# janhq/cortex.llamacpp

Hardware: AMD Instinct MI355X
Metric: decode tok/s, Llama-3-8B Q4_K_M GGUF (prefill tok/s in `prefill_tok_s`) (higher is better)
Workload: dtype int8 dot (Q4_K/Q6_K x Q8_K), f32 accumulate

## Files before the change

cortex.llamacpp_amd/binding.py:

```python
from __future__ import annotations

import ctypes as C
import os

import numpy as np

HERE = os.path.dirname(os.path.abspath(__file__))
F32, F16, Q4_0, Q8_0, Q4_K, Q5_K, Q6_K, Q8_K = 0, 1, 2, 8, 12, 13, 14, 15
Q2_K, Q3_K = 10, 11
Q5_0, IQ4_NL = 6, 20
Q4_1, Q5_1 = 3, 7
IQ4_XS = 23
BF16 = 30
MXFP4 = 39


class MI355Error(RuntimeError):
    pass


def lib_path() -> str:
    return os.environ.get("MI355_LLAMA_LIB") or os.path.join(HERE, "lib", "libmi355_llama.so")


class ModelParams(C.Structure):
    _fields_ = [("n_gpu_layers", C.c_int32), ("main_gpu", C.c_int32), ("use_mmap", C.c_int32), ("use_mlock", C.c_int32),
                ("tp_rank", C.c_int32), ("tp_size", C.c_int32), ("prefill_planes", C.c_int32)]


class ContextParams(C.Structure):
    _fields_ = [("n_ctx", C.c_uint32), ("n_batch", C.c_uint32), ("n_ubatch", C.c_uint32), ("n_seq_max", C.c_uint32),
                ("type_k", C.c_int32), ("type_v", C.c_int32), ("flash_attn", C.c_int32), ("embeddings", C.c_int32),
                ("use_graphs", C.c_int32), ("logits_to_host", C.c_int32)]


class Batch(C.Structure):
    _fields_ = [("n_tokens", C.c_int32), ("token", C.POINTER(C.c_int32)), ("embd", C.POINTER(C.c_float)),
                ("pos", C.POINTER(C.c_int32)), ("n_seq_id", C.POINTER(C.c_int32)),
                ("seq_id", C.POINTER(C.POINTER(C.c_int32))), ("logits", C.POINTER(C.c_int8))]


_vp, _i32, _i64, _u32, _u64, _f32, _sz, _cp = C.c_void_p, C.c_int32, C.c_int64, C.c_uint32, C.c_uint64, C.c_float, C.c_size_t, C.c_char_p
ENGINE_CB = C.CFUNCTYPE(None, C.c_char_p, C.c_char_p, C.c_void_p)
SYMBOLS = {
    "mi355_backend_init": (C.c_int, []),
    "mi355_backend_free": (None, []),
    "mi355_device_count": (C.c_int, []),
    "mi355_last_error": (_cp, []),
    "mi355_time_us": (_i64, []),
    "mi355_print_system_info": (_cp, []),
    "mi355_model_default_params": (ModelParams, []),
    "mi355_model_load_from_file": (_vp, [_cp, ModelParams]),
    "mi355_model_free": (None, [_vp]),
    "mi355_model_n_vocab": (_i32, [_vp]),
    "mi355_model_n_embd": (_i32, [_vp]),
    "mi355_model_n_layer": (_i32, [_vp]),
    "mi355_model_n_head": (_i32, [_vp]),
    "mi355_model_n_head_kv": (_i32, [_vp]),
    "mi355_model_n_ctx_train": (_i32, [_vp]),
    "mi355_model_size": (_u64, [_vp]),
    "mi355_model_cpu_buffer": (_u64, [_vp]),
    "mi355_model_other_buffer": (_u64, [_vp]),
    "mi355_model_bytes_per_token": (_u64, [_vp]),
    "mi355_model_planes_bytes": (_u64, [_vp]),
    "mi355_debug_set_option": (C.c_int, [_cp, _i32]),
    "mi355_model_desc": (_cp, [_vp]),
    "mi355_model_meta_str": (C.c_int, [_vp, _cp, _cp, _sz]),
    "mi355_context_default_params": (ContextParams, []),
    "mi355_context_new": (_vp, [_vp, ContextParams]),
    "mi355_context_free": (None, [_vp]),
    "mi355_n_ctx": (_u32, [_vp]),
    "mi355_n_batch": (_u32, [_vp]),
    "mi355_n_ubatch": (_u32, [_vp]),
    "mi355_context_device_bytes": (_u64, [_vp]),
    "mi355_batch_init": (Batch, [_i32, _i32, _i32]),
    "mi355_batch_free": (None, [Batch]),
    "mi355_decode": (_i32, [_vp, Batch]),
    "mi355_greedy_steps": (_i32, [_vp, _i32, _i32, _i32, _i32, _vp]),
    "mi355_get_logits_ith": (C.POINTER(C.c_float), [_vp, _i32]),
    "mi355_get_argmax_ith": (_i32, [_vp, _i32]),
    "mi355_get_topk_ith": (_i32, [_vp, _i32, _i32, _i32, _vp, _vp, _vp, _f32, _f32, _f32, _vp, _vp]),
    "mi355_debug_mega_steps": (C.c_int64, [_vp]),
    "mi355_debug_engine_steps": (C.c_int64, [_vp]),
    "mi355_debug_fused_skipped_steps": (C.c_int64, [_vp]),
    "mi355_debug_qkv_attn_launches": (C.c_int64, [_vp]),
    "mi355_debug_qkv_attn_plan": (C.c_int64, [C.c_int32] * 10 + [C.POINTER(C.c_int32)]),
    "mi355_set_embeddings": (None, [_vp, _i32]),
    "mi355_get_embeddings_ith": (C.POINTER(C.c_float), [_vp, _i32]),
    "mi355_synchronize": (None, [_vp]),
    "mi355_kv_cache_clear": (None, [_vp]),
    "mi355_kv_cache_seq_rm": (_i32, [_vp, _i32, _i32, _i32]),
    "mi355_kv_cache_seq_cp": (None, [_vp, _i32, _i32, _i32, _i32]),
    "mi355_kv_cache_seq_add": (None, [_vp, _i32, _i32, _i32, _i32]),
    "mi355_kv_cache_used_cells": (_i32, [_vp]),
    "mi355_debug_enable_taps": (None, [_vp, _i32]),
    "mi355_debug_layer_out": (_i32, [_vp, _i32, _vp, _sz]),
    "mi355_op_quantize_act": (C.c_int, [_i32, _vp, _i64, _i64, _vp]),
    "mi355_op_rms_norm_quant": (C.c_int, [_vp, _vp, _i64, _i64, _f32, _vp, _vp]),
    "mi355_op_swiglu_quant": (C.c_int, [_vp, _vp, _i64, _i64, _vp]),
    "mi355_op_mul_mat": (C.c_int, [_i32, _vp, _i64, _i64, _vp, _i64, _vp, _vp, _vp]),
    "mi355_op_mul_mat_add": (C.c_int, [_i32, _vp, _i64, _i64, _vp, _i64, _vp, _vp]),
    "mi355_op_mul_mat_fused": (C.c_int, [_i32, _vp, _i64, _i64, _vp, _vp, _f32, _vp]),
    "mi355_op_f32_to_bf16": (C.c_int, [_vp, _i64, _vp]),
    "mi355_op_mul_mat_bf16": (C.c_int, [_i32, _vp, _vp, _i64, _vp, _i64, _vp, _vp, _i32, _i32, _i32, _i32, _vp]),
    "mi355_op_ffn_gate_up": (C.c_int, [_i32, _vp, _vp, _i64, _i64, _vp, _i64, _vp]),
    "mi355_op_rms_norm_mul": (C.c_int, [_vp, _vp, _i64, _i64, _f32, _vp]),
    "mi355_op_rope": (C.c_int, [_vp, _i32, _i32, _i32, _vp, _i64, _f32, _f32, _vp, _i32]),
    "mi355_op_rope_yarn": (C.c_int, [_vp, _i32, _i32, _i32, _vp, _i64, _f32, _f32, _vp, _i32, _f32, _f32, _f32, _f32]),
    "mi355_op_get_rows": (C.c_int, [_i32, _vp, _i64, _i64, _vp, _i64, _vp]),
    "mi355_op_swiglu": (C.c_int, [_vp, _vp, _i64, _vp]),
    "mi355_op_soft_max": (C.c_int, [_vp, _vp, _i64, _i64, _f32, _vp]),
    "mi355_op_moe_route": (C.c_int, [_vp, _i64, _i32, _i32, _vp, _vp]),
    "mi355_op_moe_router": (C.c_int, [_i32, _vp, _i32, _i64, _vp, _i64, _i32, _i32, _vp, _vp, _vp, _vp]),
    "mi355_op_flash_attn": (C.c_int, [_vp, _i64, _i32, _i32, _i32, _i32, _vp, _i32, _vp, _i32, _vp, _vp, _f32, _vp]),
    "mi355_op_attn_step": (C.c_int, [_vp, _vp, _vp, _i32, _i32, _i32, _i32, _vp, _i32, _vp, _i32, _vp, _i32, _i32, _f32, _i32, _f32, _i32, _vp, _i64, _vp, _i32,
                                     _vp, _vp, _vp, _vp]),
    "mi355_op_attn_decode_neox": (C.c_int, [_vp, _vp, _vp, _i32, _i32, _i32, _i32, _vp, _i32, _vp, _i32, _vp, _i32, _i32, _f32, _f32, _vp, _vp, _f32, _i32,
                                            _vp, _vp, _vp]),
    "mi355_op_kv_store": (C.c_int, [_i32, _vp, _vp, _vp, _i64, _i32, _i32, _i32, _i32, _i32, _i32, _i32, _i32, _vp, _vp, _f32, _f32, _vp, _vp, _vp, _f32, _vp, _vp]),
    "mi355_op_k_shift": (C.c_int, [_i32, _i32, _i32, _i32, _i32, _i32, _vp, _f32, _f32, _vp, _f32, _f32, _f32, _f32, _vp]),
    "mi355_bench_hbm_read": (C.c_double, [_sz, C.c_int]),
    "mi355_profile_last_decode": (_i32, [_vp, C.POINTER(_cp), C.POINTER(_f32), _i32]),
    "mi355_profile_enable": (None, [_vp, _i32]),
    "mi355_debug_force_moe_ids": (C.c_int, [_vp, _vp, _i32, _i32, _i32]),
    "mi355_bench_weight_sweep": (C.c_double, [_vp, C.c_int, C.POINTER(_u64)]),
    "mi355_bench_weight_sweep2": (C.c_double, [_vp, C.c_int, C.POINTER(_u64), C.POINTER(C.c_int32)]),
    "mi355_tokenize": (_i32, [_vp, _cp, _i32, C.POINTER(C.c_int32), _i32, _i32, _i32]),
    "mi355_token_to_piece": (_i32, [_vp, _i32, C.c_char_p, _i32, _i32]),
    "mi355_token_bos": (_i32, [_vp]),
    "mi355_token_eos": (_i32, [_vp]),
    "mi355_token_is_eog": (_i32, [_vp, _i32]),
    "mi355_engine_create": (_vp, []),
    "mi355_engine_destroy": (None, [_vp]),
    "mi355_engine_set_release_callback": (None, [_vp, _vp]),
    "mi355_engine_load_model": (None, [_vp, _cp, ENGINE_CB, _vp]),
    "mi355_engine_unload_model": (None, [_vp, _cp, ENGINE_CB, _vp]),
    "mi355_engine_get_model_status": (None, [_vp, _cp, ENGINE_CB, _vp]),
    "mi355_engine_get_models": (None, [_vp, _cp, ENGINE_CB, _vp]),
    "mi355_engine_handle_chat_completion": (None, [_vp, _cp, ENGINE_CB, _vp]),
    "mi355_engine_handle_embedding": (None, [_vp, _cp, ENGINE_CB, _vp]),
    "mi355_engine_is_supported": (_i32, [_vp, _cp]),
    "mi355_engine_stop_inferencing": (None, [_vp, _cp]),
    "mi355_engine_load": (None, [_vp, _cp, _cp, _i32, _cp, _i32, _i32]),
    "mi355_engine_unload": (None, [_vp]),
    "mi355_engine_set_file_logger": (None, [_vp, _i32, _cp]),
    "mi355_engine_set_log_level": (None, [_vp, _i32]),
    "mi355_engine_set_log_callback": (None, [_vp, _vp, _vp]),
    "mi355_clip_model_load": (_vp, [_cp, _i32]),
    "mi355_clip_free": (None, [_vp]),
    "mi355_clip_n_mmproj_embd": (_i32, [_vp]),
    "mi355_clip_n_patches": (_i32, [_vp]),
    "mi355_clip_image_size": (_i32, [_vp]),
    "mi355_clip_max_image_rows": (_i32, [_vp]),
    "mi355_clip_image_preprocess_grid": (_i32, [_vp, _vp, _i32, _i32, _vp, _sz, _vp, _vp]),
    "mi355_clip_image_load_from_bytes": (_i32, [_vp, _sz, C.POINTER(_i32), C.POINTER(_i32), _vp, _sz]),
    "mi355_clip_image_preprocess": (_i32, [_vp, _vp, _i32, _i32, _vp]),
    "mi355_clip_image_encode": (_i32, [_vp, _vp, _vp]),
    "mi355_llava_image_embed_from_bytes": (_i32, [_vp, _vp, _sz, _vp, _sz]),
    "mi355_tp_p2p_local_handle": (C.c_int, [_vp, _sz, _sz]),
    "mi355_tp_p2p_local_handle2": (C.c_int, [_vp, _sz, _sz, _sz]),
    "mi355_tp_p2p_prompt_exchanges": (C.c_int64, []),
    "mi355_tp_p2p_enable": (C.c_int, [_vp, _sz]),
    "mi355_tp_p2p_exchanges": (C.c_int64, []),
    "mi355_tp_unique_id": (C.c_int, [_vp, _sz]),
    "mi355_tp_init": (C.c_int, [_i32, _i32, _i32, _vp, _sz]),
    "mi355_tp_shutdown": (None, []),
    "mi355_tp_worker_main": (C.c_int, [C.c_int]),
    "mi355_tp_rank": (_i32, []),
# ... 498 lines not shown
        pos = np.asarray(pos, np.int32).reshape(-1)
        n = tokens.size
        b = self._batch(n)
        b.n_tokens = n
        C.memmove(b.token, tokens.ctypes.data, 4 * n)
        C.memmove(b.pos, pos.ctypes.data, 4 * n)
        for i in range(n):
            b.n_seq_id[i] = 1
            b.seq_id[i][0] = 0 if seq is None else int(seq[i] if np.ndim(seq) else seq)
            b.logits[i] = (1 if i == n - 1 else 0) if logits is None else int(bool(logits[i]))
        rc = self.lib.mi355_decode(self.h, b)
        if rc < 0:
            raise MI355Error(f"mi355_decode failed ({rc}): {_err(self.lib)}")
        return rc

    def decode_embd(self, embd, pos, seq=None, logits=None) -> int:
        embd = np.ascontiguousarray(embd, np.float32)
        pos = np.asarray(pos, np.int32).reshape(-1)
        n = pos.size
        if embd.shape != (n, self.model.n_embd):
            raise ValueError(f"embd must be [{n}][{self.model.n_embd}]")
        b = self.lib.mi355_batch_init(n, self.model.n_embd, 1)
        try:
            b.n_tokens = n
            C.memmove(b.embd, embd.ctypes.data, embd.nbytes)
            C.memmove(b.pos, pos.ctypes.data, 4 * n)
            for i in range(n):
                b.n_seq_id[i] = 1
                b.seq_id[i][0] = 0 if seq is None else int(seq[i] if np.ndim(seq) else seq)
                b.logits[i] = (1 if i == n - 1 else 0) if logits is None else int(bool(logits[i]))
            rc = self.lib.mi355_decode(self.h, b)
        finally:
            self.lib.mi355_batch_free(b)
        if rc < 0:
            raise MI355Error(f"mi355_decode failed ({rc}): {_err(self.lib)}")
        return rc

    def greedy_steps(self, first: int, pos0: int, n: int, seq: int = 0) -> np.ndarray:
        out = np.empty(n, np.int32)
        done = self.lib.mi355_greedy_steps(self.h, int(first), int(pos0), int(seq), int(n), out.ctypes.data)
        if done != n:
            raise MI355Error(f"mi355_greedy_steps stopped after {done} of {n}: {_err(self.lib)}")
        return out

    def logits(self, i: int = -1) -> np.ndarray:
        p = self.lib.mi355_get_logits_ith(self.h, i)
        if not p:
            raise MI355Error(f"no logits for that batch row: {_err(self.lib)}")
        return np.ctypeslib.as_array(p, shape=(self.model.n_vocab,)).copy()

    def logits_ready(self, i: int = -1) -> None:
        if not self.lib.mi355_get_logits_ith(self.h, i):
            raise MI355Error(f"no logits for that batch row: {_err(self.lib)}")

    def set_embeddings(self, on: bool = True) -> None:
        self.lib.mi355_set_embeddings(self.h, int(on))

    def embeddings(self, i: int = -1) -> np.ndarray:
        p = self.lib.mi355_get_embeddings_ith(self.h, i)
        if not p:
            raise MI355Error("no embeddings for that row")
        return np.ctypeslib.as_array(p, shape=(self.model.n_embd,)).copy()

    def argmax(self, i: int = -1) -> int:
        return int(self.lib.mi355_get_argmax_ith(self.h, i))

    def mega_steps(self) -> int:
        return int(self.lib.mi355_debug_mega_steps(self.h))

    def topk(self, k: int, i: int = -1, adj_tok=(), adj_bias=(), adj_count=(), repeat: float = 1.0, freq: float = 0.0, present: float = 0.0):
        at = np.ascontiguousarray(adj_tok, np.int32); ab = np.ascontiguousarray(adj_bias, np.float32); ac = np.ascontiguousarray(adj_count, np.int32)
        toks = np.zeros(k, np.int32); lg = np.zeros(k, np.float32)
        r = self.lib.mi355_get_topk_ith(self.h, i, k, at.size, _ptr(at), _ptr(ab), _ptr(ac), repeat, freq, present, _ptr(toks), _ptr(lg))
        if r != k:
            raise MI355Error(f"mi355_get_topk_ith failed: {_err(self.lib)}")
        return toks, lg

    def fused_skipped_steps(self) -> int:
        return int(self.lib.mi355_debug_fused_skipped_steps(self.h))

    def qkv_attn_launches(self) -> int:
        return int(self.lib.mi355_debug_qkv_attn_launches(self.h))

    def engine_steps(self) -> int:
        return int(self.lib.mi355_debug_engine_steps(self.h))

    def synchronize(self):
        self.lib.mi355_synchronize(self.h)

    def kv_clear(self):
        self.lib.mi355_kv_cache_clear(self.h)

    def kv_seq_rm(self, seq, p0, p1) -> bool:
        return bool(self.lib.mi355_kv_cache_seq_rm(self.h, seq, p0, p1))

    def kv_seq_cp(self, s, d, p0, p1):
        self.lib.mi355_kv_cache_seq_cp(self.h, s, d, p0, p1)

    def kv_seq_add(self, seq, p0, p1, delta):
        self.lib.mi355_kv_cache_seq_add(self.h, seq, p0, p1, delta)

    def kv_used(self) -> int:
        return int(self.lib.mi355_kv_cache_used_cells(self.h))

    def enable_taps(self, on: bool = True):
        self.lib.mi355_debug_enable_taps(self.h, int(on))

    def layer_out(self, il: int, n_tokens: int) -> np.ndarray:
        out = np.zeros((n_tokens, self.model.n_embd), np.float32)
        n = self.lib.mi355_debug_layer_out(self.h, il, _ptr(out), out.size)
        if n < 0:
            raise MI355Error("debug taps not enabled")
        return out[:n]

    def profile(self, on: bool = True):
        self.lib.mi355_profile_enable(self.h, int(on))

    def last_profile(self) -> dict:
        names = (_cp * 64)()
        us = (_f32 * 64)()
        n = self.lib.mi355_profile_last_decode(self.h, names, us, 64)
        return {names[i].decode(): float(us[i]) for i in range(n)}

    def force_moe_ids(self, ids: np.ndarray) -> None:
        ids = np.ascontiguousarray(ids, np.int32)
        rc = self.lib.mi355_debug_force_moe_ids(self.h, _ptr(ids), ids.shape[0], ids.shape[1], ids.shape[2])
        if rc != 0:
            raise MI355Error(f"mi355_debug_force_moe_ids failed ({rc}): {_err(self.lib)}")

    def weight_sweep_us(self, iters: int = 5):
        b = _u64(0)
        us = self.lib.mi355_bench_weight_sweep(self.h, iters, C.byref(b))
        return float(us), int(b.value)

    def weight_sweep(self, iters: int = 5):
        b, n = _u64(0), C.c_int32(0)
        us = self.lib.mi355_bench_weight_sweep2(self.h, iters, C.byref(b), C.byref(n))
        return float(us), int(b.value), int(n.value)

    def close(self):
        if self._b is not None:
            self.lib.mi355_batch_free(self._b)
            self._b = None
        if self.h:
            self.lib.mi355_context_free(self.h)
            self.h = None


class Engine:

    def __init__(self):
        import json
        import threading
        self._json, self._threading = json, threading
        self.lib = load_library()
        self.h = self.lib.mi355_engine_create()
        if not self.h:
            raise MI355Error(f"mi355_engine_create failed: {_err(self.lib)}")

    def _call(self, fn, body: dict, wait_done: bool = True, timeout: float = 120.0):
        out, done = [], self._threading.Event()

        def on(status, payload, _user):
            st, bd = self._json.loads(status.decode("utf-8", "replace")), self._json.loads(payload.decode("utf-8", "replace"))
            out.append((st, bd))
            if st.get("is_done", True) or st.get("has_error", False):
# ... 38 lines not shown
```

cortex.llamacpp_amd/csrc/c_api.cc:

```cpp
#include "../../include/mi355_llama.h"

#include <atomic>
#include <memory>
#include <new>
#include <chrono>
#include <cstdio>
#include <cstdlib>
#include <cstring>
#include <string>
#include <vector>

#include "../host/clip.h"
#include "../host/engine.h"
#include "../host/hip_backend.h"
#include "../host/log.h"
#include "../host/runtime.h"
#include "../host/tp_comm.h"
#include "../host/tp_split.h"
#include "../host/vocab.h"

namespace mi355 {
const std::string &last_error_string();
}

// ... 144 lines not shown
        std::string err;
        if (!c->init(err)) { fail(err); return nullptr; }
        mi355_context *h = new mi355_context{c.get(), {}};
        c.release();
        return h;
    )
}
void mi355_context_free(mi355_context *ctx) {
    if (!ctx) return;
    delete ctx->c;
    delete ctx;
}
uint32_t mi355_n_ctx(const mi355_context *ctx) { return ctx->c->cp.n_ctx; }
uint32_t mi355_n_batch(const mi355_context *ctx) { return ctx->c->cp.n_batch; }
uint32_t mi355_n_ubatch(const mi355_context *ctx) { return ctx->c->cp.n_ubatch; }
uint64_t mi355_context_device_bytes(const mi355_context *ctx) { return ctx->c->device_bytes; }

mi355_batch mi355_batch_init(int32_t n_tokens, int32_t embd, int32_t n_seq_max) {
    mi355_batch b{};
    if (embd > 0) b.embd = (float *)calloc((size_t)n_tokens * (size_t)embd, sizeof(float));
    else b.token = (mi355_token *)calloc((size_t)n_tokens, sizeof(mi355_token));
    b.pos = (mi355_pos *)calloc((size_t)n_tokens, sizeof(mi355_pos));
    b.n_seq_id = (int32_t *)calloc((size_t)n_tokens, sizeof(int32_t));
    b.seq_id = (mi355_seq_id **)calloc((size_t)n_tokens + 1, sizeof(mi355_seq_id *));
    for (int i = 0; i < n_tokens; i++) b.seq_id[i] = (mi355_seq_id *)calloc((size_t)(n_seq_max > 0 ? n_seq_max : 1), sizeof(mi355_seq_id));
    b.seq_id[n_tokens] = nullptr;
    b.logits = (int8_t *)calloc((size_t)n_tokens, 1);
    return b;
}
void mi355_batch_free(mi355_batch b) {
    free(b.token); free(b.embd); free(b.pos); free(b.n_seq_id); free(b.logits);
    if (b.seq_id) {
        for (int i = 0; b.seq_id[i]; i++) free(b.seq_id[i]);
        free(b.seq_id);
    }
}

int32_t mi355_decode(mi355_context *ctx, mi355_batch batch) {
    if (!ctx) return MI355_ERR_ARG;
    MI355_GUARD(return MI355_ERR_ARG,
        const int rc = ctx->c->decode(batch.n_tokens, batch.embd ? nullptr : batch.token, batch.pos, batch.n_seq_id, batch.seq_id, batch.logits, batch.embd);
        if (rc < 0) fail(ctx->c->last_error);
        return rc;
    )
}
int32_t mi355_greedy_steps(mi355_context *ctx, mi355_token first, mi355_pos pos0, mi355_seq_id seq, int32_t n, mi355_token *out_tokens) {
    if (!ctx || n < 0) return MI355_ERR_ARG;
    MI355_GUARD(return MI355_ERR_ARG,
        int32_t tok = first, one = 1, sid = seq;
        int32_t *sp = &sid;
        const int8_t flag = 1;
        for (int32_t i = 0; i < n; i++) {
            int32_t pos = pos0 + i;
            const int rc = ctx->c->decode(1, &tok, &pos, &one, &sp, &flag);
            if (rc != 0) { if (rc < 0) fail(ctx->c->last_error); return i; }
            if (!ctx->c->logits_ith(0)) { fail("no logits row"); return i; }
            tok = ctx->c->argmax_ith(0);
            if (tok < 0) { fail(ctx->c->last_error.empty() ? "arg-max failed" : ctx->c->last_error); return i; }
            if (out_tokens) out_tokens[i] = tok;
        }
        return n;
    )
}
float *mi355_get_logits_ith(mi355_context *ctx, int32_t i) {
    float *p = ctx->c->logits_ith(i);
    if (!p) fail(ctx->c->last_error.empty() ? "no logits for that batch row" : ctx->c->last_error);
    return p;
}
int32_t mi355_get_argmax_ith(mi355_context *ctx, int32_t i) { return ctx->c->argmax_ith(i); }
int32_t mi355_get_topk_ith(mi355_context *ctx, int32_t i, int32_t k, int32_t n_adj, const int32_t *adj_tok, const float *adj_bias, const int32_t *adj_count,
                           float penalty_repeat, float penalty_freq, float penalty_present, int32_t *toks_out, float *logits_out) {
    if (!ctx || !toks_out || !logits_out || n_adj < 0 || n_adj > TOPK_MAX_ADJ || (n_adj > 0 && (!adj_tok || !adj_bias || !adj_count))) { fail("bad arguments"); return -1; }
    TopkAdj a{};
    a.n = n_adj; a.repeat = penalty_repeat; a.freq = penalty_freq; a.present = penalty_present;
    for (int j = 0; j < n_adj; j++) { a.tok[j] = adj_tok[j]; a.bias[j] = adj_bias[j]; a.cnt[j] = adj_count[j]; }
    const int r = ctx->c->topk_ith(i, k, a, toks_out, logits_out);
    if (r < 0) fail(ctx->c->last_error.empty() ? "top-k failed" : ctx->c->last_error);
    return r;
}
int64_t mi355_debug_mega_steps(const mi355_context *ctx) { return ctx->c->mega_steps; }
int64_t mi355_debug_engine_steps(const mi355_context *ctx) { return ctx->c->engine_steps; }
int64_t mi355_debug_fused_skipped_steps(const mi355_context *ctx) { return ctx->c->fused_skipped_steps; }
int64_t mi355_debug_qkv_attn_launches(const mi355_context *ctx) { return ctx->c->qkv_attn_launches; }
int64_t mi355_debug_qkv_attn_plan(int32_t type_q, int32_t type_k, int32_t type_v, int32_t type_o, int32_t n_embd, int32_t n_head, int32_t n_head_kv, int32_t head_dim,
                                  int32_t type_kv, int32_t n_kv, int32_t *slots_out) {
    int slots = 0;
    const size_t lds = qkv_attn_out_plan_lds(type_q, type_k, type_v, type_o, n_embd, n_head, n_head_kv, head_dim, type_kv, n_kv, &slots);
    if (slots_out) *slots_out = slots;
    return (int64_t)lds;
}
void mi355_set_embeddings(mi355_context *ctx, int32_t enabled) { ctx->c->embeddings_enabled = enabled != 0 || ctx->c->model->hp.encoder; }
float *mi355_get_embeddings_ith(mi355_context *ctx, int32_t i) { return ctx->c->embeddings_ith(i); }
void mi355_synchronize(mi355_context *ctx) { ctx->c->synchronize(); }

mi355_clip *mi355_clip_model_load(const char *path, int32_t main_gpu) {
    if (!path) { fail("clip_model_load: no path"); return nullptr; }
    MI355_GUARD(return nullptr,
        std::unique_ptr<mi355_clip> c(new mi355_clip);
        const std::string err = c->m.load(path, main_gpu < 0 ? 0 : main_gpu);
        if (!err.empty()) { fail(err); return nullptr; }
        return c.release();
    )
}
void mi355_clip_free(mi355_clip *clip) { delete clip; }
int32_t mi355_clip_n_mmproj_embd(const mi355_clip *clip) { return clip ? clip->m.proj_dim : 0; }
int32_t mi355_clip_n_patches(const mi355_clip *clip) { return clip ? clip->m.n_patches() : 0; }
int32_t mi355_clip_image_size(const mi355_clip *clip) { return clip ? clip->m.image_size : 0; }
int32_t mi355_clip_max_image_rows(const mi355_clip *clip) { return clip ? clip->m.max_image_rows() : 0; }
int32_t mi355_clip_image_preprocess_grid(const mi355_clip *clip, const uint8_t *rgb, int32_t nx, int32_t ny, float *out, size_t out_floats, int32_t *grid_w, int32_t *grid_h) {
    if (!clip || !rgb || !out || nx <= 0 || ny <= 0) { fail("clip_image_preprocess_grid: bad arguments"); return MI355_ERR_ARG; }
    MI355_GUARD(return MI355_ERR_ARG,
        ClipImageU8 img;
        img.nx = nx; img.ny = ny; img.rgb.assign(rgb, rgb + (size_t)3 * nx * ny);
        std::vector<std::vector<float>> imgs;
        int gw = 0, gh = 0;
        clip->m.preprocess_all(img, imgs, gw, gh);
        const size_t per = (size_t)3 * clip->m.image_size * clip->m.image_size;
        if (out_floats < per * imgs.size()) { fail("clip_image_preprocess_grid: output buffer too small"); return MI355_ERR_ARG; }
        for (size_t i = 0; i < imgs.size(); i++) memcpy(out + i * per, imgs[i].data(), per * sizeof(float));
        if (grid_w) *grid_w = gw;
        if (grid_h) *grid_h = gh;
        return (int32_t)imgs.size();
    )
}
int32_t mi355_clip_image_load_from_bytes(const uint8_t *bytes, size_t n_bytes, int32_t *nx, int32_t *ny, uint8_t *rgb_out, size_t rgb_cap) {
    MI355_GUARD(return MI355_ERR_ARG,
        ClipImageU8 img;
        const std::string err = clip_image_load_from_bytes(bytes, n_bytes, img);
        if (!err.empty()) { fail(err); return MI355_ERR_ARG; }
        if (nx) *nx = img.nx;
        if (ny) *ny = img.ny;
        if (rgb_out) {
            if (rgb_cap < img.rgb.size()) { fail("clip_image_load_from_bytes: rgb_cap too small"); return MI355_ERR_ARG; }
            memcpy(rgb_out, img.rgb.data(), img.rgb.size());
        }
        return MI355_OK;
    )
}
int32_t mi355_clip_image_preprocess(const mi355_clip *clip, const uint8_t *rgb, int32_t nx, int32_t ny, float *out) {
    if (!clip || !rgb || !out || nx <= 0 || ny <= 0) { fail("clip_image_preprocess: bad arguments"); return MI355_ERR_ARG; }
    MI355_GUARD(return MI355_ERR_ARG,
        ClipImageU8 img;
        img.nx = nx; img.ny = ny; img.rgb.assign(rgb, rgb + (size_t)3 * nx * ny);
        std::vector<float> f;
        clip->m.preprocess(img, f);
        memcpy(out, f.data(), f.size() * sizeof(float));
        return MI355_OK;
    )
}
int32_t mi355_clip_image_encode(mi355_clip *clip, const float *img, float *out) {
    if (!clip || !img || !out) { fail("clip_image_encode: bad arguments"); return MI355_ERR_ARG; }
    MI355_GUARD(return MI355_ERR_ARG,
        const std::string err = clip->m.encode(img, out);
        if (!err.empty()) { fail(err); return MI355_ERR_ARG; }
        return MI355_OK;
    )
}
int32_t mi355_llava_image_embed_from_bytes(mi355_clip *clip, const uint8_t *bytes, size_t n_bytes, float *out, size_t out_floats) {
    if (!clip || !bytes || !out) { fail("llava_image_embed: bad arguments"); return MI355_ERR_ARG; }
    MI355_GUARD(return MI355_ERR_ARG,
        ClipImageU8 img;
        std::string err = clip_image_load_from_bytes(bytes, n_bytes, img);
        if (!err.empty()) { fail(err); return MI355_ERR_ARG; }
        std::vector<float> rows;
        int n_rows = 0;
        err = clip->m.embed(img, rows, n_rows);
// ... 843 lines not shown
    if (form < 2 && ((size_t)n_rot + kv_dim) * 4 > 48 * 1024) { fail("n_head_kv * head_dim too wide for the generic kernel's LDS"); return MI355_ERR_ARG; }
    if (form < 2 && (q_norm || k_norm) && (n_rot != D || (D != 64 && D != 128))) { fail("the q / k norm works on whole heads of 64 or 128"); return MI355_ERR_ARG; }
    std::vector<uint8_t> kc, vc;
    std::vector<uint16_t> ks, vs;
    cache_planes_from_rows(type_k, k_cache, G, D, n_cells, kc, ks);
    cache_planes_from_rows(type_v, v_cache, G, D, n_cells, vc, vs);
    DevBuf dk(kc.size()), dks(ks.size() * 2 + 16), dv(vc.size()), dvs(vs.size() * 2 + 16), dqn((size_t)D * 4), dkn_w((size_t)D * 4), dff((size_t)n_rot * 2 + 16);
    DevBuf dq((size_t)T * q_dim * 4), dkn((size_t)T * kv_dim * 4), dvn((size_t)T * kv_dim * 4), dtp((size_t)T * 4), dcell((size_t)T * 4), dcsb((size_t)T * n_rot * 4 + 64);
    if (!dk.up(kc.data(), kc.size()) || !dv.up(vc.data(), vc.size()) || !dks.p || !dvs.p || !dq.p || (q && !dq.up(q, (size_t)T * q_dim * 4)) ||
        !dkn.up(k, (size_t)T * kv_dim * 4) || !dvn.up(v, (size_t)T * kv_dim * 4) || !dtp.up(tok_pos, (size_t)T * 4) || !dcell.up(tok_cell, (size_t)T * 4) || !dcsb.p ||
        (q_norm && !dqn.up(q_norm, (size_t)D * 4)) || (k_norm && !dkn_w.up(k_norm, (size_t)D * 4)) ||
        (freq_factors && !dff.up(freq_factors, (size_t)(n_rot / 2) * 4))) { fail("device alloc/copy failed"); return MI355_ERR_OOM; }
    if (!ks.empty() && !dks.up(ks.data(), ks.size() * 2)) return MI355_ERR_OOM;
    if (!vs.empty() && !dvs.up(vs.data(), vs.size() * 2)) return MI355_ERR_OOM;
    RopeArgs ra{};
    ra.n_rot = n_rot; ra.freq_base = rope_base; ra.freq_scale = freq_scale; ra.freq_factors = freq_factors ? dff.as<float>() : nullptr; ra.neox = neox ? 1 : 0;
    ra.q_norm = q_norm ? dqn.as<float>() : nullptr; ra.k_norm = k_norm ? dkn_w.as<float>() : nullptr; ra.qk_eps = eps;
    if (form == 2 && !rope_q_kv_store_fast_applicable(H, G, D, type_k, type_v, ra)) { fail("the vectorised prompt store has no form for these arguments"); return MI355_ERR_ARG; }
    if (form == 3 && !kv_store_fast_applicable(G, D, type_k, type_v, ra)) { fail("the small-batch decode store has no form for these arguments"); return MI355_ERR_ARG; }
    KVLayerView kv{};
    kv.k = dk.as<uint8_t>(); kv.kd = dks.as<uint16_t>(); kv.v = dv.as<uint8_t>(); kv.vd = dvs.as<uint16_t>();
    hipError_t e = hipSuccess;
    if (form != 0) e = launch_rope_table(dtp.as<int32_t>(), (int)T, ra, dcsb.as<float>(), nullptr);
    if (e != hipSuccess) return hip_fail(e, "rope_table");
    if (form < 2)
        e = launch_rope_kv_store(dq.as<float>(), dkn.as<float>(), dvn.as<float>(), (int)T, H, G, D, dtp.as<int32_t>(), dcell.as<int32_t>(), ra, kv, type_k, type_v, n_cells,
                                 form == 1 ? dcsb.as<float>() : nullptr, nullptr);
    else if (form == 2)
        e = launch_rope_q_kv_store_fast(dq.as<float>(), dkn.as<float>(), dvn.as<float>(), (int)T, H, G, D, dcsb.as<float>(), ra, dcell.as<int32_t>(), kv, type_k, type_v,
                                        n_cells, nullptr);
    else
        e = launch_kv_store_fast(dkn.as<float>(), dvn.as<float>(), (int)T, G, D, dcsb.as<float>(), ra, dcell.as<int32_t>(), kv, type_k, type_v, n_cells, nullptr);
    if (e == hipSuccess) e = hipDeviceSynchronize();
    if (e != hipSuccess) return hip_fail(e, "kv_store");
    if (form != 3 && !dq.down(q, (size_t)T * q_dim * 4)) return MI355_ERR_HIP;
    if (!cache_rows_from_planes(type_k, dk, dks, G, D, n_cells, k_cache) || !cache_rows_from_planes(type_v, dv, dvs, G, D, n_cells, v_cache)) return MI355_ERR_HIP;
    return MI355_OK;
}

int mi355_op_k_shift(int32_t type_k, int32_t G, int32_t D, int32_t n_rot, int32_t neox, int32_t n_cells, const int32_t *delta, float rope_base, float freq_scale,
                     const float *freq_factors, float ext_factor, float attn_factor, float corr_lo, float corr_hi, void *k_cache) {
    if (!need_device()) return MI355_ERR_NO_DEVICE;
    if (!delta || !k_cache || G < 1 || D < 32 || D % 32 || n_rot < 2 || n_rot > D || n_rot % 2 || n_cells < 1) { fail("bad geometry / null argument"); return MI355_ERR_ARG; }
    if (type_k != T_F16 && type_k != T_Q8_0 && type_k != T_Q4_0) { fail("bad cache type"); return MI355_ERR_ARG; }
    if (((size_t)n_rot + (size_t)G * D) * 4 > 48 * 1024) { fail("n_head_kv * head_dim too wide for the kernel's LDS"); return MI355_ERR_ARG; }
    std::vector<uint8_t> kc;
    std::vector<uint16_t> ks;
    cache_planes_from_rows(type_k, k_cache, G, D, n_cells, kc, ks);
    DevBuf dk(kc.size()), dks(ks.size() * 2 + 16), dd((size_t)n_cells * 4), dff((size_t)n_rot * 2 + 16);
    if (!dk.up(kc.data(), kc.size()) || !dks.p || !dd.up(delta, (size_t)n_cells * 4) || (freq_factors && !dff.up(freq_factors, (size_t)(n_rot / 2) * 4))) {
        fail("device alloc/copy failed"); return MI355_ERR_OOM;
    }
    if (!ks.empty() && !dks.up(ks.data(), ks.size() * 2)) return MI355_ERR_OOM;
    RopeArgs ra{};
    ra.n_rot = n_rot; ra.freq_base = rope_base; ra.freq_scale = freq_scale; ra.freq_factors = freq_factors ? dff.as<float>() : nullptr; ra.neox = neox ? 1 : 0;
    ra.ext_factor = ext_factor; ra.attn_factor = attn_factor; ra.corr_lo = corr_lo; ra.corr_hi = corr_hi;
    KVLayerView kv{};
    kv.k = dk.as<uint8_t>(); kv.kd = dks.as<uint16_t>();
    hipError_t e = launch_k_shift(kv, type_k, G, D, n_cells, dd.as<int32_t>(), ra, nullptr);
    if (e == hipSuccess) e = hipDeviceSynchronize();
    if (e != hipSuccess) return hip_fail(e, "k_shift");
    return cache_rows_from_planes(type_k, dk, dks, G, D, n_cells, k_cache) ? MI355_OK : MI355_ERR_HIP;
}

int mi355_debug_set_option(const char *name, int32_t value) {
    if (!name) return MI355_ERR_ARG;
    if (!strcmp(name, "mmq_planes")) { g_op_mmq_planes = value != 0; return MI355_OK; }
    if (!strcmp(name, "mmq_tiles")) { mmq_set_tiles(value); return MI355_OK; }
    if (!strcmp(name, "mmq_q80_tiles")) { mmq_q80_set_tiles(value); return MI355_OK; }
    if (!strcmp(name, "mmq_split")) { mmq_set_split(value); return MI355_OK; }
    if (!strcmp(name, "mmq_lds_form")) { mmq_set_lds_form(value); return MI355_OK; }
    if (!strcmp(name, "mmq_ksplit")) { g_op_mmq_ksplit = value != 0; return MI355_OK; }
    if (!strcmp(name, "attn_store_fuse")) { set_attn_store_fuse(value != 0); return MI355_OK; }
    if (!strcmp(name, "rope_fast")) { set_rope_fast(value != 0); return MI355_OK; }
    if (!strcmp(name, "decode_mega") || !strcmp(name, "decode_engine")) {
        if (value > 0 && !experiments_built()) { fail(std::string(name) + ": the experiment kernels are not in this build (MI355_BUILD_EXPERIMENTS=1 python cortex.llamacpp_amd/build.py --force)"); return MI355_ERR_ARG; }
        if (name[7] == 'm') set_decode_mega(value != 0); else set_decode_engine(value);
        return MI355_OK;
    }
    if (!strcmp(name, "tp_p2p")) { tp_p2p_use(value != 0); return MI355_OK; }
    if (!strcmp(name, "tp_p2p_prompt")) { tp_p2p_use_prompt(value != 0); return MI355_OK; }
    if (!strcmp(name, "mmvq_stream")) { mmvq_set_stream(value != 0); return MI355_OK; }
    if (!strcmp(name, "attn_out_fused")) { set_attn_out_fused(value); return MI355_OK; }
    if (!strcmp(name, "qkv_attn_fused")) { set_qkv_attn_fused(value); return MI355_OK; }
    if (!strcmp(name, "moe_group_min")) { set_moe_group_min(value); return MI355_OK; }
    if (!strcmp(name, "moe_q80_grouped")) { set_moe_q80_grouped(value != 0); return MI355_OK; }
    if (!strcmp(name, "fa_v_acc_f16")) { set_fa_v_acc_f16(value); return MI355_OK; }
    if (!strcmp(name, "raise_stream_error")) { debug_raise_stream_error((unsigned)value); return MI355_OK; }
    if (!strcmp(name, "tp_null_group")) { tp_set_null_group(0, value); return MI355_OK; }
    fail(std::string("unknown option ") + name);
    return MI355_ERR_ARG;
}

int mi355_tp_unique_id(void *id_out, size_t cap) {
    if (!need_device()) return MI355_ERR_NO_DEVICE;
    std::string err;
    const int n = tp_unique_id(id_out, cap, err);
    if (n < 0) { fail(err); return MI355_ERR_ARG; }
    return n;
}
int mi355_tp_init(int32_t device, int32_t rank, int32_t size, const void *id, size_t id_len) {
    if (!need_device()) return MI355_ERR_NO_DEVICE;
    if (hipSetDevice(device) != hipSuccess) { fail("hipSetDevice failed"); return MI355_ERR_ARG; }
    std::string err;
    if (tp_init(rank, size, id, id_len, err) != 0) { fail(err); return MI355_ERR_ARG; }
    return MI355_OK;
}
void mi355_tp_shutdown(void) { tp_shutdown(); }
int mi355_tp_worker_main(int sock_fd) {
    try {
        if (!g_backend_ok && mi355_backend_init() != MI355_OK) return 66;
        return tp_split_worker_main(sock_fd);
    } catch (const std::exception &e) {
        fprintf(stderr, "mi355_tp_worker: %s\n", e.what());
        return 70;
    } catch (...) { return 70; }
}
int32_t mi355_tp_rank(void) { return tp_rank(); }
int32_t mi355_tp_size(void) { return tp_size(); }
int mi355_tp_set_host_exchange(mi355_tp_host_exchange fn, void *user, int32_t rank, int32_t size) {
    if (fn && (size < 1 || rank < 0 || rank >= size)) { fail("bad rank / size"); return MI355_ERR_ARG; }
    tp_set_host_exchange(reinterpret_cast<tp_host_exchange_fn>(fn), user, rank, size);
    return MI355_OK;
}

int mi355_tp_p2p_local_handle2(void *out, size_t cap, size_t max_floats, size_t prompt_floats) {
    if (!need_device()) return MI355_ERR_NO_DEVICE;
    std::string err;
    const int n = tp_p2p_local_handle(out, cap, max_floats, prompt_floats, err);
    if (n < 0) { fail(err); return MI355_ERR_ARG; }
    return n;
}
int mi355_tp_p2p_local_handle(void *out, size_t cap, size_t max_floats) { return mi355_tp_p2p_local_handle2(out, cap, max_floats, 0); }
int mi355_tp_p2p_enable(const void *handles, size_t len) {
    if (!need_device()) return MI355_ERR_NO_DEVICE;
    std::string err;
    if (tp_p2p_enable(handles, len, err) != 0) { fail(err); return MI355_ERR_HIP; }
    return MI355_OK;
}
int64_t mi355_tp_p2p_exchanges(void) { return tp_p2p_exchanges(); }
int64_t mi355_tp_p2p_prompt_exchanges(void) { return tp_p2p_prompt_exchanges(); }

double mi355_bench_hbm_read(size_t bytes, int iters) {
    if (!need_device()) return -1.0;
    return hbm_read_probe(bytes, iters);
}

static Vocab *model_vocab(mi355_model *m) {
    if (!m) { fail("null model"); return nullptr; }
    if (!m->vocab_tried) {
        m->vocab_tried = true;
        std::string err;
        m->vocab_ok = m->vocab.load(*m->m->file, err);
        if (!m->vocab_ok) fail("tokenizer: " + err);
    }
    return m->vocab_ok ? &m->vocab : nullptr;
}
int32_t mi355_tokenize(mi355_model *m, const char *text, int32_t text_len, mi355_token *out, int32_t cap, int32_t add_special, int32_t parse_special) {
    MI355_GUARD(return INT32_MIN,
        Vocab *v = model_vocab(m);
        if (!v || !text || text_len < 0) return INT32_MIN;
        const std::vector<int32_t> ids = v->tokenize(std::string(text, (size_t)text_len), add_special != 0, parse_special != 0);
        if ((int64_t)ids.size() > cap || !out) return -(int32_t)ids.size();
        memcpy(out, ids.data(), ids.size() * sizeof(int32_t));
        return (int32_t)ids.size();
    )
// ... 94 lines not shown
```

cortex.llamacpp_amd/csrc/kernels.h:

```cpp
#pragma once

#include "dev_common.h"

namespace mi355 {

struct ActQuant {
    int8_t *qs = nullptr;
    float *d = nullptr;
    int16_t *bsums = nullptr;
    int8_t *qs0 = nullptr;
    uint16_t *d0 = nullptr;
};

enum { EPI_STORE = 0, EPI_ADD = 1, EPI_SWIGLU = 2 };

struct MMVQSeg {
    const uint8_t *W;
    float *out;
    const float *resid;
    int type;
    int n_rows;
    int ld_out;
    size_t row_bytes;
    const int32_t *expert_sel;
    size_t expert_stride;
};

struct MMVQArgs {
    MMVQSeg seg[3];
    int seg_block0[4];
    int n_seg;
    int K;
    int T;
    int epi;
    int need_q8k, need_q80;
    int nck;
    int red_off;
    const int8_t *aq; const float *ad; const int16_t *abs;
    const int8_t *aq0; const uint16_t *ad0;
    int fuse_mode;
    const float *nx; const float *nw; float neps;
    int n_sel, sel_out_stride, sel_nx_stride;
    float *out_host;
};

hipError_t launch_mmvq(MMVQArgs a, hipStream_t st);
void mmvq_fast_set_threads(int nt);
inline bool mmvq_fast_kb_ok(int kb) { return (kb >= 1 && kb <= 7) || kb == 9 || kb == 10 || kb == 11 || kb == 14 || kb == 15; }
bool mmvq_fast_applicable(const MMVQArgs &a);
hipError_t launch_mmvq_fast(MMVQArgs a, hipStream_t st);
hipError_t launch_mmvq_ints(MMVQArgs a, int32_t *isum, int32_t *msum, hipStream_t st);
size_t mmvq_fast_plan(MMVQArgs &a, int blocks, int waves);
void mmvq_set_stream(bool on);
bool mmvq_stream_applicable(const MMVQArgs &a);
void mmvq_stream_set_anyorder_for_timing(bool on);
hipError_t launch_mmvq_stream(MMVQArgs a, hipStream_t st);

void mmvq_stream_plan(MMVQArgs &a, int blocks);
void mmvq_stream_set_error_word(unsigned *w);
struct KernelTimer {
    virtual ~KernelTimer() = default;
    virtual bool next(const char *role, hipEvent_t *start, hipEvent_t *stop) = 0;
};
void set_kernel_timer(KernelTimer *t);
KernelTimer *kernel_timer();

bool experiments_built();
struct EngineLayer {
    MMVQArgs wo, gu, dn, qkv;
    int has_qkv;
    int qk_norm;
};
bool decode_engine_applicable(const EngineLayer &l, int E, int FF);
void decode_engine_plan(EngineLayer &l);
size_t decode_engine_granule_words(int E, int FF);
void decode_engine_set_error_word(unsigned *w);
hipError_t launch_decode_engine(const EngineLayer *layer_dev, int E, int FF, unsigned long long *granules, const unsigned *epoch_dev, int layer_index,
                                unsigned long long *probe, hipStream_t st);

void set_num_cu(int n);
int num_cu();

bool mmq_applicable(int type, int K, int T);
void mmq_set_tiles(int mt);
size_t mmq_planes_bytes(int type, int64_t n_rows, int K);
size_t mmq_q80_copy_bytes(int type, int64_t n_rows, int K);
size_t mmq_q80_copy_row_bytes(int type, int K);
hipError_t launch_expand_q80_copy(int type, const uint8_t *W, size_t row_bytes, int n_rows, int K, uint8_t *dst, hipStream_t st);
hipError_t launch_mmq_expand(int type, const uint8_t *W, size_t row_bytes, int n_rows, int K, uint8_t *planes, hipStream_t st);
struct MMQWorkspace { float *p = nullptr; size_t bytes = 0; };
void mmq_set_split(int n);
void mmq_set_lds_form(int on);
bool mmq_planes_moe_ok(int type, int n_rows, int K);
hipError_t launch_mmq_planes_swiglu_moe(int type, const uint8_t *planes_gate, const uint8_t *planes_up, size_t plane_stride, int n_expert, const int32_t *meta,
                                        int n_rows, int K, int rows_max, const ActQuant &q, float *out, int ld_out, hipStream_t st);
hipError_t launch_mmq_planes_moe(int type, const uint8_t *planes, size_t plane_stride, int n_expert, const int32_t *meta, int n_rows, int K, int rows_max,
                                 const ActQuant &q, float *out, int ld_out, hipStream_t st);
hipError_t launch_mmq_planes(int type, const uint8_t *planes, int n_rows, int K, int T, const ActQuant &q, const int8_t *bh, const int8_t *bl,
                             float *out, int ld_out, const float *resid, hipStream_t st, MMQWorkspace wsp = MMQWorkspace());
struct MMQSeg {
    const uint8_t *W; size_t row_bytes; int n_rows, type;
    float *out; int ld_out; const float *resid;
    int tile0;
};
bool mmq_q80_applicable(int type, int K, int T);
hipError_t launch_mmq_q80(const uint8_t *W, size_t row_bytes, int n_rows, int K, int T, const ActQuant &q, float *out, int ld_out,
                          const float *resid, hipStream_t st, int form = 0, bool any_T = false);
enum : int { Q80_FORM_F16 = 0, Q80_FORM_MINS = 1, Q80_FORM_E8 = 2 };
int mmq_q80_copy_form(int type);
bool mmq_q80_moe_ok(int type, int n_rows, int K);
hipError_t launch_mmq_q80_moe(int type, const uint8_t *const *W, float *const *outs, int n_seg, size_t expert_stride, int n_expert, const int32_t *meta, int n_rows,
                              int K, int rows_max, const ActQuant &q, int ld_out, hipStream_t st);
void mmq_q80_set_tiles(int mt);
hipError_t launch_mmq_planes_multi(int type, const uint8_t *planes, const int *seg_rows, float *const *outs, const int *lds_out, int n_seg, int K, int T,
                                   const ActQuant &q, const int8_t *bh, const int8_t *bl, const float *resid, hipStream_t st,
                                   MMQWorkspace wsp = MMQWorkspace(), const int *seg_types = nullptr);
bool mmq_planes_mixed_ok(const int *seg_rows, int n_seg, int K, int T, MMQWorkspace wsp);
bool mmq_planes_swiglu_ok(int type_gate, int type_up, int n_rows, int K, int T);
hipError_t launch_mmq_planes_swiglu(int type, const uint8_t *planes_gate, const uint8_t *planes_up, int n_rows, int K, int T, const ActQuant &q,
                                    float *out, int ld_out, hipStream_t st);
bool mmq_ksplit_applicable(int type, int K, int T);
bool mmq_ksplit_preferred(int type, int n_rows, int K, int T, bool has_planes, bool pair = false);
hipError_t launch_mmq_ksplit_multi(const MMQSeg *segs, int n_seg, int K, int T, const ActQuant &q, const int8_t *bh, const int8_t *bl,
                                   bool swiglu, hipStream_t st);
hipError_t launch_mmq_ksplit(int type, const uint8_t *W, size_t row_bytes, int n_rows, int K, int T, const ActQuant &q,
                             const int8_t *bh, const int8_t *bl, float *out, int ld_out, const float *resid, hipStream_t st);
size_t mmq_prep_bytes(int K, int T);
// ... 194 lines not shown
```

cortex.llamacpp_amd/csrc/mmvq_stream.hip:

```cpp
#include "mmvq_stream_dev.h"

namespace mi355 {

namespace {

template <int KB, int FUSE, bool MOE>
__device__ __forceinline__ void stream_body(const MMVQArgs &ka) {
    extern __shared__ __attribute__((aligned(16))) uint8_t smem[];
#ifdef MI355_STREAM_PROBE
    const unsigned long long t_top = wall_clock64();
#endif
    StOp a;
    op_setup<false, MOE>(ka, a);
    const int wave = uni(tid_now() >> 6);
    sync_init(smem);
#ifdef MI355_STREAM_PROBE
    {
        unsigned dep = uni((int)a.total); asm volatile("" : "+s"(dep));
        const unsigned long long t_args = wall_clock64() + (dep & 0);
        if (g_stream_probe && (threadIdx.x & 63) == 0) {
            unsigned long long *pp = &g_stream_probe[(((size_t)(a.nck >> 2) * 256 + blockIdx.x) * ST_NW + wave) * 8];
            pp[0] = t_top; pp[7] = t_args;
        }
    }
#endif
    if (a.n_rows_wg <= 0) return;
    if (wave < ST_NL) {
        const int lane = tid_now() & 63;
        int *sy = reinterpret_cast<int *>(smem + ST_OFF_SYNC);
        LoaderState st{0, 0, 0, (unsigned)ST_RING_SLOTS, 0};
        const int early = (FUSE == 1 && a.ns_pad > ST_RING_SLOTS) ? ST_EARLY : 0;
        if (early == 0) ST_SPIN_WHILE(ld_sync(sy + SY_GO) < ST_NC, 0);
        ST_STAMP(2);
        loader_op(st, a, smem, wave, 0u, lane, early);
        ST_STAMP(1);
        loader_drain(st, smem, wave);
        ST_STAMP(5);
        return;
    }
    consumer_dispatch<KB, FUSE>(a, smem, wave - ST_NL, 0u, st_layout(KB));
}
struct StFast { const float *nx; const uint8_t *wbase; unsigned ow0, ow1, ow2, onw, kf, sg0, sg1, sg2, rb01, rb2; };
__device__ __forceinline__ void st_fast_setup(StFast f, StOp &o) {
    asm volatile("" : "+s"(f.ow0), "+s"(f.ow1), "+s"(f.ow2), "+s"(f.sg0), "+s"(f.sg1), "+s"(f.sg2), "+s"(f.rb01), "+s"(f.rb2));
    const unsigned kf = f.kf;
    const int nseg = (int)((kf >> 28) & 3u), lo1 = (int)((kf >> 8) & 1023u), lo2 = (int)((kf >> 18) & 1023u);
    const bool swiglu = ((kf >> 30) & 1u) != 0;
    const int b = (int)blockIdx.x;
    unsigned g = f.sg0, rb = f.rb01 & 0xffffu, ow = f.ow0;
    int lo = 0;
    if (nseg > 1 && b >= lo1) { g = f.sg1; rb = f.rb01 >> 16; ow = f.ow1; lo = lo1; }
    if (nseg > 2 && b >= lo2) { g = f.sg2; rb = f.rb2 & 0xffffu; ow = f.ow2; lo = lo2; }
    const int rpb = (int)(g & 2047u), full = (int)((g >> 11) & 1023u), rem = (int)(g >> 21);
    const int bl = b - lo;
    const int rows = bl < full ? rpb : bl == full ? rem : 0;
    o.W = f.wbase + ((size_t)ow << 4);
    o.W1 = f.wbase + ((size_t)f.ow1 << 4);
    o.b0 = bl * rpb; o.n_rows_wg = rows; o.row_bytes = rb;
    o.swiglu = swiglu;
    o.total = (unsigned)rows * rb;
    const int per_tensor = (int)((o.total + ST_SLOT - 1) / ST_SLOT);
    o.ns_raw = swiglu ? 2 * per_tensor : per_tensor;
    o.ns_pad = (o.ns_raw + 1) & ~1;
}

template <int KB>
__device__ __forceinline__ void stream_body_fast(const StFast &fa) {
    extern __shared__ __attribute__((aligned(16))) uint8_t smem[];
    const int wave = uni(tid_now() >> 6), lane = tid_now() & 63;
    EarlyAct<KB> ea;
    early_issue<KB, 1>(fa.nx, reinterpret_cast<const float *>(fa.wbase + ((size_t)fa.onw << 4)), (int)(fa.kf & 255u) << 8, wave >= ST_NL ? wave - ST_NL : 0, lane, ea);
    sync_init(smem);
    if (wave < ST_NL) {
        StOp a;
        st_fast_setup(fa, a);
        if (a.n_rows_wg <= 0) return;
        LoaderState st{0, 0, 0, (unsigned)ST_RING_SLOTS, 0};
        loader_op(st, a, smem, wave, 0u, lane, 0);
        loader_drain(st, smem, wave);
        return;
    }
    typedef const __attribute__((address_space(4))) MMVQArgs *KArgP;
    static_assert(alignof(MMVQArgs) == 8, "kernel argument layout: 14 preloaded dwords, then MMVQArgs at byte 56");
    const __attribute__((address_space(4))) char *kseg = (const __attribute__((address_space(4))) char *)__builtin_amdgcn_kernarg_segment_ptr();
    asm volatile("" : "+s"(kseg) :: "memory");
    const __attribute__((address_space(4))) MMVQArgs &ka = *(KArgP)(kseg + 56);
    StOp a;
    op_setup<false, false>(ka, a);
    if (wave == ST_NL && lane == 0) {
        StOp la;
        st_fast_setup(fa, la);
        const uint8_t *w_arg = a.W;
        if (la.n_rows_wg != a.n_rows_wg || (a.n_rows_wg > 0 && (la.W != w_arg || la.b0 != a.b0 || la.total != a.total || la.row_bytes != a.row_bytes || la.ns_pad != a.ns_pad ||
                                                                 (a.swiglu && la.W1 != a.W1)))) st_timeout(ST_ERR_LOADER);
    }
    if (a.n_rows_wg <= 0) return;
    consumer_dispatch<KB, 1, 0, true>(a, smem, wave - ST_NL, 0u, st_layout(KB), EngIO(), &ea);
}
#define MI355_ST_KERNEL_FAST(NAME)                                                                            \
    template <int KB>                                                                                         \
    __global__ __launch_bounds__(ST_NT) void NAME(const float *f_nx, const uint8_t *f_wbase, unsigned f_ow0, unsigned f_ow1, unsigned f_ow2, unsigned f_onw, unsigned f_kf, \
                                                  unsigned f_sg0, unsigned f_sg1, unsigned f_sg2, unsigned f_rb01, unsigned f_rb2, const MMVQArgs ka_by_value) {            \
        stream_body_fast<KB>(StFast{f_nx, f_wbase, f_ow0, f_ow1, f_ow2, f_onw, f_kf, f_sg0, f_sg1, f_sg2, f_rb01, f_rb2});                                                \
    }
MI355_ST_KERNEL_FAST(mmvq_stream_gate_up_fast)
MI355_ST_KERNEL_FAST(mmvq_stream_head_fast)
#undef MI355_ST_KERNEL_FAST

template <int KB>
__device__ __forceinline__ void stream_body_early(const float *f_nx, unsigned f_k8) {
    extern __shared__ __attribute__((aligned(16))) uint8_t smem[];
    const int wave = uni(tid_now() >> 6), lane = tid_now() & 63;
    EarlyAct<KB> ea;
    early_issue<KB, 2>(f_nx, nullptr, (int)f_k8 << 8, wave >= ST_NL ? wave - ST_NL : 0, lane, ea);
    sync_init(smem);
    typedef const __attribute__((address_space(4))) MMVQArgs *KArgP;
    const __attribute__((address_space(4))) char *kseg = (const __attribute__((address_space(4))) char *)__builtin_amdgcn_kernarg_segment_ptr();
    asm volatile("" : "+s"(kseg) :: "memory");
    const __attribute__((address_space(4))) MMVQArgs &ka = *(KArgP)(kseg + 16);
    StOp a;
    op_setup<false, false>(ka, a);
    if (a.n_rows_wg <= 0) return;
    if (wave < ST_NL) {
        int *sy = reinterpret_cast<int *>(smem + ST_OFF_SYNC);
        LoaderState st{0, 0, 0, (unsigned)ST_RING_SLOTS, 0};
        ST_SPIN_WHILE(ld_sync(sy + SY_GO) < ST_NC, 0);
        loader_op(st, a, smem, wave, 0u, lane, 0);
        loader_drain(st, smem, wave);
        return;
    }
    if (wave == ST_NL && lane == 0 && (a.nx != f_nx || (unsigned)(a.K >> 8) != f_k8)) st_timeout(ST_ERR_LOADER);
    consumer_dispatch<KB, 2, 0, true>(a, smem, wave - ST_NL, 0u, st_layout(KB), EngIO(), &ea);
}
template <int KB>
__global__ __launch_bounds__(ST_NT) void mmvq_stream_ffn_down_early(const float *f_nx, unsigned f_k8, const MMVQArgs ka_by_value) {
    static_assert(alignof(MMVQArgs) == 8, "kernel argument layout: two preloaded words (12 bytes), then MMVQArgs at byte 16");
    stream_body_early<KB>(f_nx, f_k8);
}

#define MI355_ST_KERNEL(NAME)                                                                                 \
    template <int KB, int FUSE, bool MOE = false>                                                             \
    __global__ __launch_bounds__(ST_NT) void NAME(const MMVQArgs ka) { stream_body<KB, FUSE, MOE>(ka); }
MI355_ST_KERNEL(mmvq_stream_kernel)
MI355_ST_KERNEL(mmvq_stream_qkv)
MI355_ST_KERNEL(mmvq_stream_gate_up)
MI355_ST_KERNEL(mmvq_stream_ffn_down)
MI355_ST_KERNEL(mmvq_stream_head)
#undef MI355_ST_KERNEL

}

#ifdef MI355_STREAM_PROBE
void mmvq_stream_set_probe(unsigned long long *p) { (void)hipMemcpyToSymbol(HIP_SYMBOL(g_stream_probe), &p, sizeof(p)); }
#endif

#ifndef MI355_STREAM_Q80_MIN_MB
#define MI355_STREAM_Q80_MIN_MB 16
#endif
static constexpr size_t STREAM_Q80_MIN_BYTES = (size_t)MI355_STREAM_Q80_MIN_MB << 20;

bool mmvq_stream_applicable(const MMVQArgs &a) {
    if (a.T != 1 || a.K <= 0 || (a.K % 256) != 0) return false;
    if (a.out_host && (a.n_seg != 1 || a.epi != EPI_STORE || a.n_sel > 1 || a.seg[0].expert_sel)) return false;
    if (a.n_sel > 1 && (a.n_sel > 8 || (a.epi == EPI_SWIGLU ? 1 : a.n_seg) != 1 || a.epi == EPI_ADD)) return false;
    if (a.n_sel > 1 || a.seg[0].expert_sel) {
        const int kbm = (a.K + 2047) >> 11;
        if (!((a.fuse_mode == 1 && (kbm == 1 || kbm == 2)) || (a.fuse_mode == 2 && (kbm == 2 || kbm == 4 || kbm == 7)))) return false;
    }
    const int kb = (a.K + 2047) >> 11;
    if (kb != 1 && kb != 2 && kb != 3 && kb != 4 && kb != 6 && kb != 7 && kb != 10) return false;
    if (a.fuse_mode < 0 || a.fuse_mode > 2) return false;
    if (a.fuse_mode == 1 && a.K > 8192) return false;
    const bool swiglu = a.epi == EPI_SWIGLU;
    if (swiglu && a.fuse_mode != 1) return false;
    if (swiglu && (a.n_seg != 2 || a.seg[0].type != a.seg[1].type || a.seg[0].n_rows != a.seg[1].n_rows || a.seg[0].row_bytes != a.seg[1].row_bytes)) return false;
    const int n = swiglu ? 1 : a.n_seg;
    bool all_q80 = true;
    size_t launch_bytes = 0;
    for (int s = 0; s < (swiglu ? 2 : n); s++) { all_q80 = all_q80 && a.seg[s].type == T_Q8_0; launch_bytes += (size_t)a.seg[s].n_rows * a.seg[s].row_bytes; }
    if (all_q80 && launch_bytes < STREAM_Q80_MIN_BYTES) return false;
    for (int s = 0; s < (swiglu ? 2 : n); s++) {
        const MMVQSeg &g = a.seg[s];
        const int t = g.type;
        if (t != T_Q4_K && t != T_Q5_K && t != T_Q6_K && t != T_Q8_0 && t != T_Q2_K && t != T_Q3_K && t != T_Q4_0 && t != T_Q5_0 && t != T_IQ4_NL && t != T_IQ4_XS && !nib32_has_min(t) && t != T_MXFP4) return false;
        if (g.expert_sel && (s != 0 && !(swiglu && s == 1))) return false;
        if ((g.row_bytes % 16) != 0 || g.row_bytes < 512) return false;
        if (g.row_bytes > (size_t)ST_MAX_STEP) return false;
        if (kb <= 2 && 2 * g.row_bytes > (size_t)ST_PAIR_MAX) return false;
        if ((reinterpret_cast<uintptr_t>(g.W) & 15) != 0) return false;
        if (a.fuse_mode == 0 && (act_is_q80(t) || !a.aq || !a.ad || !a.abs)) return false;
    }
    if (a.fuse_mode == 0 && (((uintptr_t)a.aq | (uintptr_t)a.ad | (uintptr_t)a.abs) & 15) != 0) return false;
    if (a.fuse_mode != 0 && (reinterpret_cast<uintptr_t>(a.nx) & 15) != 0) return false;
    if (a.fuse_mode == 1 && (reinterpret_cast<uintptr_t>(a.nw) & 15) != 0) return false;
    return true;
}

void mmvq_stream_set_error_word(unsigned *w) { (void)hipMemcpyToSymbol(HIP_SYMBOL(g_st_err_word), &w, sizeof(w)); }

void mmvq_stream_plan(MMVQArgs &a, int max_blocks) {
    const bool swiglu = a.epi == EPI_SWIGLU;
    const int n = swiglu ? 1 : a.n_seg;
    double bytes[3] = {0, 0, 0}, total = 0;
    for (int s = 0; s < n; s++) { bytes[s] = (double)a.seg[s].n_rows * (double)a.seg[s].row_bytes; total += bytes[s]; }
    int left = max_blocks;
    a.seg_block0[0] = 0;
    for (int s = 0; s < n; s++) {
        int nb = s == n - 1 ? left : (int)((double)max_blocks * bytes[s] / total + 0.5);
        if (nb < 1) nb = 1;
        if (nb > left - (n - 1 - s)) nb = left - (n - 1 - s);
        if (nb > a.seg[s].n_rows) nb = a.seg[s].n_rows;
        a.seg_block0[s + 1] = a.seg_block0[s] + nb;
        left -= nb;
    }
    for (int s = n; s < 3; s++) a.seg_block0[s + 1] = a.seg_block0[n];
    if (swiglu) a.n_seg = 1;
}

static KernelTimer *g_kernel_timer = nullptr;
void set_kernel_timer(KernelTimer *t) { g_kernel_timer = t; }
KernelTimer *kernel_timer() { return g_kernel_timer; }
static bool g_stream_anyorder = false;
void mmvq_stream_set_anyorder_for_timing(bool on) { g_stream_anyorder = on; }

static StFast st_fast_pack(const MMVQArgs &a, int blocks) {
    StFast f{};
    const bool swiglu = a.epi == EPI_SWIGLU;
    const int nseg = a.n_seg;
    if (a.n_sel > 1 || a.seg[0].expert_sel || a.fuse_mode != 1 || !a.nx || !a.nw || nseg < 1 || nseg > 3 || (a.K >> 8) > 255 || a.out_host) return f;
    uintptr_t lo = ~(uintptr_t)0, hi = 0;
    const void *ptrs[4] = {a.seg[0].W, nseg > 1 || swiglu ? (const void *)a.seg[1].W : (const void *)a.seg[0].W, nseg > 2 ? a.seg[2].W : a.seg[0].W, (const void *)a.nw};
    for (int i = 0; i < 4; i++) { const uintptr_t p = (uintptr_t)ptrs[i]; if (p & 15) return f; lo = p < lo ? p : lo; hi = p > hi ? p : hi; }
    if (((hi - lo) >> 4) > 0xffffffffull) return f;
    f.nx = a.nx; f.wbase = reinterpret_cast<const uint8_t *>(lo);
    f.ow0 = (unsigned)(((uintptr_t)ptrs[0] - lo) >> 4); f.ow1 = (unsigned)(((uintptr_t)ptrs[1] - lo) >> 4);
    f.ow2 = (unsigned)(((uintptr_t)ptrs[2] - lo) >> 4); f.onw = (unsigned)(((uintptr_t)ptrs[3] - lo) >> 4);
    unsigned sg[3] = {0, 0, 0}, rb[3] = {0, 0, 0};
    for (int s = 0; s < nseg; s++) {
        const int nblk = a.seg_block0[s + 1] - a.seg_block0[s];
        if (nblk <= 0 || a.seg[s].row_bytes > 0xffffu) return f;
        const int rpb = (a.seg[s].n_rows + nblk - 1) / nblk;
        const int full = a.seg[s].n_rows / rpb, rem = a.seg[s].n_rows - full * rpb;
        if (rpb > 2047 || full > 1023 || rem > 2047) return f;
        sg[s] = (unsigned)rpb | ((unsigned)full << 11) | ((unsigned)rem << 21);
        rb[s] = (unsigned)a.seg[s].row_bytes;
    }
    if (a.seg_block0[0] != 0 || a.seg_block0[1] > 1023 || a.seg_block0[2] > 1023 || blocks != a.seg_block0[3]) return f;
    if (swiglu && (a.seg[1].row_bytes != a.seg[0].row_bytes || a.seg[1].n_rows != a.seg[0].n_rows)) return f;
    f.sg0 = sg[0]; f.sg1 = sg[1]; f.sg2 = sg[2]; f.rb01 = rb[0] | (rb[1] << 16); f.rb2 = rb[2];
    f.kf = (unsigned)(a.K >> 8) | ((unsigned)(nseg > 1 ? a.seg_block0[1] : 0) << 8) | ((unsigned)(nseg > 2 ? a.seg_block0[2] : 0) << 18) | ((unsigned)nseg << 28) |
           (swiglu ? 1u << 30 : 0u) | (1u << 31);
    return f;
}

hipError_t launch_mmvq_stream(MMVQArgs a, hipStream_t st) {
    if (!mmvq_stream_applicable(a)) return hipErrorInvalidValue;
    const int kb = (a.K + 2047) >> 11;
    mmvq_stream_plan(a, num_cu());
    const int blocks = a.seg_block0[3];
    const size_t lds = (size_t)st_layout(kb).total;
    enum { ROLE_ANY, ROLE_QKV, ROLE_GATE_UP, ROLE_DOWN, ROLE_HEAD };
    int role = ROLE_ANY;
    if (a.n_sel <= 1 && !a.seg[0].expert_sel) {
        if (a.fuse_mode == 1 && a.epi == EPI_SWIGLU) role = ROLE_GATE_UP;
        else if (a.fuse_mode == 1 && a.epi == EPI_STORE && a.n_seg >= 2) role = ROLE_QKV;
        else if (a.fuse_mode == 1 && a.epi == EPI_STORE && a.n_seg == 1 && a.seg[0].n_rows >= 16384) role = ROLE_HEAD;
        else if (a.fuse_mode == 2 && a.epi == EPI_ADD && a.n_seg == 1) role = ROLE_DOWN;
    }
    const char *const role_name = role == ROLE_QKV ? "qkv" : role == ROLE_GATE_UP ? "gate_up" : role == ROLE_DOWN ? "ffn_down" : role == ROLE_HEAD ? "head" : "stream";
    (void)role_name;
    static const bool fast_off = getenv("MI355_STREAM_FAST_START") && getenv("MI355_STREAM_FAST_START")[0] == '0';
    const StFast fp = (role == ROLE_GATE_UP || role == ROLE_HEAD) && !fast_off && !g_stream_anyorder ? st_fast_pack(a, blocks) : StFast{};
    const bool fast_ok = (fp.kf >> 31) != 0;
    static const bool down_early_off = getenv("MI355_STREAM_DOWN_EARLY") && getenv("MI355_STREAM_DOWN_EARLY")[0] == '0';
    const bool down_early = !down_early_off && !g_stream_anyorder && a.nx && !a.out_host;
#define STREAM_K(KERNEL, KBV, FZ)                                                                                        \
    do {                                                                                                                 \
                              \
        hipError_t e = hipFuncSetAttribute(reinterpret_cast<const void *>(&KERNEL<KBV, FZ>), hipFuncAttributeMaxDynamicSharedMemorySize, (int)lds); \
        if (e != hipSuccess) return e;                                                                                   \
        hipEvent_t ev0_ = nullptr, ev1_ = nullptr;                                                                       \
        if (g_stream_anyorder) hipExtLaunchKernelGGL((KERNEL<KBV, FZ>), dim3(blocks), dim3(ST_NT), lds, st, nullptr, nullptr, hipExtAnyOrderLaunch, a); \
        else if (g_kernel_timer && g_kernel_timer->next(role_name, &ev0_, &ev1_)) hipExtLaunchKernelGGL((KERNEL<KBV, FZ>), dim3(blocks), dim3(ST_NT), lds, st, ev0_, ev1_, 0, a); \
        else hipLaunchKernelGGL((KERNEL<KBV, FZ>), dim3(blocks), dim3(ST_NT), lds, st, a);                              \
    } while (0)
#define STREAM0(KBV) STREAM_K(mmvq_stream_kernel, KBV, 0)
#define STREAM_FAST(KERNEL, KBV)                                                                                         \
    do {                                                                                                                 \
        hipError_t e = hipFuncSetAttribute(reinterpret_cast<const void *>(&KERNEL<KBV>), hipFuncAttributeMaxDynamicSharedMemorySize, (int)lds); \
        if (e != hipSuccess) return e;                                                                                   \
        hipEvent_t ev0_ = nullptr, ev1_ = nullptr;                                                                       \
        if (g_kernel_timer && g_kernel_timer->next(role_name, &ev0_, &ev1_))                                             \
            hipExtLaunchKernelGGL((KERNEL<KBV>), dim3(blocks), dim3(ST_NT), lds, st, ev0_, ev1_, 0, fp.nx, fp.wbase, fp.ow0, fp.ow1, fp.ow2, fp.onw, fp.kf, fp.sg0, fp.sg1, fp.sg2, fp.rb01, fp.rb2, a); \
        else hipLaunchKernelGGL((KERNEL<KBV>), dim3(blocks), dim3(ST_NT), lds, st, fp.nx, fp.wbase, fp.ow0, fp.ow1, fp.ow2, fp.onw, fp.kf, fp.sg0, fp.sg1, fp.sg2, fp.rb01, fp.rb2, a); \
    } while (0)
#define STREAM1(KBV)                                                                                                     \
    do {                                                                                                                 \
        if (role == ROLE_QKV) STREAM_K(mmvq_stream_qkv, KBV, 1);                                                         \
        else if (role == ROLE_GATE_UP && fast_ok) STREAM_FAST(mmvq_stream_gate_up_fast, KBV);                            \
        else if (role == ROLE_GATE_UP) STREAM_K(mmvq_stream_gate_up, KBV, 1);                                            \
        else if (role == ROLE_HEAD && fast_ok) STREAM_FAST(mmvq_stream_head_fast, KBV);                                  \
        else if (role == ROLE_HEAD) STREAM_K(mmvq_stream_head, KBV, 1);                                                  \
        else STREAM_K(mmvq_stream_kernel, KBV, 1);                                                                       \
    } while (0)
#define STREAM_EARLY(KBV)                                                                                                \
    do {                                                                                                                 \
        hipError_t e = hipFuncSetAttribute(reinterpret_cast<const void *>(&mmvq_stream_ffn_down_early<KBV>), hipFuncAttributeMaxDynamicSharedMemorySize, (int)lds); \
        if (e != hipSuccess) return e;                                                                                   \
        hipEvent_t ev0_ = nullptr, ev1_ = nullptr;                                                                       \
        if (g_kernel_timer && g_kernel_timer->next(role_name, &ev0_, &ev1_))                                             \
            hipExtLaunchKernelGGL((mmvq_stream_ffn_down_early<KBV>), dim3(blocks), dim3(ST_NT), lds, st, ev0_, ev1_, 0, a.nx, (unsigned)(a.K >> 8), a); \
        else hipLaunchKernelGGL((mmvq_stream_ffn_down_early<KBV>), dim3(blocks), dim3(ST_NT), lds, st, a.nx, (unsigned)(a.K >> 8), a); \
    } while (0)
#define STREAM2(KBV)                                                                                                     \
    do {                                                                                                                 \
        if constexpr (KBV == 6 || KBV == 7) { if (role == ROLE_DOWN && down_early) { STREAM_EARLY(KBV); break; } }       \
        if (role == ROLE_DOWN) STREAM_K(mmvq_stream_ffn_down, KBV, 2); else STREAM_K(mmvq_stream_kernel, KBV, 2);        \
    } while (0)
#define STREAM_F(KBV) do { if (a.fuse_mode == 0) STREAM0(KBV); else if (a.fuse_mode == 1) STREAM1(KBV); else STREAM2(KBV); } while (0)
#define STREAM_MOE(KBV, FZ)                                                                                              \
    do {                                                                                                                 \
        hipError_t e = hipFuncSetAttribute(reinterpret_cast<const void *>(&mmvq_stream_kernel<KBV, FZ, true>), hipFuncAttributeMaxDynamicSharedMemorySize, (int)lds); \
        if (e != hipSuccess) return e;                                                                                   \
        hipLaunchKernelGGL((mmvq_stream_kernel<KBV, FZ, true>), dim3(blocks), dim3(ST_NT), lds, st, a);                 \
    } while (0)
    if (a.n_sel > 1 || a.seg[0].expert_sel) {
        if (a.fuse_mode == 1 && kb == 1) STREAM_MOE(1, 1);
        else if (a.fuse_mode == 1 && kb == 2) STREAM_MOE(2, 1);
        else if (a.fuse_mode == 2 && kb == 2) STREAM_MOE(2, 2);
        else if (a.fuse_mode == 2 && kb == 4) STREAM_MOE(4, 2);
        else if (a.fuse_mode == 2 && kb == 7) STREAM_MOE(7, 2);
        else return hipErrorInvalidValue;
        goto STREAM_DONE;
    }
    switch (kb) {
        case 1: STREAM_F(1); break;
        case 2: STREAM_F(2); break;
        case 3: STREAM_F(3); break;
        case 4: STREAM_F(4); break;
        case 10: if (a.fuse_mode == 2) STREAM2(10); else if (a.fuse_mode == 0) STREAM0(10); else return hipErrorInvalidValue; break;
        case 6: if (a.fuse_mode == 2) STREAM2(6); else if (a.fuse_mode == 0) STREAM0(6); else return hipErrorInvalidValue; break;
        case 7: if (a.fuse_mode == 2) STREAM2(7); else if (a.fuse_mode == 0) STREAM0(7); else return hipErrorInvalidValue; break;
        default: return hipErrorInvalidValue;
    }
    STREAM_DONE:
#undef STREAM_MOE
#undef STREAM_F
#undef STREAM0
#undef STREAM1
#undef STREAM2
#undef STREAM_EARLY
// ... 7 lines not shown
```

cortex.llamacpp_amd/csrc/mmvq_stream_dev.h:

```cpp
#pragma once
#include "mmvq_fast_dev.h"
#include <hip/hip_ext.h>

namespace mi355 {

namespace {

constexpr int ST_NL = 2;
#ifndef MI355_ST_NC
#define MI355_ST_NC 8
#endif
constexpr int ST_NC = MI355_ST_NC;
static_assert(ST_NC >= 1 && ST_NC <= 14, "consumer waves");
constexpr int ST_NW = ST_NL + ST_NC, ST_NT = ST_NW * 64;
#ifndef MI355_ST_RING
#define MI355_ST_RING 131072
#endif
constexpr int ST_RING = MI355_ST_RING;
constexpr unsigned ST_MASK = ST_RING - 1;
constexpr int ST_SI = 4;
constexpr int ST_SLOT = ST_SI * 1024;
constexpr int ST_RING_SLOTS = ST_RING / ST_SLOT;
#ifndef MI355_STREAM_DEPTH
#define MI355_STREAM_DEPTH 12
// ... 64 lines not shown
}
template <bool IL> __device__ __forceinline__ void ring_load(Raw<T_Q5_K> &r, const uint8_t *ring, unsigned base, unsigned row_off, int nb, int sb, const LaneRole &L) {
    const unsigned b = row_off + (unsigned)sb * 176u;
    r.hdr = lds16(RO(b));
    r.qh = lds16(RO(b + 16u));
    r.qh1 = lds16(RO(b + 32u));
    r.q = lds16(RO(b + 48u + (unsigned)L.c * 32u));
    r.q1 = lds16(RO(b + 64u + (unsigned)L.c * 32u));
}
template <bool IL> __device__ __forceinline__ void ring_load(Raw<T_Q6_K> &r, const uint8_t *ring, unsigned base, unsigned row_off, int nb, int sb, const LaneRole &L) {
    r.ql = lds16(RO(row_off + (unsigned)sb * 128u + (unsigned)L.v * 16u));
    r.qh = lds16(RO(row_off + (unsigned)nb * 128u + (unsigned)sb * 64u + (unsigned)L.n * 32u + (unsigned)(L.w & 1) * 16u));
    const unsigned so = row_off + (unsigned)nb * 192u + (unsigned)sb * 16u + 8u * (unsigned)L.n + (unsigned)L.w;
    r.sc_lo = *reinterpret_cast<const int8_t *>(RO(so));
    r.sc_hi = *reinterpret_cast<const int8_t *>(RO(so + 4u));
    r.dh16 = *reinterpret_cast<const uint16_t *>(RO(row_off + (unsigned)nb * 208u + (unsigned)sb * 2u));
}
template <bool IL> __device__ __forceinline__ void ring_load(Raw<T_Q8_0> &r, const uint8_t *ring, unsigned base, unsigned row_off, int nb, int sb, const LaneRole &L) {
    const unsigned b = row_off + (unsigned)sb * 256u + (unsigned)L.v * 32u;
    r.q0 = lds16(RO(b));
    r.q1 = lds16(RO(b + 16u));
    r.dh16 = *reinterpret_cast<const uint16_t *>(RO(row_off + (unsigned)nb * 256u + ((unsigned)sb * 8u + (unsigned)L.v) * 2u));
}
template <bool IL> __device__ __forceinline__ void ring_load(Raw<T_Q2_K> &r, const uint8_t *ring, unsigned base, unsigned row_off, int nb, int sb, const LaneRole &L) {
    r.q = lds16(RO(row_off + (unsigned)sb * 64u + (unsigned)(L.c >> 1) * 32u + (unsigned)L.h * 16u));
    const unsigned so = row_off + (unsigned)nb * 64u + (unsigned)sb * 16u + 4u * (unsigned)L.c + (unsigned)L.h;
    r.sc_lo = *RO(so);
    r.sc_hi = *RO(so + 2u);
    r.dd = *reinterpret_cast<const uint32_t *>(RO(row_off + (unsigned)nb * 80u + (unsigned)sb * 4u));
}
template <bool IL> __device__ __forceinline__ void ring_load(Raw<T_Q3_K> &r, const uint8_t *ring, unsigned base, unsigned row_off, int nb, int sb, const LaneRole &L) {
    r.hm = lds16(RO(row_off + (unsigned)sb * 32u + (unsigned)L.h * 16u));
    r.q = lds16(RO(row_off + (unsigned)nb * 32u + (unsigned)sb * 64u + (unsigned)(L.c >> 1) * 32u + (unsigned)L.h * 16u));
    const unsigned so = row_off + (unsigned)nb * 96u + (unsigned)sb * 12u;
    r.s0w = *reinterpret_cast<const uint32_t *>(RO(so));
    r.s1w = *reinterpret_cast<const uint32_t *>(RO(so + 4u));
    r.s2w = *reinterpret_cast<const uint32_t *>(RO(so + 8u));
    r.dh16 = *reinterpret_cast<const uint16_t *>(RO(row_off + (unsigned)nb * 108u + (unsigned)sb * 2u));
}
template <bool IL, int TYPE> __device__ __forceinline__ void ring_load_nib32(RawNib32<TYPE> &r, const uint8_t *ring, unsigned base, unsigned row_off, int nb, int sb, const LaneRole &L) {
    const unsigned blk = (unsigned)sb * 8u + (unsigned)L.v, half = (unsigned)nb * 128u, nblk = (unsigned)nb * 8u;
    r.q = lds16(RO(row_off + blk * 16u));
    if (TYPE == T_Q5_0) {
        r.qh = *reinterpret_cast<const uint32_t *>(RO(row_off + half + blk * 4u));
        r.dh16 = *reinterpret_cast<const uint16_t *>(RO(row_off + half + nblk * 4u + blk * 2u));
    } else if (nib32_has_min(TYPE)) {
        const unsigned doff = half + (TYPE == T_Q5_1 ? nblk * 4u : 0u);
        r.qh = TYPE == T_Q5_1 ? *reinterpret_cast<const uint32_t *>(RO(row_off + half + blk * 4u)) : 0u;
        r.dh16 = *reinterpret_cast<const uint16_t *>(RO(row_off + doff + blk * 2u));
        r.mh16 = *reinterpret_cast<const uint16_t *>(RO(row_off + doff + nblk * 2u + blk * 2u));
    } else if (nib32_has_e8(TYPE)) {
        r.qh = 0;
        r.dh16 = *reinterpret_cast<const uint8_t *>(RO(row_off + half + blk));
    } else {
        r.qh = 0;
        r.dh16 = *reinterpret_cast<const uint16_t *>(RO(row_off + half + blk * 2u));
    }
}
template <bool IL> __device__ __forceinline__ void ring_load(Raw<T_Q4_0> &r, const uint8_t *ring, unsigned base, unsigned row_off, int nb, int sb, const LaneRole &L) { ring_load_nib32<IL, T_Q4_0>(r, ring, base, row_off, nb, sb, L); }
template <bool IL> __device__ __forceinline__ void ring_load(Raw<T_Q5_0> &r, const uint8_t *ring, unsigned base, unsigned row_off, int nb, int sb, const LaneRole &L) { ring_load_nib32<IL, T_Q5_0>(r, ring, base, row_off, nb, sb, L); }
template <bool IL> __device__ __forceinline__ void ring_load(Raw<T_IQ4_NL> &r, const uint8_t *ring, unsigned base, unsigned row_off, int nb, int sb, const LaneRole &L) { ring_load_nib32<IL, T_IQ4_NL>(r, ring, base, row_off, nb, sb, L); }
template <bool IL> __device__ __forceinline__ void ring_load(Raw<T_Q4_1> &r, const uint8_t *ring, unsigned base, unsigned row_off, int nb, int sb, const LaneRole &L) { ring_load_nib32<IL, T_Q4_1>(r, ring, base, row_off, nb, sb, L); }
template <bool IL> __device__ __forceinline__ void ring_load(Raw<T_Q5_1> &r, const uint8_t *ring, unsigned base, unsigned row_off, int nb, int sb, const LaneRole &L) { ring_load_nib32<IL, T_Q5_1>(r, ring, base, row_off, nb, sb, L); }
template <bool IL> __device__ __forceinline__ void ring_load(Raw<T_MXFP4> &r, const uint8_t *ring, unsigned base, unsigned row_off, int nb, int sb, const LaneRole &L) { ring_load_nib32<IL, T_MXFP4>(r, ring, base, row_off, nb, sb, L); }
template <bool IL> __device__ __forceinline__ void ring_load(Raw<T_IQ4_XS> &r, const uint8_t *ring, unsigned base, unsigned row_off, int nb, int sb, const LaneRole &L) {
    r.q = lds16(RO(row_off + (unsigned)sb * 128u + (unsigned)L.v * 16u));
    r.sl = *reinterpret_cast<const uint32_t *>(RO(row_off + (unsigned)nb * 128u + (unsigned)sb * 4u));
    r.sh16 = *reinterpret_cast<const uint16_t *>(RO(row_off + (unsigned)nb * 132u + (unsigned)sb * 2u));
    r.dh16 = *reinterpret_cast<const uint16_t *>(RO(row_off + (unsigned)nb * 134u + (unsigned)sb * 2u));
}
#undef RO

constexpr int ST_OFF_SYNC = 0, ST_OFF_RED = 256, ST_OFF_RING = 512, ST_OFF_ACT = ST_OFF_RING + ST_RING;
struct StLayout { int qs, d, bs, total; };
__host__ __device__ inline StLayout st_layout(int kb) {
    const int Kp = kb * 2048;
    StLayout l;
    l.qs = ST_OFF_ACT;
    l.d = l.qs + Kp;
    l.bs = l.d + 1024;
    l.total = l.bs + ((Kp / 8 + 1023) & ~1023);
    return l;
}
enum { SY_LANDED = 0, SY_GO = 2, SY_THIN = 3, SY_PRO1 = 8, SY_PRO2 = 12, SY_DONE = 16, SY_READY = 17, SY_ABORT = 18, SY_GATHER = 19, SY_GDONE = 20, SY_STEP = 21, SY_FRONT = 24 };

#ifndef MI355_STREAM_SPIN_LIMIT
#define MI355_STREAM_SPIN_LIMIT (1 << 21)
#endif
constexpr int ST_SPIN_LIMIT = MI355_STREAM_SPIN_LIMIT;
__device__ unsigned *g_st_err_word = nullptr;
__device__ __attribute__((noinline)) void st_timeout(unsigned code) {
    unsigned *w = g_st_err_word;
    if (w) __hip_atomic_fetch_or(w, code, __ATOMIC_RELAXED, __HIP_MEMORY_SCOPE_SYSTEM);
}
enum { ST_ERR_SPIN = 1u, ST_ERR_LOADER = 2u, ST_ERR_DRAIN = 4u, ST_ERR_GATHER = 8u, ST_ERR_ENGINE_WAIT = 16u };
#define ST_SPIN_WHILE(cond, sleep_arg) do { int spins_ = 0; while (cond) { if (++spins_ >= ST_SPIN_LIMIT) { st_timeout(ST_ERR_SPIN); break; } __builtin_amdgcn_s_sleep(sleep_arg); } \
                                            asm volatile("" ::: "memory"); } while (0)
__device__ __forceinline__ void consumers_rendezvous(int *word, int lane, int round = 1) {
    asm volatile("" ::: "memory");
    if (lane == 0) (void)__hip_atomic_fetch_add(word, 1, __ATOMIC_RELAXED, __HIP_MEMORY_SCOPE_WORKGROUP);
    ST_SPIN_WHILE(ld_sync(word) < ST_NC * round, 1);
}

struct StOp {
    int K, epi, nck, type, n_rows, b0, n_rows_wg;
    float neps;
    const int8_t *aq; const float *ad; const int16_t *abs;
    const float *nx, *nw;
    const uint8_t *W, *W1;
    float *out; const float *resid;
    float *out2;
    unsigned row_bytes, total;
    bool swiglu, pair;
    int ns_raw, ns_pad;
};
template <bool MEM, class T> __device__ __forceinline__ T st_uni(T v) {
    if constexpr (!MEM) return v;
    else if constexpr (sizeof(T) == 4) { int b = __builtin_bit_cast(int, v); b = __builtin_amdgcn_readfirstlane(b); return __builtin_bit_cast(T, b); }
    else {
        static_assert(sizeof(T) == 8, "st_uni");
        unsigned long long b = __builtin_bit_cast(unsigned long long, v);
        const unsigned lo = (unsigned)__builtin_amdgcn_readfirstlane((int)(b & 0xffffffffull)), hi = (unsigned)__builtin_amdgcn_readfirstlane((int)(b >> 32));
        b = ((unsigned long long)hi << 32) | lo;
        return __builtin_bit_cast(T, b);
    }
}
struct StDescRegs { unsigned r0, r1; };
static_assert(sizeof(MMVQArgs) <= 512, "MMVQArgs no longer fits two words per lane");
__device__ __forceinline__ StDescRegs st_desc_load(const MMVQArgs &ka) {
    const unsigned *p = reinterpret_cast<const unsigned *>(&ka);
    const int lane = tid_now() & 63;
    constexpr int NW = (int)(sizeof(MMVQArgs) / 4);
    StDescRegs r;
    r.r0 = p[lane < NW ? lane : NW - 1];
    r.r1 = p[64 + lane < NW ? 64 + lane : NW - 1];
    return r;
}
template <class T> __device__ __forceinline__ T st_desc_get(const StDescRegs &r, size_t byte_off) {
    const int d = (int)(byte_off >> 2);
    auto word = [&](int i) { return (unsigned)__builtin_amdgcn_readlane((int)(i < 64 ? r.r0 : r.r1), i & 63); };
    if constexpr (sizeof(T) == 4) { const unsigned w = word(d); return __builtin_bit_cast(T, w); }
    else {
        static_assert(sizeof(T) == 8, "st_desc_get");
        const unsigned long long w = (unsigned long long)word(d) | ((unsigned long long)word(d + 1) << 32);
        return __builtin_bit_cast(T, w);
    }
}
template <bool MEM = false, bool MOE = false, class KA = MMVQArgs>
__device__ __forceinline__ void op_setup(const KA &ka, StOp &o) {
    StDescRegs dr{0u, 0u};
    if constexpr (MEM) dr = st_desc_load(*reinterpret_cast<const MMVQArgs *>(&ka));
#define U(x) (MEM ? st_desc_get<decltype(st_uni<false>(x))>(dr, (size_t)((uintptr_t)&(x) - (uintptr_t)&ka)) : (x))
    const int n_seg = U(ka.n_seg), sb0 = U(ka.seg_block0[0]), sb1 = U(ka.seg_block0[1]), sb2 = U(ka.seg_block0[2]), sb3 = U(ka.seg_block0[3]);
    const int K = U(ka.K), epi = U(ka.epi), nck = U(ka.nck);
    const float neps = U(ka.neps);
    const int8_t *aq = U(ka.aq); const float *ad = U(ka.ad); const int16_t *abs = U(ka.abs); const float *nx = U(ka.nx), *nw = U(ka.nw);
    const uint8_t *w0 = U(ka.seg[0].W), *w1 = U(ka.seg[1].W), *w2 = U(ka.seg[2].W);
    float *o0 = U(ka.seg[0].out), *o1 = U(ka.seg[1].out), *o2 = U(ka.seg[2].out), *oh = U(ka.out_host);
    const float *r0 = U(ka.seg[0].resid), *r1 = U(ka.seg[1].resid), *r2 = U(ka.seg[2].resid);
    const int t0 = U(ka.seg[0].type), t1 = U(ka.seg[1].type), t2 = U(ka.seg[2].type);
    const int n0 = U(ka.seg[0].n_rows), n1 = U(ka.seg[1].n_rows), n2 = U(ka.seg[2].n_rows);
    const unsigned rb0 = (unsigned)U(ka.seg[0].row_bytes), rb1 = (unsigned)U(ka.seg[1].row_bytes), rb2 = (unsigned)U(ka.seg[2].row_bytes);
    int n_sel = 0, sel_os = 0, sel_ns = 0;
    const int32_t *es0 = nullptr, *es1 = nullptr;
    size_t est0 = 0, est1 = 0;
    if constexpr (MOE) {
        n_sel = U(ka.n_sel); sel_os = U(ka.sel_out_stride); sel_ns = U(ka.sel_nx_stride);
        es0 = U(ka.seg[0].expert_sel); es1 = U(ka.seg[1].expert_sel);
        est0 = U(ka.seg[0].expert_stride); est1 = U(ka.seg[1].expert_stride);
    }
#undef U
#define PIN(x) asm volatile("" :: "s"(x))
    PIN(n_seg); PIN(sb0); PIN(sb1); PIN(sb2); PIN(sb3); PIN(K); PIN(epi); PIN(nck); PIN(neps);
    PIN(aq); PIN(ad); PIN(abs); PIN(nx); PIN(nw);
    PIN(w0); PIN(w1); PIN(w2); PIN(o0); PIN(o1); PIN(o2); PIN(oh); PIN(r0); PIN(r1); PIN(r2);
    PIN(t0); PIN(t1); PIN(t2); PIN(n0); PIN(n1); PIN(n2); PIN(rb0); PIN(rb1); PIN(rb2);
    if constexpr (MOE) { PIN(n_sel); PIN(sel_os); PIN(sel_ns); PIN(es0); PIN(es1); PIN(est0); PIN(est1); }
#undef PIN
    int s = 0;
    if (n_seg > 1 && (int)blockIdx.x >= sb1) s = 1;
    if (n_seg > 2 && (int)blockIdx.x >= sb2) s = 2;
    const int lo = s == 0 ? sb0 : s == 1 ? sb1 : sb2, hi = s == 0 ? sb1 : s == 1 ? sb2 : sb3;
    int nblk = hi - lo, bl = (int)blockIdx.x - lo;
    int sel_j = 0;
    if (MOE && n_sel > 1 && nblk >= n_sel && bl >= 0 && bl < nblk) {
        const int per = nblk / n_sel;
        sel_j = bl / per < n_sel ? bl / per : n_sel - 1;
        bl -= sel_j * per;
        nblk = sel_j == n_sel - 1 ? nblk - sel_j * per : per;
    }
    o.K = K; o.epi = epi; o.nck = nck; o.neps = neps; o.aq = aq; o.ad = ad; o.abs = abs; o.nw = nw;
    o.W = s == 0 ? w0 : s == 1 ? w1 : w2; o.W1 = w1;
    if (MOE && es0 && s == 0) {
        o.W += (size_t)es0[sel_j] * est0;
        if (es1) o.W1 += (size_t)es1[sel_j] * est1;
    }
    o.nx = nx; o.out = s == 0 ? o0 : s == 1 ? o1 : o2;
    o.out2 = n_seg == 1 ? oh : nullptr;
    if constexpr (MOE) { o.nx = nx + (size_t)sel_j * (size_t)sel_ns; o.out += (size_t)sel_j * (size_t)sel_os; }
    o.resid = s == 0 ? r0 : s == 1 ? r1 : r2;
    o.type = s == 0 ? t0 : s == 1 ? t1 : t2;
    o.n_rows = s == 0 ? n0 : s == 1 ? n1 : n2;
    o.row_bytes = s == 0 ? rb0 : s == 1 ? rb1 : rb2;
    int b0 = 0, b1 = 0;
    if (nblk > 0 && bl >= 0 && (int)blockIdx.x < sb3) {
        const int rpb = (o.n_rows + nblk - 1) / nblk;
        b0 = bl * rpb; b1 = b0 + rpb;
        if (b0 > o.n_rows) b0 = o.n_rows;
        if (b1 > o.n_rows) b1 = o.n_rows;
    }
    o.b0 = b0; o.n_rows_wg = b1 - b0;
    o.swiglu = epi == EPI_SWIGLU;
    o.pair = 2 * o.row_bytes <= (unsigned)ST_PAIR_MAX;
    o.total = (unsigned)o.n_rows_wg * o.row_bytes;
    const int per_tensor = (int)((o.total + ST_SLOT - 1) / ST_SLOT);
    o.ns_raw = o.swiglu ? 2 * per_tensor : per_tensor;
    o.ns_pad = (o.ns_raw + 1) & ~1;
}

struct EngIO {
    const float *xf = nullptr;
    int ready_round = 0;
    int round = 1;
    unsigned long long *gran = nullptr;
    unsigned tag = 0;
    float *plain = nullptr;
    const float *rs = nullptr;
    unsigned long long *probe = nullptr;
    int step_base = 0;
};
__device__ __forceinline__ void st_store_granule(unsigned long long *g, unsigned tag, unsigned value) {
    __hip_atomic_store(g, ((unsigned long long)tag << 32) | value, __ATOMIC_RELAXED, __HIP_MEMORY_SCOPE_AGENT);
}

template <int KB> struct EarlyAct {
    static constexpr int NJW = (KB * 8 + ST_NC - 1) / ST_NC;
    f32x4_t x[NJW], w[NJW];
};
template <int KB, int FUSE>
__device__ __forceinline__ void early_issue(const float *nx, const float *nw, int K, int c, int lane, EarlyAct<KB> &ea) {
    const int nbt = K >> 8;
#pragma unroll
    for (int i = 0; i < EarlyAct<KB>::NJW; i++) {
        const int b = c + ST_NC * i;
        const int bc = b < nbt ? b : (nbt > 0 ? nbt - 1 : 0);
        ea.x[i] = *reinterpret_cast<const f32x4_t *>(nx + bc * 256 + lane * 4);
        if (FUSE == 1) ea.w[i] = *reinterpret_cast<const f32x4_t *>(nw + bc * 256 + lane * 4);
    }
}
template <int KB, int FUSE, bool Q80, bool XLDS = false, bool EARLY = false>
__device__ __forceinline__ void consumer_prologue(const StOp &a, uint8_t *smem, const StLayout &lay, int c, int lane, const EngIO &io = EngIO(), const EarlyAct<KB> *ea = nullptr) {
    constexpr int NJW = (KB * 8 + ST_NC - 1) / ST_NC;
    const int nbt = a.K >> 8;
    int8_t *qs = reinterpret_cast<int8_t *>(smem + lay.qs);
    float *d = reinterpret_cast<float *>(smem + lay.d);
    int16_t *bs = reinterpret_cast<int16_t *>(smem + lay.bs);
    double *red = reinterpret_cast<double *>(smem + ST_OFF_RED);
    int *sy = reinterpret_cast<int *>(smem + ST_OFF_SYNC);
    f32x4_t rxv[NJW], rwv[NJW];
#pragma unroll
    for (int i = 0; i < NJW; i++) {
// ... 84 lines not shown
    int idle_polls;
    int w_depth = 0, w_space = 0;
};
__device__ __forceinline__ int vm_outstanding() {
    unsigned x;
    asm volatile("s_getreg_b32 %0, hwreg(HW_REG_IB_STS)" : "=s"(x) :: "memory");
    return (int)((x & 0xfu) | ((x >> 18) & 0x30u));
}
__device__ __forceinline__ void loader_publish(LoaderState &st, int *sy, int q) {
    const int done = st.pre + ST_SI * st.issued - vm_outstanding();
    const int landed = done <= st.pre ? 0 : (done - st.pre) / ST_SI;
    if (landed > st.published) { st.published = landed; st_sync(sy + SY_LANDED + q, landed); }
}
template <bool THIN = false>
__device__ __forceinline__ void loader_op(LoaderState &st, const StOp &a, uint8_t *smem, int q, unsigned g0, int lane, int early_slots = 0) {
    int *sy = reinterpret_cast<int *>(smem + ST_OFF_SYNC);
    bool go = early_slots <= 0;
    if (a.ns_pad == 0) return;
    const unsigned ring_lds = lds_addr(smem + ST_OFF_RING);
    const uint8_t *W = (a.swiglu && q == 1 ? a.W1 : a.W) + (size_t)a.b0 * a.row_bytes;
    const unsigned total = a.total, last = total - 16u;
    const unsigned run_stride = a.swiglu ? ST_SLOT : 2u * ST_SLOT;
    unsigned run_off = a.swiglu ? 0u : (unsigned)q * ST_SLOT;
    const uint8_t *pl = W + run_off + (size_t)lane * 16;
    const int n_mine = a.ns_pad / 2;
    for (int i = 0; i < n_mine;) {
        if (!go && i >= early_slots) { ST_SPIN_WHILE(ld_sync(sy + SY_GO) < ST_NC, 0); go = true; }
        loader_publish(st, sy, q);
        const unsigned g = g0 + 2u * (unsigned)i + (unsigned)q;
        int depth = ST_D * ST_SI + st.pre <= 60 ? ST_D : (60 - st.pre) / ST_SI;
        if (THIN && uni(ld_sync(sy + SY_THIN)) != 0) depth = ST_THIN_D;
        bool wait = st.issued - st.published >= depth;
        if (wait) st.w_depth++;
        if (!wait && g + 1u > st.free_until) {
            int f = 0x7fffffff;
#pragma unroll
            for (int c = 0; c < ST_NC; c++) { const int x = uni(ld_sync(sy + SY_FRONT + c)); f = x < f ? x : f; }
            st.free_until = (unsigned)f + ST_RING_SLOTS;
            wait = g + 1u > st.free_until;
            if (wait) st.w_space++;
        }
        if (wait) {
            if (++st.idle_polls > ST_SPIN_LIMIT) { st_timeout(ST_ERR_LOADER); return; }
            __builtin_amdgcn_s_sleep(1);
            continue;
        }
        st.idle_polls = 0;
        const unsigned dst = ring_lds + ((g * ST_SLOT) & ST_MASK);
        if (run_off + ST_SLOT <= total) dma_slot(pl, dst);
        else {
#pragma unroll
            for (int p = 0; p < ST_SI; p++) {
                const unsigned off = run_off + (unsigned)lane * 16u + p * 1024u;
                dma16<true>(W + (off < total ? off : last), dst + p * 1024);
            }
        }
        pl += run_stride; run_off += run_stride;
        i++;
        st.issued++;
    }
}
__device__ __forceinline__ void loader_drain(LoaderState &st, uint8_t *smem, int q) {
    int *sy = reinterpret_cast<int *>(smem + ST_OFF_SYNC);
    int polls = 0;
    while (st.published < st.issued) {
        if (++polls >= ST_SPIN_LIMIT) { st_timeout(ST_ERR_DRAIN); break; }
        loader_publish(st, sy, q); __builtin_amdgcn_s_sleep(1);
    }
}
__device__ __forceinline__ int loader_planes(const StOp &a, uint8_t *smem, const StLayout &lay, int lane) {
    const int nb = a.K >> 8;
    const int nq = (a.K + 1023) >> 10, nbs = ((a.K >> 3) + 1023) >> 10;
    for (int c = 0; c < nq + 1 + nbs; c++) {
        const uint8_t *src; int size; unsigned dst;
        if (c < nq) { src = reinterpret_cast<const uint8_t *>(a.aq) + c * 1024; size = a.K - c * 1024; if (size > 1024) size = 1024; dst = lay.qs + c * 1024; }
        else if (c == nq) { src = reinterpret_cast<const uint8_t *>(a.ad); size = nb * 4; dst = lay.d; }
        else { const int i = c - nq - 1; src = reinterpret_cast<const uint8_t *>(a.abs) + i * 1024; size = (a.K >> 3) - i * 1024; if (size > 1024) size = 1024; dst = lay.bs + i * 1024; }
        const int o = lane * 16 < size ? lane * 16 : size - 16;
        dma16<false>(src + o, lds_addr(smem + dst));
    }
    return nq + 1 + nbs;
}

template <int TYPE, int KB, int FUSE, bool SWIGLU, bool PAIR, int ENG = 0, bool EARLY = false>
__device__ __forceinline__ void consumer_op(const StOp &a, uint8_t *smem, int c, unsigned g0, const StLayout &lay, const EngIO &io = EngIO(), const EarlyAct<KB> *ea = nullptr) {
    using R = Raw<TYPE>;
    constexpr int NP = role_passes<TYPE, KB>(), SBP = role_sbp<TYPE>();
    constexpr bool ACT_REGS = NP <= 2;
    constexpr int STEP = (SWIGLU || PAIR) ? 2 : 1;
    constexpr int UO = (PAIR && !SWIGLU) ? 2 : 1;
    const int lane = tid_now() & 63;
    const int wave = c + ST_NL; (void)wave;
    const LaneRole L = make_role<TYPE>(lane);
    const int nb = a.K >> 8;
    const unsigned rb = a.row_bytes;
    int *sy = reinterpret_cast<int *>(smem + ST_OFF_SYNC);
    const uint8_t *ring = smem + ST_OFF_RING;
    const unsigned base0 = (g0 * ST_SLOT) & ST_MASK, base1 = SWIGLU ? (base0 + ST_SLOT) & ST_MASK : base0;
    const int n_rows_wg = a.n_rows_wg, b0 = a.b0;
    const int n_steps = (n_rows_wg + UO - 1) / UO;
    auto front_of = [&](int s) { return (int)(g0 + (SWIGLU ? 2u * (((unsigned)s * rb) >> 12) : ((unsigned)s * (unsigned)STEP * rb) >> 12)); };
    if (lane == 0) st_sync(sy + SY_FRONT + c, (int)g0);
    const bool rsd_regs = !SWIGLU && a.epi == EPI_ADD && !(ENG != 0 && io.rs) && n_rows_wg <= 64;
    float rsd = 0.0f;
    if (rsd_regs && lane < n_rows_wg) rsd = a.resid[b0 + lane];

    if (FUSE == 1 || FUSE == 2) consumer_prologue<KB, FUSE, act_is_q80(TYPE), ENG == 1, EARLY>(a, smem, lay, c, lane, io, ea);
    else if (FUSE == 3) {
        ST_SPIN_WHILE(ld_sync(sy + SY_READY) < io.ready_round && ld_sync(sy + SY_ABORT) == 0, 1);
    } else if (ENG == 0) {
        const int tix = c * 64 + lane, nq16 = a.K >> 4, nbs16 = a.K >> 7, nb4 = a.K >> 8;
        constexpr int NQ = (KB * 2048 / 16 + ST_NC * 64 - 1) / (ST_NC * 64);
        u32x4_t cq[NQ], cb = {0u, 0u, 0u, 0u};
        float cd = 0.0f;
#pragma unroll
        for (int i = 0; i < NQ; i++) {
            int j = tix + i * ST_NC * 64;
            if (j >= nq16) j = nq16 - 1;
            cq[i] = *reinterpret_cast<const u32x4_t *>(a.aq + (size_t)j * 16);
        }
        cb = *reinterpret_cast<const u32x4_t *>(reinterpret_cast<const uint8_t *>(a.abs) + (size_t)(tix < nbs16 ? tix : nbs16 - 1) * 16);
        cd = a.ad[tix < nb4 ? tix : nb4 - 1];
        asm volatile("" ::: "memory");
        if (lane == 0) (void)__hip_atomic_fetch_add(sy + SY_GO, 1, __ATOMIC_RELAXED, __HIP_MEMORY_SCOPE_WORKGROUP);
#pragma unroll
        for (int i = 0; i < NQ; i++) {
            const int j = tix + i * ST_NC * 64;
            if (j < nq16) *reinterpret_cast<u32x4_t *>(smem + lay.qs + (size_t)j * 16) = cq[i];
        }
        if (tix < nbs16) *reinterpret_cast<u32x4_t *>(smem + lay.bs + (size_t)tix * 16) = cb;
        if (tix < nb4) reinterpret_cast<float *>(smem + lay.d)[tix] = cd;
        consumers_rendezvous(sy + SY_PRO2, lane, io.round);
    } else {
        asm volatile("" ::: "memory");
        if (lane == 0) (void)__hip_atomic_fetch_add(sy + SY_GO, 1, __ATOMIC_RELAXED, __HIP_MEMORY_SCOPE_WORKGROUP);
        ST_SPIN_WHILE(ld_sync(sy + SY_LANDED) < 1, 1);
    }
    ST_STAMP(2);
    const bool eprobe = ENG != 0 && io.probe != nullptr;
    unsigned long long ep_t0 = 0, ep_w = 0, ep_d = 0;
    if (eprobe) { ep_t0 = wall_clock64(); if (lane == 0) io.probe[0] = ep_t0; }
    ActL AL{reinterpret_cast<const int8_t *>(smem + lay.qs), reinterpret_cast<const float *>(smem + lay.d), reinterpret_cast<const int16_t *>(smem + lay.bs)};
    ActSlice S0, S1;
    if (ACT_REGS) {
        S0 = read_slice_t<TYPE>(AL, L.sbl, nb, L);
        if (NP > 1) S1 = read_slice_t<TYPE>(AL, SBP + L.sbl, nb, L);
    }

    float res = 0.0f;
    int rrow = b0;
    int n_done = 0, flushed = 0;
    auto flush = [&](int upto) {
        const int cnt = upto - flushed;
        const int row = rrow;
        float rv = 0.0f;
        if (rsd_regs) rv = __int_as_float(__builtin_amdgcn_ds_bpermute((row - b0) << 2, __float_as_int(rsd)));
        if (lane < cnt) {
            float v = res;
            if (!SWIGLU && a.epi == EPI_ADD) v = (ENG != 0 && io.rs ? io.rs[row - b0] : rsd_regs ? rv : a.resid[row]) + v;
            if (ENG != 0 && io.gran) {
                st_store_granule(io.gran + row, io.tag, __float_as_uint(v));
                if (io.plain) io.plain[row] = v;
            } else {
                a.out[row] = v;
                if (ENG == 0 && a.out2) a.out2[row] = v;
            }
        }
        flushed = upto;
    };
    ST_ACC_DECL;
    ST_T0();
#ifndef MI355_ST_TICKETS
#define MI355_ST_TICKETS 0
#endif
    int s_static = c;
    auto claim = [&]() {
        if (ENG == 0 && !MI355_ST_TICKETS) { const int t = s_static; s_static += ST_NC; return t; }
        int t = 0;
        if (lane == 0) t = __hip_atomic_fetch_add(sy + SY_STEP, 1, __ATOMIC_RELAXED, __HIP_MEMORY_SCOPE_WORKGROUP);
        return uni(t) - io.step_base;
    };
    for (int s = claim(); s < n_steps; s = claim()) {
        if (lane == 0) st_sync(sy + SY_FRONT + c, front_of(s));
        const bool two = STEP == 2 && (SWIGLU || s * 2 + 1 < n_rows_wg);
        const unsigned off0 = SWIGLU ? (unsigned)s * rb : (unsigned)s * (unsigned)STEP * rb;
        const unsigned off1 = SWIGLU ? off0 : (two ? off0 + rb : off0);
        const unsigned end = SWIGLU ? off0 + rb : off0 + (two ? 2u : 1u) * rb;
        const unsigned n = (end + ST_SLOT - 1) / ST_SLOT;
        const unsigned gn = g0 + (SWIGLU ? 2u * n : n);
        const int need0 = (int)((gn + 1u) >> 1), need1 = (int)(gn >> 1);
        ST_SPIN_WHILE(ld_sync(sy + SY_LANDED) < need0 || ld_sync(sy + SY_LANDED + 1) < need1, 1);
        ST_ACC(st_acc_w);
        if (eprobe) { const unsigned long long t_ = wall_clock64(); ep_w += t_ - ep_t0; ep_t0 = t_; }
        float acc0 = 0.0f, acc1 = 0.0f;
#pragma unroll NP <= 2 ? NP : 2
        for (int p = 0; p < NP; p++) {
            const ActSlice sl = ACT_REGS ? (p == 0 ? S0 : S1) : read_slice_t<TYPE>(AL, p * SBP + L.sbl, nb, L);
            int sb = p * SBP + L.sbl;
            if (sb >= nb) sb = nb - 1;
            R w0, w1;
            ring_load<SWIGLU>(w0, ring, base0, off0, nb, sb, L);
            if (STEP == 2) ring_load<SWIGLU>(w1, ring, base1, off1, nb, sb, L);
            acc0 += w0.dot(sl, L);
            if (STEP == 2) acc1 += w1.dot(sl, L);
        }
        const float v0 = wave_sum(acc0);
        const float v1 = STEP == 2 ? wave_sum(acc1) : 0.0f;
        asm volatile("" ::: "memory");
        ST_ACC(st_acc_d);
        if (eprobe) { const unsigned long long t_ = wall_clock64(); ep_d += t_ - ep_t0; ep_t0 = t_; }
        const int row0 = b0 + s * UO;
        if (SWIGLU) {
            const float y = (v0 / (1.0f + expf(-v0))) * v1;
            if (lane == (n_done & 63)) { res = y; rrow = row0; }
            n_done++;
        } else {
            if (lane == (n_done & 63)) { res = v0; rrow = row0; }
            n_done++;
            if (two) {
                if ((n_done & 63) == 0) flush(n_done);
                if (lane == (n_done & 63)) { res = v1; rrow = row0 + 1; }
                n_done++;
            }
        }
        if ((n_done & 63) == 0) flush(n_done);
    }
    asm volatile("" ::: "memory");
    if (lane == 0) st_sync(sy + SY_FRONT + c, (int)(g0 + (unsigned)a.ns_pad));
    ST_STAMP(4);
    ST_ACC_OUT();
    if (eprobe && lane == 0) { io.probe[1] = ep_w; io.probe[2] = ep_d; }
    if (flushed < n_done) flush(n_done);
#ifdef MI355_STREAM_PROBE
    asm volatile("s_waitcnt vmcnt(0)" ::: "memory");
    ST_STAMP(5);
#endif
}
template <int KB, int FUSE, int ENG = 0, bool EARLY = false>
__device__ __forceinline__ void consumer_dispatch(const StOp &a, uint8_t *smem, int c, unsigned g0, const StLayout &lay, const EngIO &io = EngIO(), const EarlyAct<KB> *ea = nullptr) {
#define RUN(TY)                                                                                               \
    do {                                                                                                      \
        if (a.swiglu) { if constexpr (FUSE == 1 || (FUSE == 3 && KB <= 4)) consumer_op<TY, KB, FUSE, true, true, ENG, EARLY>(a, smem, c, g0, lay, io, ea); } \
        else if (a.pair) { if constexpr (KB <= 4 || ENG == 0) consumer_op<TY, KB, FUSE, false, true, ENG, EARLY>(a, smem, c, g0, lay, io, ea); } \
        else { if constexpr (KB >= 3) consumer_op<TY, KB, FUSE, false, false, ENG, EARLY>(a, smem, c, g0, lay, io, ea); } \
    } while (0)
    switch (a.type) {
        case T_Q4_K: RUN(T_Q4_K); break;
        case T_Q5_K: RUN(T_Q5_K); break;
        case T_Q6_K: RUN(T_Q6_K); break;
        case T_Q8_0: if constexpr (FUSE == 1 || FUSE == 2) RUN(T_Q8_0); break;
        case T_Q2_K: if constexpr (ENG == 0) RUN(T_Q2_K); break;
        case T_Q3_K: if constexpr (ENG == 0) RUN(T_Q3_K); break;
        case T_Q4_0: if constexpr (ENG == 0 && (FUSE == 1 || FUSE == 2)) RUN(T_Q4_0); break;
        case T_Q5_0: if constexpr (ENG == 0 && (FUSE == 1 || FUSE == 2)) RUN(T_Q5_0); break;
        case T_IQ4_NL: if constexpr (ENG == 0 && (FUSE == 1 || FUSE == 2)) RUN(T_IQ4_NL); break;
        case T_Q4_1: if constexpr (ENG == 0 && (FUSE == 1 || FUSE == 2)) RUN(T_Q4_1); break;
        case T_Q5_1: if constexpr (ENG == 0 && (FUSE == 1 || FUSE == 2)) RUN(T_Q5_1); break;
        case T_MXFP4: if constexpr (ENG == 0 && (FUSE == 1 || FUSE == 2)) RUN(T_MXFP4); break;
        case T_IQ4_XS: if constexpr (ENG == 0) RUN(T_IQ4_XS); break;
        default: break;
    }
#undef RUN
}

__device__ __forceinline__ void sync_init(uint8_t *smem) {
    if (threadIdx.x < 64) reinterpret_cast<int *>(smem + ST_OFF_SYNC)[threadIdx.x] = 0;
    __syncthreads();
}

}

}
```

cortex.llamacpp_amd/host/runtime.cc:

```cpp
#include "runtime.h"

#include <dlfcn.h>
#include "tp_comm.h"

#include <algorithm>
#include <atomic>
#include <cmath>
#include <cstdarg>
#include <cstdio>
#include <cstring>

namespace mi355 {

unsigned stream_error_epoch();
static unsigned *stream_error_word();

static thread_local std::string g_err;
void set_error(const char *fmt, ...) {
    char buf[1024];
    va_list ap;
    va_start(ap, fmt);
    vsnprintf(buf, sizeof buf, fmt, ap);
    va_end(ap);
    g_err = buf;
// ... 313 lines not shown
    d_delta_ = (int32_t *)dalloc(NC * 4);
    const size_t Tp = (T + 1) & ~(size_t)1;
    stage_bytes_ = 16 + Tp * 4 * 5 + Tp * 8;
    stage_bytes_ = (stage_bytes_ + 15) & ~(size_t)15;
    d_stage_ = (uint8_t *)dalloc(stage_bytes_);
    if (hipHostMalloc((void **)&h_stage_, stage_bytes_, hipHostMallocDefault) != hipSuccess) { err = "pinned alloc failed"; return false; }
    d_nkv_ = (int32_t *)d_stage_;
    d_tok_ = (int32_t *)(d_stage_ + 16);
    d_pos_ = d_tok_ + Tp;
    d_seq_ = d_pos_ + Tp;
    d_cell_ = d_seq_ + Tp;
    d_outrow_ = d_cell_ + Tp;
    d_seqmask_ = (uint64_t *)(d_outrow_ + Tp);

    const size_t QA = std::max(E, (size_t)hp.n_head * D);
    x_ = (float *)dalloc(T * E * 4);
    xn_ = (float *)dalloc(T * E * 4);
    q_ = (float *)dalloc(T * QA * 4);
    k_ = (float *)dalloc(T * G * D * 4);
    v_ = (float *)dalloc(T * G * D * 4);
    att_ = (float *)dalloc(T * QA * 4);
    ffn_ = (float *)dalloc(T * FF * 4);
    ffn_u_ = (float *)dalloc(T * FF * 4);
    xo_ = (float *)dalloc(T * E * 4);
    xb_ = (uint16_t *)dalloc(T * std::max({E, FF, QA}) * 2);
    if (hp.tp_exchange) {
        if (!tp_active() || tp_size() != hp.tp_size || tp_rank() != hp.tp_rank) { err = "model was loaded as rank " + std::to_string(hp.tp_rank) + " of " + std::to_string(hp.tp_size) + " but the process has no matching row-split group (mi355_tp_init)"; return false; }
        tp_part_ = (float *)dalloc(T * E * 4);
        if (tp_uses_host()) cp.use_graphs = false;
        if (const char *tg = getenv("MI355_TP_GRAPHS")) { if (tg[0] == '0') cp.use_graphs = false; }
    }
    if (hp.n_expert > 0) {
        router_ = (float *)dalloc(T * hp.n_expert * 4);
        moe_ids_ = (int32_t *)dalloc(T * hp.n_expert_used * 4);
        moe_w_ = (float *)dalloc(T * hp.n_expert_used * 4);
        moe_out_ = (float *)dalloc((size_t)hp.n_expert_used * T * E * 4);
        if (T >= 8) {
            const size_t GR = (size_t)hp.n_expert_used * T;
            bool okg = true;
            alloc_actq(aq_eg_, E, GR, true, true, allocs_, device_bytes, okg);
            alloc_actq(aq_ffg_, FF, GR, true, true, allocs_, device_bytes, okg);
            ffn_g_ = (float *)dalloc(GR * FF * 4);
            ffn_ug_ = (float *)dalloc(GR * FF * 4);
            y_g_ = (float *)dalloc(GR * E * 4);
            moe_meta_ = (int32_t *)dalloc((size_t)(2 * hp.n_expert + 1) * 4);
            moe_slot_ = (int32_t *)dalloc(GR * 4);
            moe_tok_ = (int32_t *)dalloc(GR * 4);
            if (!okg || !ffn_g_ || !ffn_ug_ || !y_g_ || !moe_tok_ ||
                hipHostMalloc((void **)&h_moe_meta_, (size_t)(2 * hp.n_expert + 1) * 4, hipHostMallocDefault) != hipSuccess) { err = "MoE batch buffers allocation failed"; return false; }
        }
    }
    bool ok = true;
    alloc_actq(aq_e_, E, T, true, true, allocs_, device_bytes, ok);
    alloc_actq(aq_o_, QA, T, true, true, allocs_, device_bytes, ok);
    alloc_actq(aq_ff_, FF, T, true, true, allocs_, device_bytes, ok);
    const int prep_rows = (int)T * (hp.n_expert > 0 ? std::max(1, (int)hp.n_expert_used) : 1);
    mmq_bh_ = (int8_t *)dalloc(mmq_prep_bytes((int)std::max({E, FF, QA}), prep_rows));
    mmq_bl_ = (int8_t *)dalloc(mmq_prep_bytes((int)std::max({E, FF, QA}), prep_rows));
    mmq_ws_.bytes = std::min((size_t)4 * T * std::max<size_t>(QA, (size_t)(hp.n_head + 2 * hp.n_head_kv) * D) * sizeof(float),
                             (size_t)(num_cu() * 7 / 4) * 128 * 256 * sizeof(float));
    mmq_ws_.p = T >= 128 ? (float *)dalloc(mmq_ws_.bytes) : nullptr;
    if (!mmq_ws_.p) mmq_ws_.bytes = 0;
    if (!ok || !x_ || !ffn_u_ || !xb_) { err = "activation buffer allocation failed"; return false; }

    size_t ws = 0;
    for (int t = 1; t <= (int)T; t++) {
        const int sp = flash_attn_pick_splits(t, (int)G, (int)NC);
        ws = std::max(ws, flash_attn_workspace_floats(t, hp.n_head, (int)D, sp));
    }
    ws = std::max(ws, flash_attn_workspace_floats(std::min<int>((int)T, 64), hp.n_head, (int)D, flash_attn_decode_splits((int)NC)));
    for (int t = 32; t <= (int)T; t += 32)
        ws = std::max(ws, flash_attn_workspace_floats(t, hp.n_head, (int)D, flash_attn_prefill_splits(t, hp.n_head, (int)G, (int)D, (int)NC)));
    att_part_ = (float *)dalloc(ws * 4);
    att_part_floats_ = ws;
    att_counters_ = (unsigned *)dalloc(64 * ATT_SYNC_STRIDE * sizeof(unsigned));
    if (!att_part_ || !att_counters_) { err = "attention workspace allocation failed"; return false; }
    if (hipMemset(att_counters_, 0, 64 * ATT_SYNC_STRIDE * sizeof(unsigned)) != hipSuccess) { err = "hipMemset failed"; return false; }
    d_step_serial_ = (unsigned *)dalloc(64);
    d_ao_flags_ = (unsigned *)dalloc((size_t)std::max(1, hp.n_layer) * 64 * ATT_SYNC_STRIDE * sizeof(unsigned));
    d_ao_gran_ = (unsigned long long *)dalloc(attn_out_granule_words((int)(hp.n_head * D)) * 8);
    d_qkv_gran_ = (unsigned long long *)dalloc(qkv_attn_granule_words((int)(hp.n_head * D), (int)(hp.n_head_kv * D)) * 8);
    if (!d_step_serial_ || !d_ao_flags_ || !d_ao_gran_ || !d_qkv_gran_) { err = "step serial / flag allocation failed"; return false; }
    d_argmax_ = (int32_t *)dalloc(T * 4);
    argmax_scratch_ = (float *)dalloc(T * 129 * 4);
    rope_cs_ = (float *)dalloc(T * (size_t)hp.n_rot * 4);
    chunk_stride_ = (int)((NC + 63) / 64);
    d_chunks_ = (int32_t *)dalloc((size_t)64 * (chunk_stride_ + 1) * 4);
    if (hipHostMalloc((void **)&h_chunks_, (size_t)64 * (chunk_stride_ + 1) * 4, hipHostMallocDefault) != hipSuccess) { err = "pinned alloc failed"; return false; }
    d_embd_ = (float *)dalloc(T * E * 4);
    if (hipHostMalloc((void **)&h_embd_, T * E * 4, hipHostMallocDefault) != hipSuccess) { err = "pinned alloc failed"; return false; }
    if (hipHostMalloc((void **)&h_argmax_, T * 4, hipHostMallocDefault) != hipSuccess) { err = "pinned alloc failed"; return false; }
    embeddings_enabled = cp.embeddings || model->hp.encoder;
    if (model->hp.encoder) {
        d_pos_open_ = (int32_t *)dalloc(T * 4);
        std::vector<int32_t> open((size_t)T, 0x7fffffff);
        if (!d_pos_open_ || hipMemcpy(d_pos_open_, open.data(), T * 4, hipMemcpyHostToDevice) != hipSuccess) { err = "encoder position buffer allocation failed"; return false; }
    }
    kv_clear();
    if (hipDeviceSynchronize() != hipSuccess) { err = "device synchronise failed"; return false; }
    return true;
}

void Context::kv_clear() {
    for (auto &c : cells_) c = KVCell();
    head_ = 0;
    has_shift_ = false;
    meta_dirty_ = true;
    region_next_.clear();
}
bool Context::kv_seq_rm(int seq, int p0, int p1) {
    if (seq >= 64) return false;
    if (p0 < 0) p0 = 0;
    if (p1 < 0) p1 = 0x7fffffff;
    int new_head = (int)cells_.size();
    for (int i = 0; i < (int)cells_.size(); i++) {
        KVCell &c = cells_[(size_t)i];
        if (c.pos < p0 || c.pos >= p1) continue;
        if (seq < 0) c.seqs = 0;
        else if (c.seqs & (1ull << seq)) c.seqs &= ~(1ull << seq);
        else continue;
        if (!c.seqs) { c.pos = -1; c.delta = 0; if (i < new_head) new_head = i; }
    }
    if (new_head < (int)cells_.size() && new_head < head_) head_ = new_head;
    if (new_head < (int)cells_.size()) region_next_.clear();
    meta_dirty_ = true;
    return true;
}
void Context::kv_seq_cp(int src, int dst, int p0, int p1) {
    if (src == dst || src < 0 || dst < 0 || src >= 64 || dst >= 64) return;
    if (p0 < 0) p0 = 0;
    if (p1 < 0) p1 = 0x7fffffff;
    for (auto &c : cells_)
        if ((c.seqs & (1ull << src)) && c.pos >= p0 && c.pos < p1) c.seqs |= 1ull << dst;
    meta_dirty_ = true;
}
void Context::kv_seq_add(int seq, int p0, int p1, int delta) {
    if (seq < 0 || seq >= 64) return;
    if (p0 < 0) p0 = 0;
    if (p1 < 0) p1 = 0x7fffffff;
    if (p0 == p1 || delta == 0) return;
    for (auto &c : cells_) {
        if (!(c.seqs & (1ull << seq)) || c.pos < p0 || c.pos >= p1) continue;
        has_shift_ = true;
        c.pos += delta;
        c.delta += delta;
        if (c.pos < 0) { c.pos = -1; c.seqs = 0; c.delta = 0; region_next_.clear(); }
    }
    meta_dirty_ = true;
}
int Context::kv_used_cells() const {
    int n = 0;
    for (const auto &c : cells_) n += c.pos >= 0;
    return n;
}

int Context::find_slot(int n) {
    const int NC = (int)cells_.size();
    if (n > NC) return -1;
    int head = head_, tested = 0;
    while (true) {
        if (head + n > NC) { tested += NC - head; head = 0; if (tested >= NC) return -1; continue; }
        bool ok = true;
        for (int i = 0; i < n; i++)
            if (cells_[(size_t)(head + i)].pos >= 0) { ok = false; head += i + 1; tested += i + 1; break; }
        if (ok) return head;
        if (tested >= NC) return -1;
// ... 46 lines not shown
    (void)hipStreamSynchronize(stream_);
    RopeArgs ra = rope_args(*model, true);
    for (int il = 0; il < hp.n_layer; il++)
        (void)launch_k_shift(kv_[(size_t)il], cp.type_k, hp.n_head_kv, hp.head_dim, (int)cp.n_ctx, d_delta_, ra, stream_);
    has_shift_ = false;
}

void Context::prof_begin() {
    if (!profile_) return;
    for (auto &pe : prof_events_) (void)hipEventDestroy(pe.second);
    prof_events_.clear();
    if (!ktimer_) ktimer_ = new KTimer;
    ktimer_->used = 0;
    set_kernel_timer(ktimer_);
    prof_mark("begin");
}
void Context::prof_mark(const char *name) {
    if (!profile_) return;
    hipEvent_t ev;
    if (hipEventCreate(&ev) != hipSuccess) return;
    (void)hipEventRecord(ev, stream_);
    prof_events_.emplace_back(name, ev);
}
void Context::prof_end() {
    if (!profile_) return;
    set_kernel_timer(nullptr);
    (void)hipStreamSynchronize(stream_);
    last_profile_.clear();
    if (ktimer_) {
        for (size_t i = 0; i < ktimer_->used; i++) {
            const KTimer::Rec &r = ktimer_->pool[i];
            float ms = 0;
            if (hipEventElapsedTime(&ms, r.a, r.b) != hipSuccess) continue;
            const std::string kn = std::string("k:") + r.role, nn = std::string("n:") + r.role;
            bool fk = false, fn = false;
            for (auto &e : last_profile_) { if (e.name == kn) { e.us += ms * 1000.0f; fk = true; } else if (e.name == nn) { e.us += 1.0f; fn = true; } }
            if (!fk) last_profile_.push_back({kn, ms * 1000.0f});
            if (!fn) last_profile_.push_back({nn, 1.0f});
        }
    }
    for (size_t i = 1; i < prof_events_.size(); i++) {
        float ms = 0;
        (void)hipEventElapsedTime(&ms, prof_events_[i - 1].second, prof_events_[i].second);
        bool found = false;
        for (auto &e : last_profile_)
            if (e.name == prof_events_[i].first) { e.us += ms * 1000.0f; found = true; break; }
        if (!found) last_profile_.push_back({prof_events_[i].first, ms * 1000.0f});
    }
}


static MMVQSeg make_seg(const DevTensor &w, float *out, int ld_out, const float *resid, const int32_t *esel) {
    MMVQSeg s{};
    s.W = w.data; s.out = out; s.resid = resid; s.type = w.type; s.n_rows = (int)w.N; s.ld_out = ld_out; s.row_bytes = w.row_bytes;
    s.expert_sel = esel; s.expert_stride = w.row_bytes * (size_t)w.N;
    return s;
}

static void chunk_act(MMVQArgs &a, const ActQuant &aq, int K, int t0) {
    a.aq = aq.qs ? aq.qs + (size_t)t0 * K : nullptr;
    a.ad = aq.d ? aq.d + (size_t)t0 * (K / 256) : nullptr;
    a.abs = aq.bsums ? aq.bsums + (size_t)t0 * (K / 16) : nullptr;
    a.aq0 = aq.qs0 ? aq.qs0 + (size_t)t0 * K : nullptr;
    a.ad0 = aq.d0 ? aq.d0 + (size_t)t0 * (K / 32) : nullptr;
}

static MMVQArgs single_token_desc(int n_seg, int K, int epi, int fuse, const float *nx, const float *nw, float eps, const ActQuant &aq) {
    MMVQArgs a{};
    a.n_seg = n_seg; a.K = K; a.T = 1; a.epi = epi;
    a.fuse_mode = fuse; a.nx = nx; a.nw = nw; a.neps = eps;
    chunk_act(a, aq, K, 0);
    return a;
}

static bool can_fuse(int K, int T) { return T == 1 && K <= 8192 && (K & 31) == 0; }

static hipError_t mmvq_tokens(MMVQSeg *segs, int n_seg, int K, int T, int epi, const ActQuant &aq, hipStream_t st, const Fuse &fz = Fuse()) {
    for (int t0 = 0; t0 < T;) {
        const int rem = T - t0, nt = rem >= 16 ? 16 : rem >= 8 ? 8 : rem >= 4 ? 4 : rem >= 2 ? 2 : 1;
        MMVQArgs a{};
        a.n_seg = n_seg; a.K = K; a.T = nt; a.epi = epi;
        a.fuse_mode = fz.mode; a.nx = fz.x; a.nw = fz.w; a.neps = fz.eps;
        a.out_host = nt == 1 && T == 1 ? fz.out_host : nullptr;
        for (int s = 0; s < n_seg; s++) {
            a.seg[s] = segs[s];
            a.seg[s].out = segs[s].out + (size_t)t0 * segs[s].ld_out;
            if (segs[s].resid) a.seg[s].resid = segs[s].resid + (size_t)t0 * segs[s].ld_out;
        }
        chunk_act(a, aq, K, t0);
        hipError_t e = launch_mmvq(a, st);
        if (e != hipSuccess) return e;
        t0 += nt;
    }
    return hipSuccess;
}

hipError_t Context::ensure_prep(const ActQuant &aq, int K, int T) {
    if (prep_owner_ == aq.qs && prep_K_ == K && prep_T_ == T && aq.qs) return hipSuccess;
    HIP_TRY(launch_mmq_prep(aq, K, T, mmq_bh_, mmq_bl_, stream_));
    prep_written(aq, K, T);
    return hipSuccess;
}

static bool q80_copy(const DevTensor &w, int K, int T) {
    return type_has_q80_copy(w.type) && w.planes && w.n_expert == 1 && mmq_q80_applicable(T_Q8_0, K, T);
}
static bool planes_small(const DevTensor &w, int K, int T) { return type_is_planes_only(w.type) && w.planes && T >= 32 && (K % 256) == 0; }

hipError_t Context::linear(const DevTensor &w, const ActQuant &aq, const float *x_f32, int K, int T, float *out, int ld_out,
                           const float *resid, int epi) {
    if (type_is_quant(w.type)) {
        if (mmq_q80_applicable(w.type, K, T) && pending_fuse_.mode == 0 && epi != EPI_SWIGLU && aq.qs0)
            return launch_mmq_q80(w.data, w.row_bytes, (int)w.N, K, T, aq, out, ld_out, epi == EPI_ADD ? resid : nullptr, stream_);
        const int8_t *bh = bh_over_ ? bh_over_ : mmq_bh_, *bl = bh_over_ ? bl_over_ : mmq_bl_;
        if (mmq_ksplit_preferred(w.type, (int)w.N, K, T, w.planes != nullptr) && pending_fuse_.mode == 0 && epi != EPI_SWIGLU) {
            if (w.type != T_Q6_K && !bh_over_) HIP_TRY(ensure_prep(aq, K, T));
            return launch_mmq_ksplit(w.type, w.data, w.row_bytes, (int)w.N, K, T, aq, bh, bl, out, ld_out, epi == EPI_ADD ? resid : nullptr, stream_);
        }
        if (mmq_applicable(w.type, K, T) && pending_fuse_.mode == 0 && epi != EPI_SWIGLU) {
            if ((w.type != T_Q6_K || !w.planes) && !bh_over_) HIP_TRY(ensure_prep(aq, K, T));
            if (w.planes) return launch_mmq_planes(w.type, w.planes, (int)w.N, K, T, aq, bh, bl, out, ld_out, epi == EPI_ADD ? resid : nullptr, stream_, mmq_ws_);
            return launch_mmq(w.type, w.data, w.row_bytes, (int)w.N, K, T, aq, bh, bl, out, ld_out, epi == EPI_ADD ? resid : nullptr, stream_);
        }
        if (q80_copy(w, K, T) && pending_fuse_.mode == 0 && epi != EPI_SWIGLU && aq.qs0)
            return launch_mmq_q80(w.planes, mmq_q80_copy_row_bytes(w.type, K), (int)w.N, K, T, aq, out, ld_out, epi == EPI_ADD ? resid : nullptr, stream_, mmq_q80_copy_form(w.type));
        if (planes_small(w, K, T) && pending_fuse_.mode == 0 && epi != EPI_SWIGLU && aq.qs) {
            if (w.type == T_Q2_K && !bh_over_) HIP_TRY(ensure_prep(aq, K, T));
            return launch_mmq_planes(w.type, w.planes, (int)w.N, K, T, aq, bh, bl, out, ld_out, epi == EPI_ADD ? resid : nullptr, stream_, mmq_ws_);
        }
        MMVQSeg s = make_seg(w, out, ld_out, resid, nullptr);
        return mmvq_tokens(&s, 1, K, T, epi, aq, stream_, pending_fuse_);
    }
    if (w.type == T_BF16) {
        const DevTensor *ws1[1] = {&w};
        float *outs1[1] = {out};
        HIP_TRY(launch_f32_to_bf16(x_f32, xb_, (size_t)T * K, stream_));
        return linear_bf16(ws1, outs1, nullptr, 1, K, T, ld_out, resid, epi);
    }
    if (mmf16_applicable(w.type, (int)w.N, K, T, w.data, x_f32, out) && w.n_expert == 1 && (ld_out & 3) == 0)
        return launch_mmf16(w.data, (int)w.N, K, x_f32, T, out, ld_out, epi == EPI_ADD ? resid : nullptr, stream_);
    return launch_mmv_float(w.type, w.data, (int)w.N, K, x_f32, T, out, ld_out, epi == EPI_ADD ? resid : nullptr, stream_);
}

static bool bf16_takes_mfma(const DevTensor *const *ws, float *const *outs, int n, int K, int T, int ld_out, const void *xb) {
    bool mfma = true;
    for (int i = 0; i < n; i++) mfma &= mmbf16_applicable(T_BF16, (int)ws[i]->N, K, T, ws[i]->data, xb, outs[i]) && ws[i]->n_expert == 1 && ((n == 1 ? ld_out : (int)ws[i]->N) & 3) == 0;
    return mfma;
}

hipError_t Context::linear_bf16(const DevTensor *const *ws, float *const *outs, const float *const *bias, int n, int K, int T, int ld_out, const float *resid, int epi) {
    if (bf16_takes_mfma(ws, outs, n, K, T, ld_out, xb_)) {
        for (int i = 0; i < n; i++)
            HIP_TRY(launch_mmbf16(ws[i]->data, (int)ws[i]->N, K, xb_, T, outs[i], n == 1 ? ld_out : (int)ws[i]->N, epi == EPI_ADD ? resid : nullptr, bias ? bias[i] : nullptr, 1.0f, false, stream_));
        if (epi == EPI_SWIGLU) HIP_TRY(launch_swiglu(outs[0], outs[1], outs[0], (int64_t)T * ws[0]->N, stream_));
        return hipSuccess;
    }
    MMVBF16Args a{};
    a.n_seg = n; a.K = K; a.epi = epi; a.resid = epi == EPI_ADD ? resid : nullptr; a.xb = xb_;
    for (int i = 0; i < n; i++) a.seg[i] = MMVBF16Seg{ws[i]->data, outs[i], bias ? bias[i] : nullptr, (int)ws[i]->N, n == 1 ? ld_out : (int)ws[i]->N, ws[i]->row_bytes};
    return launch_mmv_bf16_tokens(a, T, stream_);
}

hipError_t Context::linear_multi(const DevTensor *const *ws, float *const *outs, int n, const ActQuant &aq, const float *x_f32, int T, const float *const *bias, bool *bias_done) {
    bool all_q = true, all_bf = n <= 3;
    for (int i = 0; i < n; i++) { all_q &= type_is_quant(ws[i]->type); all_bf &= ws[i]->type == T_BF16 && ws[i]->n_expert == 1; }
    const int K = (int)ws[0]->K;
// ... 711 lines not shown
    if (exps_q && T >= g_moe_group_min && aq_eg_.qs) {
        HIP_TRY(launch_moe_group(moe_ids_, T, KU, hp.n_expert, moe_meta_, moe_slot_, moe_tok_, stream_));
        const bool one_launch = T >= 32 && L.gate_exps.planes && L.up_exps.planes && L.down_exps.planes && L.gate_exps.type == L.up_exps.type &&
                                L.gate_exps.N == L.up_exps.N && mmq_planes_moe_ok(L.gate_exps.type, (int)L.gate_exps.N, E) &&
                                mmq_planes_moe_ok(L.down_exps.type, (int)L.down_exps.N, FF) && (L.gate_exps.N % 64) == 0;
        const bool q80_ok = T >= 32 && L.gate_exps.planes && L.up_exps.planes && L.down_exps.planes && L.gate_exps.type == T_MXFP4 && L.up_exps.type == T_MXFP4 &&
                            L.down_exps.type == T_MXFP4 && L.gate_exps.N == L.up_exps.N && mmq_q80_moe_ok(T_MXFP4, (int)L.gate_exps.N, E) &&
                            mmq_q80_moe_ok(T_MXFP4, (int)L.down_exps.N, FF) && aq_eg_.qs0 && aq_ffg_.qs0;
        if (q80_ok && g_moe_q80_grouped) HIP_TRY(moe_grouped_q80(il, T));
        else HIP_TRY(one_launch ? moe_grouped_one_launch(il, T) : moe_grouped_per_expert(il, T, q80_ok));
    } else {
        HIP_TRY(moe_selected(il, T));
    }
    prof_mark("moe_ffn");
    return hipSuccess;
}

hipError_t Context::ffn_block(int il, const Step &st) {
    if (model->hp.n_expert > 0) return ffn_moe(il, st);
    bool quantised = false;
    HIP_TRY(ffn_dense_gate_up(il, st, quantised));
    HIP_TRY(ffn_down(il, st, quantised));
    if (st.tp) HIP_TRY(tp_reduce_into_x(st.T));
    prof_mark("ffn_down");
    return hipSuccess;
}

hipError_t Context::tap_layer(int il, int T) {
    if (!debug_taps_ || !dbg_) return hipSuccess;
    return hipMemcpyAsync(dbg_ + (size_t)il * cp.n_ubatch * model->hp.n_embd, x_, (size_t)T * model->hp.n_embd * 4, hipMemcpyDeviceToDevice, stream_);
}

hipError_t Context::run_layers(int T, int n_kv_cap) {
    if (model->hp.encoder) return run_layers_encoder(T, n_kv_cap);
    cur_T_ = T;
    const HParams &hp = model->hp;
    const int E = hp.n_embd, FF = hp.n_ff;
    Step st = step_constants(T, n_kv_cap);
    att_splits_ = flash_attn_pick_splits(T, hp.n_head_kv, st.n_kv_max);

    bool mega = T == 1 && !profile_ && !debug_taps_ && !ub_embd_ && mega_prepare();
    AttnArgs ma{};
    if (mega) {
        ma = attn_args(0, 1, st.n_kv_max, d_pos_);
        ma.out_q = &aq_o_; ma.out_q8k = !act_is_q80(model->layers[0].wo.type); ma.out_q80 = false;
        ma.splits = flash_attn_decode_splits(st.n_kv_max);
        if (st.chunk_lists) attn_chunk_lists(ma);
        mega = flash_attn_decode_fused_applicable(ma, st.ra_step);
    }
    st.engine = T == 1 && !mega && !profile_ && !debug_taps_ && !ub_embd_ && engine_prepare();
    last_layers_engine_ = st.engine;
    HIP_TRY(launch_step_setup_embed(d_pos_, T, st.ra_step, rope_cs_, d_cell_pos_, d_cell_seq_, d_cell_, d_seqmask_, mega ? d_mega_sync_ : nullptr,
                                    d_step_serial_, model->tok_embd.type, model->tok_embd.data, E, d_tok_, x_, stream_));
    if (ub_embd_) HIP_TRY(hipMemcpyAsync(x_, ub_embd_, (size_t)T * E * sizeof(float), hipMemcpyHostToDevice, stream_));
    prof_mark("embed");
    last_layers_mega_ = mega;
    if (mega)
        return launch_decode_mega(d_mega_layers_, hp.n_layer, (E + 2047) >> 11, (FF + 2047) >> 11, ma, rope_cs_, st.ra_step.n_rot, k_, v_, d_cell_,
                                  att_counters_, d_mega_sync_, h_mega_flag_, d_mega_probe_, mega_lds_, stream_);

    for (int il = 0; il < hp.n_layer; il++) {
        const AttnPlan ap = plan_attn(il, st);
        HIP_TRY(attn_qkv(il, st, ap));
        HIP_TRY(attn_core(il, st, ap));
        if (st.engine) {
            HIP_TRY(launch_decode_engine(d_engine_layers_ + il, E, FF, d_engine_gran_, d_engine_epoch_, il, il == engine_probe_layer_ ? d_engine_probe_ : nullptr, stream_));
        } else {
            HIP_TRY(attn_output(il, st, ap));
            if (st.tp) HIP_TRY(tp_reduce_into_x(T));
            prof_mark("attn_out");
            HIP_TRY(ffn_block(il, st));
        }
        HIP_TRY(tap_layer(il, T));
    }
    return hipSuccess;
}

hipError_t Context::tp_reduce_into_x(int T) {
    return tp_all_reduce_sum(tp_part_, x_, (size_t)T * model->hp.n_embd, stream_);
}

hipError_t Context::run_output(int n_out, int out_base) {
    logits_on_host_ = false;
    if (n_out <= 0) return hipSuccess;
    const HParams &hp = model->hp;
    const int E = hp.n_embd, V = hp.n_vocab;
    float *const xo = cur_T_ == 1 && n_out == 1 ? x_ : xo_;
    if (xo != x_) HIP_TRY(launch_gather_rows_f32(x_, d_outrow_, n_out, E, xo_, stream_));
    if (hp.encoder) {
        HIP_TRY(hipMemcpyAsync(d_embd_ + (size_t)out_base * E, xo, (size_t)n_out * E * 4, hipMemcpyDeviceToDevice, stream_));
        prof_mark("embd");
        return hipSuccess;
    }
    if (embeddings_enabled) {
        HIP_TRY(launch_rmsnorm_quant(xo, (const float *)model->out_norm.data, E, n_out, hp.eps, d_embd_ + (size_t)out_base * E, nullptr, false, false, stream_));
        prof_mark("embd");
        return hipSuccess;
    }
    const bool oq = type_is_quant(model->output.type);
    static const bool zc_env = !(getenv("MI355_LOGITS_ZERO_COPY") && getenv("MI355_LOGITS_ZERO_COPY")[0] == '0');
    logits_on_host_ = zc_env && oq && cur_T_ == 1 && n_out == 1 && cp.logits_to_host && !hp.tp_exchange && h_logits_ != nullptr;
    if (oq && can_fuse(E, n_out)) {
        pending_fuse_.mode = 1; pending_fuse_.x = xo; pending_fuse_.w = (const float *)model->out_norm.data; pending_fuse_.eps = hp.eps;
    } else {
        prep_owner_ = nullptr;
        HIP_TRY(launch_rmsnorm_quant(xo, (const float *)model->out_norm.data, E, n_out, hp.eps, oq ? nullptr : xn_, &aq_e_,
                                     oq && !act_is_q80(model->output.type), act_is_q80(model->output.type), stream_));
        prof_mark("norm_quant");
    }
    float *lg = d_logits_ + (size_t)out_base * V;
    const int VL = hp.n_vocab_local, P = hp.tp_size;
    if (hp.tp_exchange && VL * P == V) {
        if (n_out > 1 && (size_t)n_out > tp_logits_rows_) {
            HIP_TRY(hipStreamSynchronize(stream_));
            tp_logits_ = (float *)dalloc((size_t)n_out * V * 4);
            if (!tp_logits_) return hipErrorOutOfMemory;
            tp_logits_rows_ = (size_t)n_out;
            HIP_TRY(hipDeviceSynchronize());
        }
        float *gathered = n_out == 1 ? lg : tp_logits_;
        float *part = gathered + (size_t)hp.tp_rank * n_out * VL;
        HIP_TRY(linear(model->output, aq_e_, xn_, E, n_out, part, VL, nullptr, EPI_STORE));
        pending_fuse_ = Fuse();
        HIP_TRY(tp_all_gather(part, gathered, (size_t)n_out * VL, stream_));
        for (int r = 0; r < P && n_out > 1; r++)
            HIP_TRY(hipMemcpy2DAsync(lg + (size_t)r * VL, (size_t)V * 4, tp_logits_ + (size_t)r * n_out * VL, (size_t)VL * 4, (size_t)VL * 4, (size_t)n_out,
                                     hipMemcpyDeviceToDevice, stream_));
    } else {
        if (logits_on_host_) pending_fuse_.out_host = h_logits_ + (size_t)out_base * V;
        HIP_TRY(linear(model->output, aq_e_, xn_, E, n_out, lg, V, nullptr, EPI_STORE));
    }
    pending_fuse_ = Fuse();
    prof_mark("lm_head");
    for (int r0 = 0; r0 < n_out; r0 += (int)cp.n_ubatch) {
        const int nr = std::min((int)cp.n_ubatch, n_out - r0);
        HIP_TRY(launch_argmax_rows(lg + (size_t)r0 * V, V, nr, h_argmax_ + out_base + r0, argmax_scratch_, (int)cp.n_ubatch, stream_));
    }
    prof_mark("argmax");
    return hipSuccess;
}

int Context::decode_ubatch(int n, const int32_t *tokens, const int32_t *pos, const int32_t *seq, const uint64_t *seqmask,
                           const int8_t *flags, int out_base) {
    { const unsigned long long ls = next_launch_serial(); if (!first_unchecked_launch_) first_unchecked_launch_ = ls; }
    cur_max_pos_ = 0;
    for (int i = 0; i < n; i++) cur_max_pos_ = std::max(cur_max_pos_, (int)pos[i]);
    std::vector<int> tcell;
    if (!alloc_cells(n, seqmask, tcell)) return 1;
    for (int i = 0; i < n; i++) {
        KVCell &c = cells_[(size_t)tcell[(size_t)i]];
        c.pos = pos[i]; c.seqs = seqmask[i]; c.delta = 0;
    }
    int hi = 0;
    for (int i = (int)cells_.size() - 1; i >= 0; i--) if (cells_[(size_t)i].pos >= 0) { hi = i + 1; break; }
    n_kv_ = std::min((int)cp.n_ctx, (hi + 31) & ~31);

    if (meta_dirty_) {
        std::vector<int32_t> cpos(cells_.size());
        std::vector<uint64_t> cseq(cells_.size());
        for (size_t i = 0; i < cells_.size(); i++) { cpos[i] = cells_[i].pos; cseq[i] = cells_[i].seqs; }
        if (hipMemcpyAsync(d_cell_pos_, cpos.data(), cpos.size() * 4, hipMemcpyHostToDevice, stream_) != hipSuccess ||
            hipMemcpyAsync(d_cell_seq_, cseq.data(), cseq.size() * 8, hipMemcpyHostToDevice, stream_) != hipSuccess ||
            hipStreamSynchronize(stream_) != hipSuccess) { last_error = "cell table upload failed"; return -1; }
        meta_dirty_ = false;
    }
    if (stage_event_) (void)hipEventSynchronize(stage_event_);
    const size_t T = ((size_t)cp.n_ubatch + 1) & ~(size_t)1;
    int32_t *h_nkv = (int32_t *)h_stage_;
    int32_t *h_tok = (int32_t *)(h_stage_ + 16), *h_pos = h_tok + T, *h_seq = h_pos + T, *h_cell = h_seq + T, *h_out = h_cell + T;
    uint64_t *h_mask = (uint64_t *)(h_out + T);
    h_nkv[0] = n_kv_;
    int n_out = 0;
    for (int i = 0; i < n; i++) {
        h_tok[i] = tokens[i]; h_pos[i] = pos[i]; h_seq[i] = seq[i]; h_cell[i] = tcell[(size_t)i]; h_mask[i] = seqmask[i];
        if (flags[i]) h_out[n_out++] = i;
    }
    if (hipMemcpyAsync(d_stage_, h_stage_, stage_bytes_, hipMemcpyHostToDevice, stream_) != hipSuccess) { last_error = "token upload failed"; return -1; }
    chunk_lmax_ = 0;
    batch_distinct_ = n >= 2 && n <= 64;
    {
        uint64_t seen = 0;
        for (int i = 0; i < n && batch_distinct_; i++) {
            const uint64_t mk = seqmask[i];
            if (mk == 0 || (mk & (mk - 1)) != 0 || (seen & mk) != 0) batch_distinct_ = false;
            seen |= mk;
        }
    }
    bool lists_usable = false;
    {
        const HParams &hp = model->hp;
        RopeArgs ra = rope_args(*model, false);
        AttnArgs aa{};
        aa.T = n; aa.H = hp.n_head; aa.G = hp.n_head_kv; aa.D = hp.head_dim; aa.n_kv_max = n_kv_; aa.type_k = cp.type_k; aa.type_v = cp.type_v;
        lists_usable = n <= 64 && flash_attn_decode_applicable(aa, ra) && kv_store_fast_applicable(aa.G, aa.D, cp.type_k, cp.type_v, ra);
    }
    if ((n >= 2 || cp.n_seq_max > 1) && lists_usable) {
        const int nch = (n_kv_ + 63) / 64;
        std::vector<uint64_t> seq_of_chunk((size_t)nch, 0ull);
        for (int i = 0; i < n_kv_ && i < (int)cells_.size(); i++)
            if (cells_[(size_t)i].pos >= 0) seq_of_chunk[(size_t)(i >> 6)] |= cells_[(size_t)i].seqs;
        int32_t *cnt = h_chunks_ + (size_t)64 * chunk_stride_;
        for (int t = 0; t < n; t++) {
            int32_t *lst = h_chunks_ + (size_t)t * chunk_stride_;
            int c = 0;
            const uint64_t bit = 1ull << (seq[t] & 63);
            for (int ch = 0; ch < nch; ch++) if (seq_of_chunk[(size_t)ch] & bit) lst[c++] = ch;
            cnt[t] = c;
            chunk_lmax_ = std::max(chunk_lmax_, c);
        }
        if (chunk_lmax_ < 1) chunk_lmax_ = 1;
        if (hipMemcpyAsync(d_chunks_, h_chunks_, (size_t)64 * (chunk_stride_ + 1) * 4, hipMemcpyHostToDevice, stream_) != hipSuccess) { last_error = "chunk list upload failed"; return -1; }
    }
    static const bool profiler_safe = getenv("MI355_PROFILER_SAFE") && getenv("MI355_PROFILER_SAFE")[0] == '1';
    if (profiler_safe) (void)hipStreamSynchronize(stream_);
    if (!stage_event_) (void)hipEventCreateWithFlags(&stage_event_, hipEventDisableTiming);
    if (stage_event_) (void)hipEventRecord(stage_event_, stream_);

    const int V = model->hp.n_vocab;
    if (n == 1 && !model->hp.encoder && !ub_embd_) { (void)mega_prepare(); (void)engine_prepare(); }
    attn_out_skip_step_ = n == 1 && !attn_out_off_ && !model->hp.encoder && !fused_acquire();
    if (attn_out_skip_step_) fused_skipped_steps++;
    bool graph_ok = cp.use_graphs && n == 1 && n_out == 1 && out_base == 0 && !profile_ && !debug_taps_ && !embeddings_enabled && moe_forced_T_ == 0 && !ub_embd_ && !attn_out_skip_step_;
    hipError_t e = hipSuccess;
    if (graph_ok) {
        int bucket = std::min((int)cp.n_ctx, (n_kv_ + 255) & ~255);
        chunk_cap_ = 0;
        if (chunk_lmax_ > 0) {
            chunk_cap_ = std::min(chunk_stride_, (chunk_lmax_ + 3) & ~3);
            bucket = -chunk_cap_;
        }
        auto git = graphs_.find(bucket);
        graph_exec_ = git == graphs_.end() ? nullptr : git->second;
        if (!graph_exec_) {
            hipGraph_t g = nullptr;
            std::string inner;
            e = hipStreamBeginCapture(stream_, hipStreamCaptureModeThreadLocal);
            if (e == hipSuccess) {
                last_error.clear();
                hipError_t e2 = run_layers(1, bucket > 0 ? bucket : std::min((int)cp.n_ctx, chunk_cap_ * 64));
                if (e2 == hipSuccess) e2 = run_output(1, 0);
                if (e2 == hipSuccess && cp.logits_to_host && !logits_on_host_) e2 = hipMemcpyAsync(h_logits_, d_logits_, (size_t)V * 4, hipMemcpyDeviceToHost, stream_);
                if (e2 != hipSuccess) inner = last_error;
                e = hipStreamEndCapture(stream_, &g);
                if (e2 != hipSuccess) e = e2;
            }
            if (e == hipSuccess) e = hipGraphInstantiate(&graph_exec_, g, nullptr, nullptr, 0);
            if (g) (void)hipGraphDestroy(g);
            if (e != hipSuccess && model->hp.tp_exchange) {
                (void)hipGetLastError();
                cp.use_graphs = false;
                graph_ok = false;
                graph_exec_ = nullptr;
                e = hipSuccess;
            } else {
                if (e != hipSuccess) { last_error = std::string("graph capture failed: ") + hipGetErrorString(e) + (inner.empty() ? "" : " / " + inner); return -1; }
                graphs_[bucket] = graph_exec_;
                graph_is_mega_[graph_exec_] = last_layers_mega_;
                graph_is_engine_[graph_exec_] = last_layers_engine_;
            }
        }
        if (graph_ok) e = hipGraphLaunch(graph_exec_, stream_);
    }
    if (!graph_ok) {
        prof_begin();
        chunk_cap_ = chunk_lmax_;
        e = run_layers(n, n_kv_);
        if (e == hipSuccess) e = run_output(n_out, out_base);
        if (profiler_safe) (void)hipStreamSynchronize(stream_);
        if (e == hipSuccess && n_out > 0 && cp.logits_to_host && !embeddings_enabled && !logits_on_host_)
            e = hipMemcpyAsync(h_logits_ + (size_t)out_base * V, d_logits_ + (size_t)out_base * V, (size_t)n_out * V * 4, hipMemcpyDeviceToHost, stream_);
        prof_end();
    }
    if (e != hipSuccess) { last_error = std::string("decode failed: ") + hipGetErrorString(e) + " / " + last_error_string(); return -1; }
    if (n == 1 && (graph_ok ? graph_is_mega_[graph_exec_] : last_layers_mega_)) mega_steps++;
    if (n == 1 && (graph_ok ? graph_is_engine_[graph_exec_] : last_layers_engine_)) engine_steps++;
    dbg_tokens_ = n;
    return 0;
}

namespace {
struct RoctxApi {
    int (*push)(const char *) = nullptr;
    int (*pop)() = nullptr;
    RoctxApi() {
        const char *ev = getenv("MI355_ROCTX");
        if (!ev || ev[0] != '1') return;
        for (const char *n : {"librocprofiler-sdk-roctx.so.1", "librocprofiler-sdk-roctx.so", "libroctx64.so.4", "libroctx64.so"}) {
            if (void *h = dlopen(n, RTLD_NOW | RTLD_GLOBAL)) {
                push = reinterpret_cast<int (*)(const char *)>(dlsym(h, "roctxRangePushA"));
                pop = reinterpret_cast<int (*)()>(dlsym(h, "roctxRangePop"));
                if (push && pop) return;
                push = nullptr; pop = nullptr;
            }
        }
    }
};
struct TraceRange {
    static RoctxApi &api() { static RoctxApi a; return a; }
    bool on = false;
    TraceRange(const char *what, int n) {
        if (!api().push) return;
        char buf[96];
        snprintf(buf, sizeof buf, "mi355_decode %s n=%d", what, n);
        api().push(buf);
        on = true;
    }
    ~TraceRange() { if (on) api().pop(); }
};
}

int Context::decode(int n_tokens, const int32_t *tokens, const int32_t *pos, const int32_t *n_seq_id, int32_t *const *seq_id,
                    const int8_t *logits_flags, const float *embd) {
    if (n_tokens <= 0) { last_error = "empty batch"; return -1; }
    const TraceRange trace_range(embd ? "embeddings" : n_tokens == 1 ? "step" : n_tokens <= 64 ? "steps" : "prompt", n_tokens);
    std::vector<int32_t> no_tokens;
    if (embd) {
        if (model->hp.encoder) { last_error = "an encoder model takes token ids, not embeddings"; return -1; }
        if (tokens) { last_error = "a batch carries token ids or embeddings, not both"; return -1; }
        if (!pos) { last_error = "an embeddings batch needs positions"; return -1; }
        no_tokens.assign((size_t)n_tokens, 0);
        tokens = no_tokens.data();
    } else if (!tokens) { last_error = "batch without tokens"; return -1; }
    if (hipSetDevice(model->device) != hipSuccess) return -1;
    const HParams &hp = model->hp;
    if (hp.encoder && (size_t)n_tokens > cp.n_ubatch) { last_error = "encoder model: a batch of " + std::to_string(n_tokens) + " tokens does not fit one micro-batch (n_ubatch " + std::to_string(cp.n_ubatch) + ")"; return -1; }
    if (has_shift_) apply_k_shift();
    if (debug_taps_ && !dbg_) dbg_ = (float *)dalloc((size_t)hp.n_layer * cp.n_ubatch * hp.n_embd * 4);

    std::vector<int32_t> seq((size_t)n_tokens);
    std::vector<uint64_t> mask((size_t)n_tokens);
    std::vector<int8_t> flags((size_t)n_tokens);
    int n_out = 0;
    out_row_of_batch_.assign((size_t)n_tokens, -1);
    for (int i = 0; i < n_tokens; i++) {
        if (tokens[i] < 0 || tokens[i] >= hp.n_vocab) { last_error = "token id " + std::to_string(tokens[i]) + " out of range [0, " + std::to_string(hp.n_vocab) + ")"; return -1; }
        if (pos && pos[i] < 0) { last_error = "negative position " + std::to_string(pos[i]) + " for token " + std::to_string(i); return -1; }
        uint64_t mk = 0;
        const int ns = n_seq_id ? n_seq_id[i] : 1;
        for (int j = 0; j < ns; j++) {
            const int s = seq_id ? seq_id[i][j] : 0;
            if (s < 0 || s >= 64) { last_error = "seq id " + std::to_string(s) + " out of range [0, 64)"; return -1; }
            mk |= 1ull << s;
        }
        seq[(size_t)i] = seq_id ? seq_id[i][0] : 0;
        mask[(size_t)i] = mk;
        flags[(size_t)i] = logits_flags ? (logits_flags[i] != 0) : (i == n_tokens - 1);
        if (flags[(size_t)i]) out_row_of_batch_[(size_t)i] = n_out++;
    }
    if ((size_t)n_out > logits_cap_rows_) {
        (void)hipStreamSynchronize(stream_);
        if (d_logits_) { (void)hipFree(d_logits_); allocs_.erase(std::find(allocs_.begin(), allocs_.end(), (void *)d_logits_)); }
        if (h_logits_) (void)hipHostFree(h_logits_);
        if (d_argmax_) {  }
        const size_t rows = std::max<size_t>((size_t)n_out, 1);
        d_logits_ = (float *)dalloc(rows * hp.n_vocab * 4);
        if (!d_logits_ || hipHostMalloc((void **)&h_logits_, rows * hp.n_vocab * 4, hipHostMallocDefault) != hipSuccess) { last_error = "logits alloc failed"; return -1; }
        if (rows > cp.n_ubatch) {
            d_argmax_ = (int32_t *)dalloc(rows * 4);
// ... 244 lines not shown
```

cortex.llamacpp_amd/host/runtime.h:

```cpp
#pragma once

#include <hip/hip_runtime.h>

#include <cstdint>
#include <map>
#include <memory>
#include <string>
#include <vector>

#include "../csrc/kernels.h"
#include "gguf.h"
#include "model_plan.h"

namespace mi355 {

struct Model : ModelLayout {
    std::unique_ptr<GGUFFile> file;
    std::string path, desc;
    int device = 0;
    std::vector<uint8_t *> arenas;
    uint64_t device_bytes = 0, host_bytes = 0, file_tensor_bytes = 0, bytes_per_token = 0, planes_bytes = 0;
    ~Model();
};

Model *model_load(const std::string &path, int main_gpu, std::string &err, int &status, int prefill_planes = -1, int tp_rank = 0, int tp_size = 1);

struct KVCell {
    int32_t pos = -1;
    int32_t delta = 0;
    uint64_t seqs = 0;
};

void debug_raise_stream_error(unsigned code);
struct ContextParams {
    uint32_t n_ctx = 512, n_batch = 2048, n_ubatch = 512, n_seq_max = 1;
    int type_k = T_F16, type_v = T_F16;
    bool flash_attn = true, embeddings = false, use_graphs = true;
    bool logits_to_host = true;
};

struct ProfileEntry { std::string name; float us; };

struct Fuse {
    int mode = 0;
    const float *x = nullptr, *w = nullptr;
    float eps = 0.0f;
    float *out_host = nullptr;
};

void set_moe_q80_grouped(bool on);
void set_moe_group_min(int tokens);
void set_attn_store_fuse(bool on);
void set_rope_fast(bool on);
void set_decode_engine(int on);
void set_decode_mega(bool on);

class Context {
  public:
    int64_t engine_steps = 0;
    int64_t qkv_attn_launches = 0;
    int64_t fused_skipped_steps = 0;
    int64_t mega_steps = 0;
    Context(Model *m, const ContextParams &p);
    ~Context();
    bool init(std::string &err);

    int decode(int n_tokens, const int32_t *tokens, const int32_t *pos, const int32_t *n_seq_id, int32_t *const *seq_id,
               const int8_t *logits_flags, const float *embd = nullptr);
    float *logits_ith(int i);
    float *embeddings_ith(int i);
    int32_t argmax_ith(int i);
    int force_moe_ids(const int32_t *ids, int n_layer, int T, int k);
    int topk_ith(int i, int k, const TopkAdj &adj, int32_t *toks, float *logits);
    int topk_rows(int n, const int *is, const int *ks, const TopkAdj *adjs, int32_t *toks, float *logits);
    void synchronize();

    void kv_clear();
    bool kv_seq_rm(int seq, int p0, int p1);
    void kv_seq_cp(int src, int dst, int p0, int p1);
    void kv_seq_add(int seq, int p0, int p1, int delta);
    int kv_used_cells() const;

    int debug_layer_out(int il, float *dst, size_t cap);
    void set_debug_taps(bool on) { debug_taps_ = on; }
    void set_profile(bool on) { profile_ = on; }
    const std::vector<ProfileEntry> &last_profile() const { return last_profile_; }
    double bench_weight_sweep(int iters, uint64_t *bytes, int *launches = nullptr);

    Model *model;
    ContextParams cp;
    uint64_t device_bytes = 0;
    std::string last_error;
    bool embeddings_enabled = false;

  private:
    struct Bufs;
    const float *ub_embd_ = nullptr;
    int decode_ubatch(int n, const int32_t *tokens, const int32_t *pos, const int32_t *seq, const uint64_t *seqmask,
                      const int8_t *flags, int out_base);
    int find_slot(int n);
    bool alloc_cells(int n, const uint64_t *seqmask, std::vector<int> &out);
    std::vector<int> region_next_;
    void apply_k_shift();
    struct Step {
        int T = 0, n_kv_max = 0;
        RopeArgs ra_step{};
        bool engine = false;
        bool tp = false;
        bool chunk_lists = false;
        int attn_mode = 2;
        bool rope_fast = true, fuse_down_env = true;
        float *out = nullptr;
        const float *resid = nullptr;
    };
    struct AttnPlan {
        RopeArgs ra;
        AttnArgs aa, af;
        MMVQSeg ao_seg;
        int ao_epi;
        QKVFuse qf;
        bool qkv_float, qkv_prologue;
        bool o_planes;
        bool decode_attn, fused_step;
        bool ao_form, qkv_in_attn;
    };
    Step step_constants(int T, int n_kv_cap) const;
    AttnArgs attn_args(int il, int T, int n_kv_max, const int32_t *tok_pos) const;
    void attn_chunk_lists(AttnArgs &aa) const;
    AttnPlan plan_attn(int il, const Step &st) const;
    hipError_t attn_qkv(int il, const Step &st, const AttnPlan &p);
    hipError_t attn_core(int il, const Step &st, const AttnPlan &p);
    hipError_t attn_output(int il, const Step &st, const AttnPlan &p);
    hipError_t ffn_block(int il, const Step &st);
    hipError_t ffn_moe(int il, const Step &st);
    bool moe_selected_desc(int il, MMVQArgs &a, MMVQArgs &d) const;
    hipError_t moe_grouped_one_launch(int il, int T);
    hipError_t moe_grouped_per_expert(int il, int T, bool q80_any = false);
    hipError_t moe_grouped_q80(int il, int T);
    hipError_t moe_selected(int il, int T);
    hipError_t ffn_dense_gate_up(int il, const Step &st, bool &quantised);
    hipError_t quantise_for_down(int il, int T, bool combined, bool planes_any_T);
    hipError_t ffn_down(int il, const Step &st, bool quantised, int *n_matvec = nullptr);
    hipError_t tap_layer(int il, int T);
    hipError_t run_layers(int T, int n_kv_cap);
    hipError_t run_layers_encoder(int T, int n_kv_cap);
    hipError_t run_output(int n_out, int out_base);
    hipError_t linear(const DevTensor &w, const ActQuant &aq, const float *x_f32, int K, int T, float *out, int ld_out,
                      const float *resid, int epi);
    hipError_t linear_multi(const DevTensor *const *ws, float *const *outs, int n, const ActQuant &aq, const float *x_f32, int T, const float *const *bias = nullptr,
                            bool *bias_done = nullptr);
    hipError_t linear_bf16(const DevTensor *const *ws, float *const *outs, const float *const *bias, int n, int K, int T, int ld_out, const float *resid, int epi);
    void prof_mark(const char *name);
    void prof_begin();
    void prof_end();
    void *dalloc(size_t bytes);

    hipStream_t stream_ = nullptr;
    int cur_T_ = 0;
    std::vector<void *> allocs_;
    std::vector<KVCell> cells_;
    int head_ = 0;
    bool has_shift_ = false;
    bool meta_dirty_ = true;

    std::vector<KVLayerView> kv_;
    int32_t *d_cell_pos_ = nullptr;
    uint64_t *d_cell_seq_ = nullptr;
    int32_t *d_delta_ = nullptr;
    int32_t *d_pos_open_ = nullptr;
    int32_t *d_tok_ = nullptr, *d_pos_ = nullptr, *d_seq_ = nullptr, *d_cell_ = nullptr, *d_nkv_ = nullptr, *d_outrow_ = nullptr;
    uint64_t *d_seqmask_ = nullptr;
    uint8_t *h_stage_ = nullptr;
    size_t stage_bytes_ = 0;
    uint8_t *d_stage_ = nullptr;
    hipEvent_t stage_event_ = nullptr;
    float *x_ = nullptr, *xn_ = nullptr, *q_ = nullptr, *k_ = nullptr, *v_ = nullptr, *att_ = nullptr, *ffn_ = nullptr, *ffn_u_ = nullptr;
    float *xo_ = nullptr, *router_ = nullptr, *moe_out_ = nullptr;
    uint16_t *xb_ = nullptr;
    float *tp_part_ = nullptr, *tp_logits_ = nullptr;
    size_t tp_logits_rows_ = 0;
    hipError_t tp_reduce_into_x(int T);
    int32_t *moe_ids_ = nullptr;
    float *moe_w_ = nullptr;
    ActQuant aq_eg_, aq_ffg_;
    float *ffn_g_ = nullptr, *ffn_ug_ = nullptr, *y_g_ = nullptr;
    int32_t *moe_meta_ = nullptr, *moe_slot_ = nullptr, *moe_tok_ = nullptr, *h_moe_meta_ = nullptr;
    ActQuant aq_e_, aq_ff_, aq_o_;
    int8_t *mmq_bh_ = nullptr, *mmq_bl_ = nullptr;
    MMQWorkspace mmq_ws_;
    const void *prep_owner_ = nullptr;
    int prep_K_ = 0, prep_T_ = 0;
    hipError_t ensure_prep(const ActQuant &aq, int K, int T);
    void prep_written(const ActQuant &aq, int K, int T) { prep_owner_ = aq.qs; prep_K_ = K; prep_T_ = T; }
    bool batch_distinct_ = false;
    const int8_t *bh_over_ = nullptr, *bl_over_ = nullptr;
    float *att_part_ = nullptr;
    size_t att_part_floats_ = 0;
    int cur_max_pos_ = 0;
    float *d_embd_ = nullptr, *h_embd_ = nullptr;
    bool embd_fetched_ = false, last_was_embd_ = false;
    int32_t *h_chunks_ = nullptr, *d_chunks_ = nullptr;
    int chunk_stride_ = 0, chunk_lmax_ = 0, chunk_cap_ = 0;
    MegaLayer *d_mega_layers_ = nullptr;
    unsigned *d_mega_sync_ = nullptr;
    int *h_mega_flag_ = nullptr;
    unsigned long long *d_mega_probe_ = nullptr;
    size_t mega_lds_ = 0;
    bool last_layers_mega_ = false;
    std::map<hipGraphExec_t, bool> graph_is_mega_, graph_is_engine_;
    bool last_layers_engine_ = false;
    int mega_state_ = 0;
    bool mega_prepare();
    bool mega_check();
    EngineLayer *d_engine_layers_ = nullptr;
    unsigned long long *d_engine_gran_ = nullptr;
    unsigned *d_engine_epoch_ = nullptr;
    unsigned long long *d_engine_probe_ = nullptr;
    int engine_probe_layer_ = -1;
    unsigned err_epoch_seen_ = 0;
    unsigned long long first_unchecked_launch_ = 0;
    bool logits_on_host_ = false;
    bool attn_out_off_ = false;
    int engine_state_ = 0;
    bool engine_prepare();
    bool fused_acquire();
    void fused_release();
    bool holds_fused_ = false, attn_out_skip_step_ = false;
    bool stream_check();
    int32_t *d_moe_forced_ = nullptr;
    int moe_forced_T_ = 0, moe_forced_cap_ = 0;
    unsigned *att_counters_ = nullptr;
    unsigned *d_step_serial_ = nullptr;
    unsigned long long *d_qkv_gran_ = nullptr;
    unsigned long long *d_ao_gran_ = nullptr;
    unsigned *d_ao_flags_ = nullptr;
    float *argmax_scratch_ = nullptr, *rope_cs_ = nullptr;
    void *topk_scratch_ = nullptr;
    uint8_t *d_topk_adj_ = nullptr, *h_topk_adj_ = nullptr;
    int topk_rows_cap_ = 0;
    unsigned long long *h_topk_ = nullptr;
    Fuse pending_fuse_;
    int att_splits_ = 1;
    float *dbg_ = nullptr;
    bool debug_taps_ = false;
    int dbg_tokens_ = 0;
    float *d_logits_ = nullptr, *h_logits_ = nullptr;
    int32_t *d_argmax_ = nullptr, *h_argmax_ = nullptr;
    size_t logits_cap_rows_ = 0;
    std::vector<int> out_row_of_batch_;
    int n_out_last_ = 0;
    bool logits_fetched_ = false, argmax_fetched_ = false;
    hipGraphExec_t graph_exec_ = nullptr;
    std::map<int, hipGraphExec_t> graphs_;
    bool profile_ = false;
    std::vector<std::pair<std::string, hipEvent_t>> prof_events_;
    std::vector<ProfileEntry> last_profile_;
    struct KTimer;
    KTimer *ktimer_ = nullptr;
    int n_kv_ = 0;
};

}
```

include/mi355_llama.h:

```cpp
#ifndef MI355_LLAMA_H
#define MI355_LLAMA_H

#include <stddef.h>
#include <stdint.h>

#ifdef __cplusplus
extern "C" {
#endif

#define MI355_API __attribute__((visibility("default")))

typedef struct mi355_model   mi355_model;
typedef struct mi355_context mi355_context;

typedef int32_t mi355_token;
typedef int32_t mi355_pos;
typedef int32_t mi355_seq_id;

enum mi355_status {
    MI355_OK            = 0,
    MI355_ERR_NO_DEVICE = -100,
    MI355_ERR_IO        = -101,
    MI355_ERR_FORMAT    = -102,
    MI355_ERR_ARG       = -103,
// ... 7 lines not shown
};

MI355_API int         mi355_backend_init(void);
MI355_API void        mi355_backend_free(void);
MI355_API int         mi355_device_count(void);
MI355_API const char *mi355_last_error(void);
MI355_API int64_t     mi355_time_us(void);
MI355_API const char *mi355_print_system_info(void);

typedef struct mi355_model_params {
    int32_t n_gpu_layers;
    int32_t main_gpu;
    int32_t use_mmap;
    int32_t use_mlock;
    int32_t tp_rank;
    int32_t tp_size;
    int32_t prefill_planes;
} mi355_model_params;

MI355_API mi355_model_params mi355_model_default_params(void);
MI355_API mi355_model *mi355_model_load_from_file(const char *path_gguf, mi355_model_params params);
MI355_API void         mi355_model_free(mi355_model *model);

MI355_API int32_t  mi355_model_n_vocab(const mi355_model *m);
MI355_API int32_t  mi355_model_n_embd(const mi355_model *m);
MI355_API int32_t  mi355_model_n_layer(const mi355_model *m);
MI355_API int32_t  mi355_model_n_head(const mi355_model *m);
MI355_API int32_t  mi355_model_n_head_kv(const mi355_model *m);
MI355_API int32_t  mi355_model_n_ctx_train(const mi355_model *m);
MI355_API uint64_t mi355_model_size(const mi355_model *m);
MI355_API uint64_t mi355_model_cpu_buffer(const mi355_model *m);
MI355_API uint64_t mi355_model_other_buffer(const mi355_model *m);
MI355_API uint64_t mi355_model_bytes_per_token(const mi355_model *m);
MI355_API uint64_t mi355_model_planes_bytes(const mi355_model *m);
MI355_API const char *mi355_model_desc(const mi355_model *m);
MI355_API int mi355_model_meta_str(const mi355_model *m, const char *key, char *buf, size_t buf_size);

typedef struct mi355_context_params {
    uint32_t n_ctx;
    uint32_t n_batch;
    uint32_t n_ubatch;
    uint32_t n_seq_max;
    int32_t  type_k;
    int32_t  type_v;
    int32_t  flash_attn;
    int32_t  embeddings;
    int32_t  use_graphs;
    int32_t  logits_to_host;
} mi355_context_params;

MI355_API mi355_context_params mi355_context_default_params(void);
MI355_API mi355_context *mi355_context_new(mi355_model *model, mi355_context_params params);
MI355_API void           mi355_context_free(mi355_context *ctx);

MI355_API uint32_t mi355_n_ctx(const mi355_context *ctx);
MI355_API uint32_t mi355_n_batch(const mi355_context *ctx);
MI355_API uint32_t mi355_n_ubatch(const mi355_context *ctx);
MI355_API uint64_t mi355_context_device_bytes(const mi355_context *ctx);

typedef struct mi355_batch {
    int32_t        n_tokens;
    mi355_token   *token;
    float         *embd;
    mi355_pos     *pos;
    int32_t       *n_seq_id;
    mi355_seq_id **seq_id;
    int8_t        *logits;
} mi355_batch;

MI355_API mi355_batch mi355_batch_init(int32_t n_tokens, int32_t embd, int32_t n_seq_max);
MI355_API void        mi355_batch_free(mi355_batch batch);

MI355_API int32_t mi355_decode(mi355_context *ctx, mi355_batch batch);
MI355_API int32_t mi355_greedy_steps(mi355_context *ctx, mi355_token first, mi355_pos pos0, mi355_seq_id seq, int32_t n, mi355_token *out_tokens);
MI355_API float  *mi355_get_logits_ith(mi355_context *ctx, int32_t i);
MI355_API int32_t mi355_get_argmax_ith(mi355_context *ctx, int32_t i);
MI355_API int32_t mi355_get_topk_ith(mi355_context *ctx, int32_t i, int32_t k, int32_t n_adj, const int32_t *adj_tok, const float *adj_bias,
                                     const int32_t *adj_count, float penalty_repeat, float penalty_freq, float penalty_present,
                                     int32_t *toks_out, float *logits_out);
MI355_API int64_t mi355_debug_mega_steps(const mi355_context *ctx);
MI355_API int64_t mi355_debug_engine_steps(const mi355_context *ctx);
MI355_API int64_t mi355_debug_fused_skipped_steps(const mi355_context *ctx);
MI355_API int64_t mi355_debug_qkv_attn_launches(const mi355_context *ctx);
MI355_API int64_t mi355_debug_qkv_attn_plan(int32_t type_q, int32_t type_k, int32_t type_v, int32_t type_o, int32_t n_embd, int32_t n_head, int32_t n_head_kv, int32_t head_dim,
                                            int32_t type_kv, int32_t n_kv, int32_t *slots_out);
MI355_API void    mi355_set_embeddings(mi355_context *ctx, int32_t enabled);
MI355_API float  *mi355_get_embeddings_ith(mi355_context *ctx, int32_t i);
MI355_API void    mi355_synchronize(mi355_context *ctx);

MI355_API void    mi355_kv_cache_clear(mi355_context *ctx);
MI355_API int32_t mi355_kv_cache_seq_rm(mi355_context *ctx, mi355_seq_id seq, mi355_pos p0, mi355_pos p1);
MI355_API void    mi355_kv_cache_seq_cp(mi355_context *ctx, mi355_seq_id src, mi355_seq_id dst, mi355_pos p0, mi355_pos p1);
MI355_API void    mi355_kv_cache_seq_add(mi355_context *ctx, mi355_seq_id seq, mi355_pos p0, mi355_pos p1, mi355_pos delta);
MI355_API int32_t mi355_kv_cache_used_cells(const mi355_context *ctx);

MI355_API void    mi355_debug_enable_taps(mi355_context *ctx, int32_t enabled);
MI355_API int32_t mi355_debug_layer_out(mi355_context *ctx, int32_t il, float *dst, size_t dst_floats);


MI355_API int mi355_op_quantize_act(int32_t act_type, const float *x, int64_t n_per_row, int64_t n_rows, void *out_blocks);
MI355_API int mi355_op_rms_norm_quant(const float *x, const float *w, int64_t n, int64_t T, float eps, float *y_f32, void *out_blocks);
MI355_API int mi355_op_swiglu_quant(const float *gate, const float *up, int64_t n, int64_t T, void *out_blocks);
MI355_API int mi355_op_mul_mat(int32_t type, const void *W, int64_t N, int64_t K, const float *x, int64_t T,
                               float *y, int32_t *isum, int32_t *msum);
MI355_API int mi355_op_mul_mat_add(int32_t type, const void *W, int64_t N, int64_t K, const float *x, int64_t T, const float *resid, float *y);
MI355_API int mi355_op_mul_mat_fused(int32_t type, const void *W, int64_t N, int64_t K, const float *x, const float *norm_w, float eps, float *y);
MI355_API int mi355_op_f32_to_bf16(const float *x, int64_t n, uint16_t *out);
MI355_API int mi355_op_mul_mat_bf16(int32_t n_seg, const void *const *W, const int64_t *N, int64_t K, const float *x, int64_t T, const float *const *bias,
                                    const float *resid, int32_t epi, int32_t path, int32_t tokens_per_launch, int32_t use_graph, float *const *y);
MI355_API int mi355_op_ffn_gate_up(int32_t type, const void *Wg, const void *Wu, int64_t N, int64_t K, const float *x, int64_t T, float *y);
MI355_API int mi355_op_rms_norm_mul(const float *x, const float *w, int64_t n, int64_t T, float eps, float *y);
MI355_API int mi355_op_rope(float *x, int32_t n_head, int32_t head_dim, int32_t n_rot, const int32_t *pos, int64_t T,
                            float freq_base, float freq_scale, const float *freq_factors, int32_t neox);
MI355_API int mi355_op_rope_yarn(float *x, int32_t n_head, int32_t head_dim, int32_t n_rot, const int32_t *pos, int64_t T,
                                 float freq_base, float freq_scale, const float *freq_factors, int32_t neox,
                                 float ext_factor, float attn_factor, float corr_lo, float corr_hi);
MI355_API int mi355_op_get_rows(int32_t type, const void *table, int64_t row_elems, int64_t n_rows_table,
                                const int32_t *ids, int64_t n_ids, float *dst);
MI355_API int mi355_op_swiglu(const float *gate, const float *up, int64_t n, float *y);
MI355_API int mi355_op_soft_max(const float *x, const float *mask, int64_t n, int64_t rows, float scale, float *y);
MI355_API int mi355_op_moe_route(const float *logits, int64_t T, int32_t n_expert, int32_t k, int32_t *ids, float *w);
MI355_API int mi355_op_moe_router(int32_t type, const void *gate_inp, int32_t n_expert, int64_t K, const float *x, int64_t T, int32_t k, int32_t fused,
                                  const int32_t *forced, float *logits, int32_t *ids, float *w);
MI355_API int mi355_op_flash_attn(const float *q, int64_t T, int32_t n_head, int32_t n_head_kv, int32_t head_dim,
                                  int32_t type_k, const void *k, int32_t type_v, const void *v, int32_t n_cells,
                                  const int32_t *cell_pos, const int32_t *q_pos, float scale, float *out);

MI355_API int mi355_op_attn_step(const float *q, const float *k_new, const float *v_new, int32_t n_head, int32_t n_head_kv, int32_t head_dim, int32_t type_k,
                                 const void *k, int32_t type_v, const void *v, int32_t n_cells, const int32_t *cell_pos, int32_t tok_pos, int32_t tok_cell,
                                 float rope_base, int32_t n_rot, float scale, int32_t type_o, const void *W_o, int64_t n_embd, const float *resid, int32_t fused,
                                 float *att_out, float *out, void *k_row_out, void *v_row_out);
MI355_API int mi355_op_attn_decode_neox(const float *q, const float *k_new, const float *v_new, int32_t n_head, int32_t n_head_kv, int32_t head_dim,
                                        int32_t type_k, const void *k, int32_t type_v, const void *v, int32_t n_cells, const int32_t *cell_pos, int32_t tok_pos,
                                        int32_t tok_cell, float rope_base, float scale, const float *q_norm, const float *k_norm, float eps, int32_t mode,
                                        float *att_out, void *k_row_out, void *v_row_out);
MI355_API int mi355_op_kv_store(int32_t form, float *q, const float *k, const float *v, int64_t T, int32_t n_head, int32_t n_head_kv, int32_t head_dim,
                                int32_t n_rot, int32_t neox, int32_t type_k, int32_t type_v, int32_t n_cells, const int32_t *tok_pos, const int32_t *tok_cell,
                                float rope_base, float freq_scale, const float *freq_factors, const float *q_norm, const float *k_norm, float eps,
                                void *k_cache, void *v_cache);
MI355_API int mi355_op_k_shift(int32_t type_k, int32_t n_head_kv, int32_t head_dim, int32_t n_rot, int32_t neox, int32_t n_cells, const int32_t *delta,
                               float rope_base, float freq_scale, const float *freq_factors, float ext_factor, float attn_factor, float corr_lo,
                               float corr_hi, void *k_cache);

MI355_API int32_t mi355_tokenize(mi355_model *m, const char *text, int32_t text_len, mi355_token *out, int32_t cap,
                                 int32_t add_special, int32_t parse_special);
MI355_API int32_t mi355_token_to_piece(mi355_model *m, mi355_token tok, char *buf, int32_t cap, int32_t special);
MI355_API mi355_token mi355_token_bos(mi355_model *m);
MI355_API mi355_token mi355_token_eos(mi355_model *m);
MI355_API int32_t mi355_token_is_eog(mi355_model *m, mi355_token tok);

typedef struct mi355_engine mi355_engine;
typedef void (*mi355_engine_callback)(const char *status_json, const char *body_json, void *user);
MI355_API mi355_engine *mi355_engine_create(void);
MI355_API void mi355_engine_destroy(mi355_engine *e);
MI355_API void mi355_engine_set_release_callback(mi355_engine *e, void (*release)(void *user));
MI355_API void mi355_engine_load_model(mi355_engine *e, const char *body_json, mi355_engine_callback cb, void *user);
MI355_API void mi355_engine_unload_model(mi355_engine *e, const char *body_json, mi355_engine_callback cb, void *user);
MI355_API void mi355_engine_get_model_status(mi355_engine *e, const char *body_json, mi355_engine_callback cb, void *user);
MI355_API void mi355_engine_get_models(mi355_engine *e, const char *body_json, mi355_engine_callback cb, void *user);
MI355_API void mi355_engine_handle_chat_completion(mi355_engine *e, const char *body_json, mi355_engine_callback cb, void *user);
MI355_API void mi355_engine_handle_embedding(mi355_engine *e, const char *body_json, mi355_engine_callback cb, void *user);
MI355_API int32_t mi355_engine_is_supported(mi355_engine *e, const char *feature);
MI355_API void mi355_engine_stop_inferencing(mi355_engine *e, const char *model_id);
MI355_API void mi355_engine_load(mi355_engine *e, const char *engine_path, const char *deps_path, int32_t is_custom_engine_path, const char *log_path,
                                 int32_t max_log_lines, int32_t log_level);
MI355_API void mi355_engine_unload(mi355_engine *e);
// ... 49 lines not shown
```

Baseline: 679.3.

## Fuse greedy argmax into the streaming LM-head matvec epilogue

When a single decode token needs one output row, the LM-head streaming kernel now tracks a running per-lane argmax as it stores logits. It reduces within each wave and workgroup, then across workgroups through a global partial buffer with an atomic last-block-finishes pattern. That lets the host skip the separate argmax_rows launch. It adds atomics, an extra reduction tail in the head kernel, and debug counters for graph node count and fused steps, and it is enabled by default unless an env var turns it off.

```diff
diff --git a/cortex.llamacpp_amd/binding.py b/cortex.llamacpp_amd/binding.py
--- a/cortex.llamacpp_amd/binding.py
+++ b/cortex.llamacpp_amd/binding.py
@@ -84,6 +84,8 @@
     "mi355_debug_engine_steps": (C.c_int64, [_vp]),
     "mi355_debug_fused_skipped_steps": (C.c_int64, [_vp]),
     "mi355_debug_qkv_attn_launches": (C.c_int64, [_vp]),
+    "mi355_debug_head_argmax_steps": (C.c_int64, [_vp]),
+    "mi355_debug_last_graph_nodes": (C.c_int64, [_vp]),
     "mi355_debug_qkv_attn_plan": (C.c_int64, [C.c_int32] * 10 + [C.POINTER(C.c_int32)]),
     "mi355_set_embeddings": (None, [_vp, _i32]),
     "mi355_get_embeddings_ith": (C.POINTER(C.c_float), [_vp, _i32]),
@@ -748,6 +750,12 @@
     def qkv_attn_launches(self) -> int:
         return int(self.lib.mi355_debug_qkv_attn_launches(self.h))
 
+    def head_argmax_steps(self) -> int:
+        return int(self.lib.mi355_debug_head_argmax_steps(self.h))
+
+    def last_graph_nodes(self) -> int:
+        return int(self.lib.mi355_debug_last_graph_nodes(self.h))
+
     def engine_steps(self) -> int:
         return int(self.lib.mi355_debug_engine_steps(self.h))
 
diff --git a/cortex.llamacpp_amd/csrc/c_api.cc b/cortex.llamacpp_amd/csrc/c_api.cc
--- a/cortex.llamacpp_amd/csrc/c_api.cc
+++ b/cortex.llamacpp_amd/csrc/c_api.cc
@@ -250,6 +250,8 @@
 int64_t mi355_debug_engine_steps(const mi355_context *ctx) { return ctx->c->engine_steps; }
 int64_t mi355_debug_fused_skipped_steps(const mi355_context *ctx) { return ctx->c->fused_skipped_steps; }
 int64_t mi355_debug_qkv_attn_launches(const mi355_context *ctx) { return ctx->c->qkv_attn_launches; }
+int64_t mi355_debug_head_argmax_steps(const mi355_context *ctx) { return ctx->c->head_argmax_steps; }
+int64_t mi355_debug_last_graph_nodes(const mi355_context *ctx) { return ctx->c->last_graph_nodes; }
 int64_t mi355_debug_qkv_attn_plan(int32_t type_q, int32_t type_k, int32_t type_v, int32_t type_o, int32_t n_embd, int32_t n_head, int32_t n_head_kv, int32_t head_dim,
                                   int32_t type_kv, int32_t n_kv, int32_t *slots_out) {
     int slots = 0;
@@ -1259,6 +1261,7 @@
     if (!strcmp(name, "tp_p2p_prompt")) { tp_p2p_use_prompt(value != 0); return MI355_OK; }
     if (!strcmp(name, "mmvq_stream")) { mmvq_set_stream(value != 0); return MI355_OK; }
     if (!strcmp(name, "attn_out_fused")) { set_attn_out_fused(value); return MI355_OK; }
+    if (!strcmp(name, "head_argmax")) { set_head_argmax(value); return MI355_OK; }
     if (!strcmp(name, "qkv_attn_fused")) { set_qkv_attn_fused(value); return MI355_OK; }
     if (!strcmp(name, "moe_group_min")) { set_moe_group_min(value); return MI355_OK; }
     if (!strcmp(name, "moe_q80_grouped")) { set_moe_q80_grouped(value != 0); return MI355_OK; }
diff --git a/cortex.llamacpp_amd/csrc/kernels.h b/cortex.llamacpp_amd/csrc/kernels.h
--- a/cortex.llamacpp_amd/csrc/kernels.h
+++ b/cortex.llamacpp_amd/csrc/kernels.h
@@ -42,7 +42,15 @@
     const float *nx; const float *nw; float neps;
     int n_sel, sel_out_stride, sel_nx_stride;
     float *out_host;
-};
+    int32_t *amax_out;
+    unsigned *amax_sync;
+    int amax_parts;
+    int *amax_taken;
+};
+constexpr int MMVQ_AMAX_MAX_PARTS = 1024;
+constexpr size_t MMVQ_AMAX_SYNC_BYTES = 128 + (size_t)MMVQ_AMAX_MAX_PARTS * 8;
+void set_head_argmax(int on);
+bool head_argmax_enabled();
 
 hipError_t launch_mmvq(MMVQArgs a, hipStream_t st);
 void mmvq_fast_set_threads(int nt);
diff --git a/cortex.llamacpp_amd/csrc/mmvq_stream.hip b/cortex.llamacpp_amd/csrc/mmvq_stream.hip
--- a/cortex.llamacpp_amd/csrc/mmvq_stream.hip
+++ b/cortex.llamacpp_amd/csrc/mmvq_stream.hip
@@ -4,14 +4,14 @@
 
 namespace {
 
-template <int KB, int FUSE, bool MOE>
+template <int KB, int FUSE, bool MOE, bool HEAD = false>
 __device__ __forceinline__ void stream_body(const MMVQArgs &ka) {
     extern __shared__ __attribute__((aligned(16))) uint8_t smem[];
 #ifdef MI355_STREAM_PROBE
     const unsigned long long t_top = wall_clock64();
 #endif
     StOp a;
-    op_setup<false, MOE>(ka, a);
+    op_setup<false, MOE, HEAD>(ka, a);
     const int wave = uni(tid_now() >> 6);
     sync_init(smem);
 #ifdef MI355_STREAM_PROBE
@@ -38,7 +38,7 @@
         ST_STAMP(5);
         return;
     }
-    consumer_dispatch<KB, FUSE>(a, smem, wave - ST_NL, 0u, st_layout(KB));
+    consumer_dispatch<KB, FUSE, 0, false, HEAD>(a, smem, wave - ST_NL, 0u, st_layout(KB));
 }
 struct StFast { const float *nx; const uint8_t *wbase; unsigned ow0, ow1, ow2, onw, kf, sg0, sg1, sg2, rb01, rb2; };
 __device__ __forceinline__ void st_fast_setup(StFast f, StOp &o) {
@@ -64,7 +64,7 @@
     o.ns_pad = (o.ns_raw + 1) & ~1;
 }
 
-template <int KB>
+template <int KB, bool HEAD>
 __device__ __forceinline__ void stream_body_fast(const StFast &fa) {
     extern __shared__ __attribute__((aligned(16))) uint8_t smem[];
     const int wave = uni(tid_now() >> 6), lane = tid_now() & 63;
@@ -86,7 +86,7 @@
     asm volatile("" : "+s"(kseg) :: "memory");
     const __attribute__((address_space(4))) MMVQArgs &ka = *(KArgP)(kseg + 56);
     StOp a;
-    op_setup<false, false>(ka, a);
+    op_setup<false, false, HEAD>(ka, a);
     if (wave == ST_NL && lane == 0) {
         StOp la;
         st_fast_setup(fa, la);
@@ -95,16 +95,16 @@
                                                                  (a.swiglu && la.W1 != a.W1)))) st_timeout(ST_ERR_LOADER);
     }
     if (a.n_rows_wg <= 0) return;
-    consumer_dispatch<KB, 1, 0, true>(a, smem, wave - ST_NL, 0u, st_layout(KB), EngIO(), &ea);
-}
-#define MI355_ST_KERNEL_FAST(NAME)                                                                            \
+    consumer_dispatch<KB, 1, 0, true, HEAD>(a, smem, wave - ST_NL, 0u, st_layout(KB), EngIO(), &ea);
+}
+#define MI355_ST_KERNEL_FAST(NAME, HEAD)                                                                      \
     template <int KB>                                                                                         \
     __global__ __launch_bounds__(ST_NT) void NAME(const float *f_nx, const uint8_t *f_wbase, unsigned f_ow0, unsigned f_ow1, unsigned f_ow2, unsigned f_onw, unsigned f_kf, \
                                                   unsigned f_sg0, unsigned f_sg1, unsigned f_sg2, unsigned f_rb01, unsigned f_rb2, const MMVQArgs ka_by_value) {            \
-        stream_body_fast<KB>(StFast{f_nx, f_wbase, f_ow0, f_ow1, f_ow2, f_onw, f_kf, f_sg0, f_sg1, f_sg2, f_rb01, f_rb2});                                                \
-    }
-MI355_ST_KERNEL_FAST(mmvq_stream_gate_up_fast)
-MI355_ST_KERNEL_FAST(mmvq_stream_head_fast)
+        stream_body_fast<KB, HEAD>(StFast{f_nx, f_wbase, f_ow0, f_ow1, f_ow2, f_onw, f_kf, f_sg0, f_sg1, f_sg2, f_rb01, f_rb2});                                                \
+    }
+MI355_ST_KERNEL_FAST(mmvq_stream_gate_up_fast, false)
+MI355_ST_KERNEL_FAST(mmvq_stream_head_fast, true)
 #undef MI355_ST_KERNEL_FAST
 
 template <int KB>
@@ -138,14 +138,14 @@
     stream_body_early<KB>(f_nx, f_k8);
 }
 
-#define MI355_ST_KERNEL(NAME)                                                                                 \
+#define MI355_ST_KERNEL(NAME, HEAD)                                                                           \
     template <int KB, int FUSE, bool MOE = false>                                                             \
-    __global__ __launch_bounds__(ST_NT) void NAME(const MMVQArgs ka) { stream_body<KB, FUSE, MOE>(ka); }
-MI355_ST_KERNEL(mmvq_stream_kernel)
-MI355_ST_KERNEL(mmvq_stream_qkv)
-MI355_ST_KERNEL(mmvq_stream_gate_up)
-MI355_ST_KERNEL(mmvq_stream_ffn_down)
-MI355_ST_KERNEL(mmvq_stream_head)
+    __global__ __launch_bounds__(ST_NT) void NAME(const MMVQArgs ka) { stream_body<KB, FUSE, MOE, HEAD>(ka); }
+MI355_ST_KERNEL(mmvq_stream_kernel, false)
+MI355_ST_KERNEL(mmvq_stream_qkv, false)
+MI355_ST_KERNEL(mmvq_stream_gate_up, false)
+MI355_ST_KERNEL(mmvq_stream_ffn_down, false)
+MI355_ST_KERNEL(mmvq_stream_head, true)
 #undef MI355_ST_KERNEL
 
 }
@@ -196,6 +196,13 @@
     return true;
 }
 
+static int g_head_argmax = -1;
+void set_head_argmax(int on) { g_head_argmax = on < 0 ? -1 : on ? 1 : 0; }
+bool head_argmax_enabled() {
+    static const bool env_off = getenv("MI355_HEAD_ARGMAX") && getenv("MI355_HEAD_ARGMAX")[0] == '0';
+    return g_head_argmax < 0 ? !env_off : g_head_argmax > 0;
+}
+
 void mmvq_stream_set_error_word(unsigned *w) { (void)hipMemcpyToSymbol(HIP_SYMBOL(g_st_err_word), &w, sizeof(w)); }
 
 void mmvq_stream_plan(MMVQArgs &a, int max_blocks) {
@@ -264,9 +271,16 @@
     if (a.n_sel <= 1 && !a.seg[0].expert_sel) {
         if (a.fuse_mode == 1 && a.epi == EPI_SWIGLU) role = ROLE_GATE_UP;
         else if (a.fuse_mode == 1 && a.epi == EPI_STORE && a.n_seg >= 2) role = ROLE_QKV;
-        else if (a.fuse_mode == 1 && a.epi == EPI_STORE && a.n_seg == 1 && a.seg[0].n_rows >= 16384) role = ROLE_HEAD;
+        else if (a.fuse_mode == 1 && a.epi == EPI_STORE && a.n_seg == 1 && (a.seg[0].n_rows >= 16384 || (a.amax_out && a.amax_sync))) role = ROLE_HEAD;
         else if (a.fuse_mode == 2 && a.epi == EPI_ADD && a.n_seg == 1) role = ROLE_DOWN;
     }
+    if (role == ROLE_HEAD && a.amax_out && a.amax_sync && blocks > 0) {
+        const int rpb = (a.seg[0].n_rows + blocks - 1) / blocks;
+        a.amax_parts = (a.seg[0].n_rows + rpb - 1) / rpb;
+    } else a.amax_parts = 0;
+    if (a.amax_parts < 1 || a.amax_parts > MMVQ_AMAX_MAX_PARTS) { a.amax_out = nullptr; a.amax_sync = nullptr; a.amax_parts = 0; }
+    else if (a.amax_taken) *a.amax_taken = 1;
+    a.amax_taken = nullptr;
     const char *const role_name = role == ROLE_QKV ? "qkv" : role == ROLE_GATE_UP ? "gate_up" : role == ROLE_DOWN ? "ffn_down" : role == ROLE_HEAD ? "head" : "stream";
     (void)role_name;
     static const bool fast_off = getenv("MI355_STREAM_FAST_START") && getenv("MI355_STREAM_FAST_START")[0] == '0';
diff --git a/cortex.llamacpp_amd/csrc/mmvq_stream_dev.h b/cortex.llamacpp_amd/csrc/mmvq_stream_dev.h
--- a/cortex.llamacpp_amd/csrc/mmvq_stream_dev.h
+++ b/cortex.llamacpp_amd/csrc/mmvq_stream_dev.h
@@ -170,7 +170,7 @@
     l.total = l.bs + ((Kp / 8 + 1023) & ~1023);
     return l;
 }
-enum { SY_LANDED = 0, SY_GO = 2, SY_THIN = 3, SY_PRO1 = 8, SY_PRO2 = 12, SY_DONE = 16, SY_READY = 17, SY_ABORT = 18, SY_GATHER = 19, SY_GDONE = 20, SY_STEP = 21, SY_FRONT = 24 };
+enum { SY_LANDED = 0, SY_GO = 2, SY_THIN = 3, SY_PRO1 = 8, SY_PRO2 = 12, SY_DONE = 16, SY_READY = 17, SY_ABORT = 18, SY_GATHER = 19, SY_GDONE = 20, SY_STEP = 21, SY_FRONT = 24, SY_AMAX = 40 };
 
 #ifndef MI355_STREAM_SPIN_LIMIT
 #define MI355_STREAM_SPIN_LIMIT (1 << 21)
@@ -201,6 +201,7 @@
     unsigned row_bytes, total;
     bool swiglu, pair;
     int ns_raw, ns_pad;
+    int32_t *amax_out; unsigned *amax_sync; int amax_parts;
 };
 template <bool MEM, class T> __device__ __forceinline__ T st_uni(T v) {
     if constexpr (!MEM) return v;
@@ -234,7 +235,7 @@
         return __builtin_bit_cast(T, w);
     }
 }
-template <bool MEM = false, bool MOE = false, class KA = MMVQArgs>
+template <bool MEM = false, bool MOE = false, bool HEAD = false, class KA = MMVQArgs>
 __device__ __forceinline__ void op_setup(const KA &ka, StOp &o) {
     StDescRegs dr{0u, 0u};
     if constexpr (MEM) dr = st_desc_load(*reinterpret_cast<const MMVQArgs *>(&ka));
@@ -257,6 +258,8 @@
         es0 = U(ka.seg[0].expert_sel); es1 = U(ka.seg[1].expert_sel);
         est0 = U(ka.seg[0].expert_stride); est1 = U(ka.seg[1].expert_stride);
     }
+    int32_t *amo = nullptr; unsigned *ams = nullptr; int amp = 0;
+    if constexpr (HEAD) { amo = U(ka.amax_out); ams = U(ka.amax_sync); amp = U(ka.amax_parts); }
 #undef U
 #define PIN(x) asm volatile("" :: "s"(x))
     PIN(n_seg); PIN(sb0); PIN(sb1); PIN(sb2); PIN(sb3); PIN(K); PIN(epi); PIN(nck); PIN(neps);
@@ -264,7 +267,9 @@
     PIN(w0); PIN(w1); PIN(w2); PIN(o0); PIN(o1); PIN(o2); PIN(oh); PIN(r0); PIN(r1); PIN(r2);
     PIN(t0); PIN(t1); PIN(t2); PIN(n0); PIN(n1); PIN(n2); PIN(rb0); PIN(rb1); PIN(rb2);
     if constexpr (MOE) { PIN(n_sel); PIN(sel_os); PIN(sel_ns); PIN(es0); PIN(es1); PIN(est0); PIN(est1); }
+    if constexpr (HEAD) { PIN(amo); PIN(ams); PIN(amp); }
 #undef PIN
+    o.amax_out = n_seg == 1 ? amo : nullptr; o.amax_sync = ams; o.amax_parts = amp;
     int s = 0;
     if (n_seg > 1 && (int)blockIdx.x >= sb1) s = 1;
     if (n_seg > 2 && (int)blockIdx.x >= sb2) s = 2;
@@ -515,13 +520,66 @@
     return nq + 1 + nbs;
 }
 
-template <int TYPE, int KB, int FUSE, bool SWIGLU, bool PAIR, int ENG = 0, bool EARLY = false>
+__device__ __forceinline__ bool amax_better(float v, int i, float best, int idx) { return v > best || (v == best && i < idx); }
+__device__ __forceinline__ void amax_wave_reduce(float &best, int &idx) {
+#pragma unroll
+    for (int o = 32; o > 0; o >>= 1) {
+        const float ov = __shfl_xor(best, o, 64);
+        const int oi = __shfl_xor(idx, o, 64);
+        if (amax_better(ov, oi, best, idx)) { best = ov; idx = oi; }
+    }
+}
+__device__ __noinline__ void head_argmax_finish(int32_t *out, unsigned *sync, int parts, uint8_t *smem, int c, float best, int idx) {
+    const int lane = tid_now() & 63;
+    int *sy = reinterpret_cast<int *>(smem + ST_OFF_SYNC);
+    float *wv = reinterpret_cast<float *>(smem + ST_OFF_RED + 128);
+    int *wi = reinterpret_cast<int *>(smem + ST_OFF_RED + 192);
+    amax_wave_reduce(best, idx);
+    int t = 0;
+    if (lane == 0) {
+        __hip_atomic_store(wv + c, best, __ATOMIC_RELAXED, __HIP_MEMORY_SCOPE_WORKGROUP);
+        __hip_atomic_store(wi + c, idx, __ATOMIC_RELAXED, __HIP_MEMORY_SCOPE_WORKGROUP);
+        asm volatile("" ::: "memory");
+        t = __hip_atomic_fetch_add(sy + SY_AMAX, 1, __ATOMIC_RELAXED, __HIP_MEMORY_SCOPE_WORKGROUP);
+    }
+    if (uni(t) != ST_NC - 1) return;
+    asm volatile("" ::: "memory");
+    best = -INFINITY; idx = 0x7fffffff;
+    if (lane < ST_NC) {
+        best = __hip_atomic_load(wv + lane, __ATOMIC_RELAXED, __HIP_MEMORY_SCOPE_WORKGROUP);
+        idx = __hip_atomic_load(wi + lane, __ATOMIC_RELAXED, __HIP_MEMORY_SCOPE_WORKGROUP);
+    }
+    amax_wave_reduce(best, idx);
+    unsigned long long *part = reinterpret_cast<unsigned long long *>(sync + 32);
+    int last = 0;
+    if (lane == 0) {
+        __hip_atomic_store(part + blockIdx.x, ((unsigned long long)(unsigned)idx << 32) | __float_as_uint(best), __ATOMIC_RELAXED, __HIP_MEMORY_SCOPE_AGENT);
+        asm volatile("s_waitcnt vmcnt(0)" ::: "memory");
+        const unsigned tk = __hip_atomic_fetch_add(sync, 1u, __ATOMIC_RELAXED, __HIP_MEMORY_SCOPE_AGENT);
+        last = tk == (unsigned)(parts - 1) ? 1 : 0;
+        if (last) __hip_atomic_store(sync, 0u, __ATOMIC_RELAXED, __HIP_MEMORY_SCOPE_AGENT);
+    }
+    if (!uni(last)) return;
+    asm volatile("" ::: "memory");
+    best = -INFINITY; idx = 0x7fffffff;
+    for (int j = lane; j < parts; j += 64) {
+        const unsigned long long w = __hip_atomic_load(part + j, __ATOMIC_RELAXED, __HIP_MEMORY_SCOPE_AGENT);
+        const float v = __uint_as_float((unsigned)w);
+        const int i = (int)(unsigned)(w >> 32);
+        if (amax_better(v, i, best, idx)) { best = v; idx = i; }
+    }
+    amax_wave_reduce(best, idx);
+    if (lane == 0) out[0] = idx;
+}
+
+template <int TYPE, int KB, int FUSE, bool SWIGLU, bool PAIR, int ENG = 0, bool EARLY = false, bool HEAD = false>
 __device__ __forceinline__ void consumer_op(const StOp &a, uint8_t *smem, int c, unsigned g0, const StLayout &lay, const EngIO &io = EngIO(), const EarlyAct<KB> *ea = nullptr) {
     using R = Raw<TYPE>;
     constexpr int NP = role_passes<TYPE, KB>(), SBP = role_sbp<TYPE>();
     constexpr bool ACT_REGS = NP <= 2;
     constexpr int STEP = (SWIGLU || PAIR) ? 2 : 1;
     constexpr int UO = (PAIR && !SWIGLU) ? 2 : 1;
+    constexpr bool AMAX = HEAD && ENG == 0 && !SWIGLU;
     const int lane = tid_now() & 63;
     const int wave = c + ST_NL; (void)wave;
     const LaneRole L = make_role<TYPE>(lane);
@@ -580,6 +638,8 @@
         if (NP > 1) S1 = read_slice_t<TYPE>(AL, SBP + L.sbl, nb, L);
     }
 
+    float am_best = -INFINITY;
+    int am_idx = 0x7fffffff;
     float res = 0.0f;
     int rrow = b0;
     int n_done = 0, flushed = 0;
@@ -597,6 +657,7 @@
             } else {
                 a.out[row] = v;
                 if (ENG == 0 && a.out2) a.out2[row] = v;
+                if (AMAX && amax_better(v, row, am_best, am_idx)) { am_best = v; am_idx = row; }
             }
         }
         flushed = upto;
@@ -664,18 +725,19 @@
     ST_ACC_OUT();
     if (eprobe && lane == 0) { io.probe[1] = ep_w; io.probe[2] = ep_d; }
     if (flushed < n_done) flush(n_done);
+    if constexpr (AMAX) { if (a.amax_out) head_argmax_finish(a.amax_out, a.amax_sync, a.amax_parts, smem, c, am_best, am_idx); }
 #ifdef MI355_STREAM_PROBE
     asm volatile("s_waitcnt vmcnt(0)" ::: "memory");
     ST_STAMP(5);
 #endif
 }
-template <int KB, int FUSE, int ENG = 0, bool EARLY = false>
+template <int KB, int FUSE, int ENG = 0, bool EARLY = false, bool HEAD = false>
 __device__ __forceinline__ void consumer_dispatch(const StOp &a, uint8_t *smem, int c, unsigned g0, const StLayout &lay, const EngIO &io = EngIO(), const EarlyAct<KB> *ea = nullptr) {
 #define RUN(TY)                                                                                               \
     do {                                                                                                      \
-        if (a.swiglu) { if constexpr (FUSE == 1 || (FUSE == 3 && KB <= 4)) consumer_op<TY, KB, FUSE, true, true, ENG, EARLY>(a, smem, c, g0, lay, io, ea); } \
-        else if (a.pair) { if constexpr (KB <= 4 || ENG == 0) consumer_op<TY, KB, FUSE, false, true, ENG, EARLY>(a, smem, c, g0, lay, io, ea); } \
-        else { if constexpr (KB >= 3) consumer_op<TY, KB, FUSE, false, false, ENG, EARLY>(a, smem, c, g0, lay, io, ea); } \
+        if (a.swiglu) { if constexpr (FUSE == 1 || (FUSE == 3 && KB <= 4)) consumer_op<TY, KB, FUSE, true, true, ENG, EARLY, HEAD>(a, smem, c, g0, lay, io, ea); } \
+        else if (a.pair) { if constexpr (KB <= 4 || ENG == 0) consumer_op<TY, KB, FUSE, false, true, ENG, EARLY, HEAD>(a, smem, c, g0, lay, io, ea); } \
+        else { if constexpr (KB >= 3) consumer_op<TY, KB, FUSE, false, false, ENG, EARLY, HEAD>(a, smem, c, g0, lay, io, ea); } \
     } while (0)
     switch (a.type) {
         case T_Q4_K: RUN(T_Q4_K); break;
diff --git a/cortex.llamacpp_amd/host/runtime.cc b/cortex.llamacpp_amd/host/runtime.cc
--- a/cortex.llamacpp_amd/host/runtime.cc
+++ b/cortex.llamacpp_amd/host/runtime.cc
@@ -419,6 +419,7 @@
     d_qkv_gran_ = (unsigned long long *)dalloc(qkv_attn_granule_words((int)(hp.n_head * D), (int)(hp.n_head_kv * D)) * 8);
     if (!d_step_serial_ || !d_ao_flags_ || !d_ao_gran_ || !d_qkv_gran_) { err = "step serial / flag allocation failed"; return false; }
     d_argmax_ = (int32_t *)dalloc(T * 4);
+    head_amax_sync_ = (unsigned *)dalloc(MMVQ_AMAX_SYNC_BYTES);
     argmax_scratch_ = (float *)dalloc(T * 129 * 4);
     rope_cs_ = (float *)dalloc(T * (size_t)hp.n_rot * 4);
     chunk_stride_ = (int)((NC + 63) / 64);
@@ -631,6 +632,7 @@
         a.n_seg = n_seg; a.K = K; a.T = nt; a.epi = epi;
         a.fuse_mode = fz.mode; a.nx = fz.x; a.nw = fz.w; a.neps = fz.eps;
         a.out_host = nt == 1 && T == 1 ? fz.out_host : nullptr;
+        if (nt == 1 && T == 1 && n_seg == 1 && epi == EPI_STORE) { a.amax_out = fz.amax_out; a.amax_sync = fz.amax_sync; a.amax_taken = fz.amax_taken; }
         for (int s = 0; s < n_seg; s++) {
             a.seg[s] = segs[s];
             a.seg[s].out = segs[s].out + (size_t)t0 * segs[s].ld_out;
@@ -1508,6 +1510,8 @@
 
 hipError_t Context::run_output(int n_out, int out_base) {
     logits_on_host_ = false;
+    last_head_argmax_ = false;
+    int amax_taken = 0;
     if (n_out <= 0) return hipSuccess;
     const HParams &hp = model->hp;
     const int E = hp.n_embd, V = hp.n_vocab;
@@ -1554,11 +1558,15 @@
                                      hipMemcpyDeviceToDevice, stream_));
     } else {
         if (logits_on_host_) pending_fuse_.out_host = h_logits_ + (size_t)out_base * V;
+        if (pending_fuse_.mode == 1 && cur_T_ == 1 && n_out == 1 && head_amax_sync_ && head_argmax_enabled()) {
+            pending_fuse_.amax_out = h_argmax_ + out_base; pending_fuse_.amax_sync = head_amax_sync_; pending_fuse_.amax_taken = &amax_taken;
+        }
         HIP_TRY(linear(model->output, aq_e_, xn_, E, n_out, lg, V, nullptr, EPI_STORE));
     }
     pending_fuse_ = Fuse();
     prof_mark("lm_head");
-    for (int r0 = 0; r0 < n_out; r0 += (int)cp.n_ubatch) {
+    last_head_argmax_ = amax_taken != 0;
+    for (int r0 = 0; r0 < n_out && !last_head_argmax_; r0 += (int)cp.n_ubatch) {
         const int nr = std::min((int)cp.n_ubatch, n_out - r0);
         HIP_TRY(launch_argmax_rows(lg + (size_t)r0 * V, V, nr, h_argmax_ + out_base + r0, argmax_scratch_, (int)cp.n_ubatch, stream_));
     }
@@ -1670,6 +1678,8 @@
                 e = hipStreamEndCapture(stream_, &g);
                 if (e2 != hipSuccess) e = e2;
             }
+            size_t n_nodes = 0;
+            if (e == hipSuccess && g) (void)hipGraphGetNodes(g, nullptr, &n_nodes);
             if (e == hipSuccess) e = hipGraphInstantiate(&graph_exec_, g, nullptr, nullptr, 0);
             if (g) (void)hipGraphDestroy(g);
             if (e != hipSuccess && model->hp.tp_exchange) {
@@ -1683,6 +1693,8 @@
                 graphs_[bucket] = graph_exec_;
                 graph_is_mega_[graph_exec_] = last_layers_mega_;
                 graph_is_engine_[graph_exec_] = last_layers_engine_;
+                graph_head_argmax_[graph_exec_] = last_head_argmax_;
+                graph_nodes_[graph_exec_] = (int64_t)n_nodes;
             }
         }
         if (graph_ok) e = hipGraphLaunch(graph_exec_, stream_);
@@ -1700,6 +1712,8 @@
     if (e != hipSuccess) { last_error = std::string("decode failed: ") + hipGetErrorString(e) + " / " + last_error_string(); return -1; }
     if (n == 1 && (graph_ok ? graph_is_mega_[graph_exec_] : last_layers_mega_)) mega_steps++;
     if (n == 1 && (graph_ok ? graph_is_engine_[graph_exec_] : last_layers_engine_)) engine_steps++;
+    if (n == 1 && n_out == 1 && (graph_ok ? graph_head_argmax_[graph_exec_] : last_head_argmax_)) head_argmax_steps++;
+    if (n == 1) last_graph_nodes = graph_ok ? graph_nodes_[graph_exec_] : 0;
     dbg_tokens_ = n;
     return 0;
 }
diff --git a/cortex.llamacpp_amd/host/runtime.h b/cortex.llamacpp_amd/host/runtime.h
--- a/cortex.llamacpp_amd/host/runtime.h
+++ b/cortex.llamacpp_amd/host/runtime.h
@@ -46,6 +46,7 @@
     const float *x = nullptr, *w = nullptr;
     float eps = 0.0f;
     float *out_host = nullptr;
+    int32_t *amax_out = nullptr; unsigned *amax_sync = nullptr; int *amax_taken = nullptr;
 };
 
 void set_moe_q80_grouped(bool on);
@@ -59,6 +60,8 @@
   public:
     int64_t engine_steps = 0;
     int64_t qkv_attn_launches = 0;
+    int64_t head_argmax_steps = 0;
+    int64_t last_graph_nodes = 0;
     int64_t fused_skipped_steps = 0;
     int64_t mega_steps = 0;
     Context(Model *m, const ContextParams &p);
@@ -207,7 +210,10 @@
     unsigned long long *d_mega_probe_ = nullptr;
     size_t mega_lds_ = 0;
     bool last_layers_mega_ = false;
-    std::map<hipGraphExec_t, bool> graph_is_mega_, graph_is_engine_;
+    std::map<hipGraphExec_t, bool> graph_is_mega_, graph_is_engine_, graph_head_argmax_;
+    std::map<hipGraphExec_t, int64_t> graph_nodes_;
+    bool last_head_argmax_ = false;
+    unsigned *head_amax_sync_ = nullptr;
     bool last_layers_engine_ = false;
     int mega_state_ = 0;
     bool mega_prepare();
diff --git a/include/mi355_llama.h b/include/mi355_llama.h
--- a/include/mi355_llama.h
+++ b/include/mi355_llama.h
@@ -113,6 +113,8 @@
 MI355_API int64_t mi355_debug_engine_steps(const mi355_context *ctx);
 MI355_API int64_t mi355_debug_fused_skipped_steps(const mi355_context *ctx);
 MI355_API int64_t mi355_debug_qkv_attn_launches(const mi355_context *ctx);
+MI355_API int64_t mi355_debug_head_argmax_steps(const mi355_context *ctx);
+MI355_API int64_t mi355_debug_last_graph_nodes(const mi355_context *ctx);
 MI355_API int64_t mi355_debug_qkv_attn_plan(int32_t type_q, int32_t type_k, int32_t type_v, int32_t type_o, int32_t n_embd, int32_t n_head, int32_t n_head_kv, int32_t head_dim,
                                             int32_t type_kv, int32_t n_kv, int32_t *slots_out);
 MI355_API void    mi355_set_embeddings(mi355_context *ctx, int32_t enabled);
```

Result: slower. 662.9 (-2.4%).
